# CRIPAC-DIG/GET

Measured on AMD Instinct MI355X. Metric: claim-evidence pairs/sec fwd+bwd (B=32, h=300), higher is better.
Workload: dtype f32

## Files before the change

### get_amd/_lib.py

```python
from __future__ import annotations

import ctypes
import os

import torch

_HERE = os.path.dirname(os.path.abspath(__file__))
LIB_PATH = os.environ.get("GET_AMD_LIB") or os.path.join(_HERE, "lib", "libget_hip.so")

_P = ctypes.c_void_p
_I = ctypes.c_int
_F = ctypes.c_float
_L = ctypes.c_int64
_U = ctypes.c_uint32
ABI_VERSION = 10

SIGNATURES = {
    "gh_graph_build": [_P, _P, _I, _I, _I, _P, _P, _P, _P, _P],
    "gh_adj_pack_f64": [_P, _I, _I, _P, _P, _P],
    "gh_ref_depad": [_P, _I, _I, _I, _P, _I, _P, _P, _P, _P, _P, _P, _P, _I, _P],
    "gh_adj_pack_f32": [_P, _I, _I, _P, _P, _P],
    "gh_ragged_plan": [_P, _P, _I, _I, _P, _P, _P, _P, _P, _P],
    "gh_spmm": [_P, _P, _P, _P, _P, _I, _P, _P, _I, _I, _I, _I, _I, _P],
    "gh_spmm_bf16": [_P, _P, _P, _P, _P, _I, _P, _P, _I, _I, _I, _I, _I, _P],
    "gh_transpose": [_P, _P, _I, _I, _P],
    "gh_transpose_batch": [_I, _P, _P, _P, _P, _P],
    "gh_ggnn_cell_fwd": [_P] * 5 + [_I, _I] + [_P] * 2 + [_I] * 4 + [_P] * 13 + [_P] * 7 + [_F, _U, _P, _P, _F, _U, _P],
    "gh_ggnn_cell_bwd": [_P] * 5 + [_I] + [_P] * 2 + [_I] * 4 + [_P] * 7 + [_P] * 7 + [_P] * 5 + [_P] * 14 + [_F, _U, _P],
    "gh_ggnn_cell_fwd_bf16": [_P] * 5 + [_I, _I] + [_P] * 2 + [_I] * 4 + [_P] * 13 + [_P] * 8 + [_F, _U, _P, _P, _F, _U, _P],
    "gh_ggnn_cell_bwd_bf16": [_P] * 5 + [_I] + [_P] * 2 + [_I] * 4 + [_P] * 7 + [_P] * 7 + [_P] * 5 + [_P] * 14 + [_F, _U, _P],
    "gh_scorer_gsl": [_P, _P, _P, _P, _I, _P, _P, _P, _P, _I, _I, _I, _I, _P, _P, _F, _U, _P],
    "gh_gsl_topk": [_P, _I, _I, _I, _P, _P],
    "gh_adj_unpack": [_P, _P, _P, _P, _I, _I, _P, _P],
    "gh_concat_att_fwd": [_P, _P, _P, _P, _P, _I, _I, _I, _I, _I, _I, _I, _P, _P, _P, _P, _P, _P, _P, _P],
    "gh_concat_att_bwd": [_P, _P, _P, _I, _I, _I, _I, _I, _I, _I, _P, _P, _P, _P, _P, _P, _P, _P, _P, _P, _P, _P, _P, _P],
    "gh_linear_fwd": [_P, _P, _P, _P, _I, _I, _I, _P],
    "gh_linear_bwd": [_P, _P, _P, _P, _I, _I, _I, _P, _P, _P, _P],
    "gh_linear_wgrad_bf16": [_P, _I, _P, _I, _I, _I, _I, _P, _I, _P, _P],
    "gh_gat_layer_fwd": [_P] * 6 + [_I] * 5 + [_F, _I, _I, _F, _U] + [_P] * 5 + [_P],
    "gh_gat_layer_bwd": [_P] * 6 + [_I] * 5 + [_F, _I, _I, _F, _U] + [_P] * 11 + [_P],
    "gh_gcn_norm": [_P, _P, _P, _P, _I, _I, _P, _P],
    "gh_feat_dropout": [_P, _P, _I, _I, _F, _U, _P],
    "gh_scale_rows": [_P, _P, _P, _P, _I, _I, _P],
    "gh_evd_assemble_fwd": [_P, _P, _P, _I, _P, _I, _P, _I, _I, _I, _I, _I, _I, _P, _P, _P],
    "gh_evd_assemble_bwd": [_P, _P, _P, _I, _I, _I, _I, _I, _I, _P, _P, _P],
    "gh_clamp_events": [_P, _I],
    "gh_weights_refresh": [_I, _P, _P, _P, _P, _P, _P, _P],
    "gh_seg_offsets": [_P, _I, _P, _P, _I, _P, _P],
    "gh_seg_broadcast": [_P, _P, _P, _I, _I, _P],
    "gh_seg_sum": [_P, _P, _P, _I, _I, _P],
    "gh_seg_pad": [_P, _P, _P, _I, _I, _I, _I, _P],
    "gh_seg_unpad": [_P, _P, _P, _I, _I, _I, _I, _P],
    "gh_masked_mean_fwd": [_P, _P, _P, _P, _I, _I, _I, _P],
    "gh_masked_mean_bwd": [_P, _P, _P, _P, _I, _I, _I, _P],
    "gh_adam_step": [_P, _P, _P, _P, _L, _F, _F, _F, _F, _F, _I, _F, _P],
    "gh_set_workspace": [_P, _L],
    "gh_set_stream_workspace": [_P, _P, _L],
    "gh_profile_enable": [_I],
    "gh_profile_select": [_U],
    "gh_profile_collect": [_P, _I],
    "gh_gemm_path_counters": [_P, _I],
    "gh_set_gemm_mode": [_I],
    "gh_weights_changed": [],
    "gh_fp32x3_refresh": [_P],
    "gh_fp32x3_clear": [],
    "gh_get_plan_buffers": [_P, _P, _P],
    "gh_get_forward": [_P, _P, _P, _P, _P, _P],
    "gh_get_backward": [_P, _P, _P, _P, _P, _P, _P, _P, _I, _P, _P],
    "gh_cross_entropy": [_P, _P, _I, _I, _P, _P, _P],
    "gh_get_prepare": [_P, _P, _I, _I, _P, _P, _I, _I, _I] + [_P] * 8 + [_I] + [_P] * 5 + [_P, _P, _P],
    "gh_get_struct_sizes": [_P],
    "gh_comm_unique_id": [_P],
    "gh_comm_init": [_P, _I, _I, _P],
    "gh_comm_destroy": [_P],
    "gh_comm_info": [_P, _P, _P],
    "gh_flat_allreduce": [_P, _P, _L, _P],
    "gh_flat_broadcast": [_P, _P, _L, _I, _P],
}

PROFILE_ROWS = ["gemm_big", "gemm_big_tn", "gemm_small", "gemm_small_tn", "spmm", "scorer_gsl",
                "graph_build", "att_softmax_fwd", "att_softmax_bwd", "att_dpre", "gate_bwd_pre", "colsum", "adam",
                "few_row_streams"]


def profile_enable(on: bool, only=None):
    mask = 0xFFFFFFFF if only is None else sum(1 << PROFILE_ROWS.index(n) for n in only)
    call("gh_profile_select", mask)
    call("gh_profile_enable", 1 if on else 0)


def profile_collect() -> dict:
    buf = (ctypes.c_double * (len(PROFILE_ROWS) * 3))()
    call("gh_profile_collect", ctypes.cast(buf, ctypes.c_void_p), len(PROFILE_ROWS))
    return {name: {"ms": buf[3 * i], "work": buf[3 * i + 1], "launches": int(buf[3 * i + 2])}
            for i, name in enumerate(PROFILE_ROWS)}

_GEMM_MODE = "fp32"


def set_gemm_mode(mode: str):
    global _GEMM_MODE
    call("gh_set_gemm_mode", {"fp32": 0, "bf16": 1, "fp32x3": 2, "fp32x3p": 3}[mode])
    _GEMM_MODE = mode


def gemm_mode() -> str:
    return _GEMM_MODE


def gemm_path_counters(reset: bool = False) -> dict:
    buf = (ctypes.c_int64 * 3)()
    call("gh_gemm_path_counters", ctypes.cast(buf, ctypes.c_void_p), 1 if reset else 0)
    return {"fast": int(buf[0]), "generic": int(buf[1]), "generic_large": int(buf[2])}


_lib = None


def load():
    global _lib
    if _lib is not None:
        return _lib
    if not os.path.exists(LIB_PATH):
        raise RuntimeError(
            f"get_amd: HIP library not found at {LIB_PATH}. Build it with "
            "`python -c \"import __graft_entry__ as g; g.build()\"` or `make -C get_amd/csrc`. "
            "There is no CPU fallback.")
    lib = ctypes.CDLL(LIB_PATH)
    lib.gh_abi_version.restype = _I
    lib.gh_last_error.restype = ctypes.c_char_p
    lib.gh_comm_library.restype = ctypes.c_char_p
    for name, args in SIGNATURES.items():
        fn = getattr(lib, name)
        fn.argtypes = args
        fn.restype = _I
    if lib.gh_abi_version() != ABI_VERSION:
        raise RuntimeError(f"get_amd: ABI version mismatch ({lib.gh_abi_version()} != {ABI_VERSION})")
    _lib = lib
    return lib


_workspaces = {}


def has_workspace(device, raw_stream) -> bool:
    dev = torch.device(device)
    idx = dev.index if dev.index is not None else _get_device()
    return (idx, raw_stream) in _workspaces


def ensure_workspace(device, nbytes: int = 256 << 20):
    dev = torch.device(device)
    if dev.index is None:
        dev = torch.device("cuda", torch.cuda.current_device())
    st = _get_raw_stream(dev.index) if _get_raw_stream is not None else torch.cuda.current_stream(dev).cuda_stream
    key = (dev.index, st)
    ws = _workspaces.get(key)
    if ws is None or ws.numel() * 4 < nbytes:
        ws = torch.empty(nbytes // 4, device=dev, dtype=torch.float32)
        _workspaces[key] = ws
        if dev.index != _get_device():
            with torch.cuda.device(dev):
                call("gh_set_stream_workspace", st, ws.data_ptr(), ws.numel() * 4)
        else:
            call("gh_set_stream_workspace", st, ws.data_ptr(), ws.numel() * 4)
    return ws


_get_device = torch._C._cuda_getDevice
_get_raw_stream = getattr(torch._C, "_cuda_getCurrentRawStream", None)


def ptr(t):
    if t is None:
        return None
    assert t.is_contiguous(), "get_amd: non-contiguous tensor handed to the C-ABI"
    if t.is_cuda and t.device.index != _get_device():
        raise RuntimeError(f"get_amd: tensor on cuda:{t.device.index} but the current device is cuda:{torch.cuda.current_device()}; "
                           "launches go to the current device's stream -- use `with torch.cuda.device(tensor.device):`")
    return t.data_ptr()


def stream():
    if _get_raw_stream is not None:
        return _get_raw_stream(_get_device())
    return torch.cuda.current_stream().cuda_stream


_fns: dict = {}


def call(name: str, *args):
    fn = _fns.get(name)
    if fn is None:
        fn = _fns[name] = getattr(load(), name)
    rc = fn(*args)
    if rc != 0:
        raise RuntimeError(f"get_amd: {name} failed (rc={rc}): {load().gh_last_error().decode(errors='replace')}")


def require_cuda(*tensors):
    for t in tensors:
        if t is not None and not t.is_cuda:
            raise RuntimeError("get_amd: tensors must live on a ROCm device (cuda:N); there is no CPU path")
```

### get_amd/csrc/common.h

```cpp
#pragma once
#include <hip/hip_runtime.h>
#include <stdint.h>
#include <stdio.h>
#include <stdlib.h>
#include <string.h>

namespace gh {

void set_error(const char* fmt, ...);

#define GH_CHECK_HIP(expr)                                                                  \
  do {                                                                                      \
    hipError_t _e = (expr);                                                                 \
    if (_e != hipSuccess) {                                                                 \
      gh::set_error("%s:%d: %s -> %s", __FILE__, __LINE__, #expr, hipGetErrorString(_e));   \
      return 1;                                                                             \
    }                                                                                       \
  } while (0)

#define GH_REQUIRE(cond, ...)                     \
  do {                                            \
    if (!(cond)) {                                \
      gh::set_error(__VA_ARGS__);                 \
      return 2;                                   \
    }                                             \
  } while (0)

#define GH_LAUNCH_CHECK() GH_CHECK_HIP(hipGetLastError())

inline int words_for(int r) { return (r + 63) / 64; }

inline int measure_env(const char* name, int dflt) {
#ifdef GH_MEASURE
  const char* e = getenv(name);
  return e ? atoi(e) : dflt;
#else
  (void)name;
  return dflt;
#endif
}
#ifdef GH_MEASURE
#define GH_DBG_BITS(L) ((L).dbg)
#else
#define GH_DBG_BITS(L) 0
#endif

enum ProfTag : int {
  PROF_GEMM_BIG = 0, PROF_GEMM_BIG_TN, PROF_GEMM_SMALL, PROF_GEMM_SMALL_TN,
  PROF_SPMM, PROF_SCORER_GSL, PROF_GRAPH_BUILD, PROF_ATT_SOFTMAX_FWD, PROF_ATT_SOFTMAX_BWD, PROF_ATT_DPRE,
  PROF_GATE_BWD_PRE, PROF_COLSUM, PROF_ADAM,
  PROF_FEW_ROWS,
  PROF_NTAGS
};
constexpr int PROF_FEW_GROUPS = 256;
unsigned int* clamp_counter();
bool prof_enabled();
void prof_begin(hipStream_t s, int tag);
void prof_end(int tag, double work, hipStream_t s);

int scorer_gsl_impl(const uint64_t* bits, const float* dinv, const float* vals, const int32_t* goff, int pads_collapsed, const float* feat,
                    const float* score_x, int score_parts, long long score_stride, const float* w_p, const float* gate, int n, int r, int h,
                    int k, float* score, uint64_t* keep, float drop_p, uint32_t drop_seed, hipStream_t stream);
int launch_ragged_plan(const int32_t* n_nodes, const int32_t* node_ids, int n, int r, int32_t* goff, int32_t* rowg, int32_t* src,
                       int32_t* cids, float* maskf, const int64_t* slot, int32_t* document, hipStream_t s, bool* scattered);
int launch_graph_build2(const int32_t* ta, const int32_t* la, int na, int ra, int32_t* ida, int32_t* nna, uint64_t* ba, float* da,
                        const int32_t* tb, const int32_t* lb, int nb, int rb, int32_t* idb, int32_t* nnb, uint64_t* bb, float* db,
                        int window, hipStream_t s);
struct ZeroFill { float* p0; long long n0; float* p1; long long n1; };
int launch_spmm(const uint64_t* bits, const float* dinv, const float* vals, const uint64_t* keep, const int32_t* goff,
                int m_real, const float* x, float* y, int n, int r, int h, int transpose, int accumulate, hipStream_t s,
                int bf16 = 0,
                const ZeroFill* zf = nullptr, bool* zf_done = nullptr);
int launch_gate_bwd_pre(const float* g, const float* z, const float* hh, const float* xp, float* dhp, float* dzp,
                        float* dxp, size_t count, hipStream_t s, int bf16 = 0);
int launch_colsum3(const float* a, const float* b, const float* c, float* oa, float* ob, float* oc, int m, int h,
                   hipStream_t s, float* oa2 = nullptr, float* ob2 = nullptr, float* oc2 = nullptr);
int launch_colsum(const float* a, float* oa, int m, int h, hipStream_t s);
struct Workspace { float* p; size_t bytes; float* cs; size_t cs_bytes; };
Workspace workspace_for(hipStream_t s);
int launch_gather_rows(const float* table, const int32_t* ids, float* dst, int m, int d, hipStream_t s,
                       float drop_p = 0.f, unsigned drop_seed = 0, int bf16 = 0);
int launch_tiny_linear_fwd(const float* x, const float* w, const float* bias, float* y, int m, int k, int n, hipStream_t s);
int launch_head_bwd(const float* g_phi, const float* y0, const float* w1, const float* w0, int B, int H, int C, int Xl, int E,
                    float* d_y0, float* dw1, float* db1, float* dx0, int dx0_accumulate, float* dx1, hipStream_t s);
size_t head_bwd_lds(int B, int H, int C, int E, const float* w0);
int launch_tiny_linear_bwd(const float* x, const float* w, const float* g, float* dx, float* dw, float* db, int m, int k, int n,
                           hipStream_t s);
int launch_att_softmax_fwd(float* e, const float* mask, const float* right, const int32_t* goff, int m_real,
                           int b, int l, int dr, int heads, float* weights, float* attended, hipStream_t s,
                           const float* e_parts = nullptr, int n_parts = 0, long long part_stride = 0, const void* right16 = nullptr);
int launch_att_softmax_bwd(const float* right, const float* weights, const float* g_att, const float* g_w,
                           const int32_t* goff, int m_real, int b, int l, int dr, int heads, float* de, float* dright,
                           hipStream_t s, const int32_t* rowg = nullptr, float* dw_tmp = nullptr, int* dw_written = nullptr,
                           const void* right16 = nullptr);
int gemm_mode();
int launch_att_dpre(const float* de, const float* w2, const float* t, const int32_t* goff, int m_real, int b, int l,
                    int ha, int heads, float* dpre, float* du, float* dw2_part, hipStream_t s, const float* dw_in = nullptr,
                    const float* weights = nullptr, float* de_out = nullptr, void* dpre16 = nullptr,
                    long long dw_range_stride = 0, int dw_ranges = 1);

struct GateFuse { const float* z; const float* hh; const float* xp; float* dhp; float* dzp; float* dxp; int bf16; };

int cell_fwd_impl(int bf, float* out32, const uint64_t* bits, const float* dinv, const float* vals, const uint64_t* keep,
                  const int32_t* goff, int m_real, int m_rows, const float* x, const int32_t* ids, int n, int r, int din, int h,
                  const float* w_p, const float* w_z0, const float* w_z1, const float* w_r0, const float* w_r1, const float* w_h0,
                  const float* w_h1, const float* b_z0, const float* b_z1, const float* b_r0, const float* b_r1, const float* b_h0,
                  const float* b_h1, float* xp, float* a, float* z, float* rr, float* rx, float* hh, float* out, float drop_p,
                  uint32_t drop_seed, const float* score_w, float* score_x, float score_drop_p, uint32_t score_drop_seed,
                  void* stream, int pad_out_dead = 0,
                  int* score_parts = nullptr,
                  float* xdrop = nullptr);
int cell_bwd_impl(int bf, const uint64_t* bits, const float* dinv, const float* vals, const uint64_t* keep, const int32_t* goff,
                  int m_real, const float* x, const int32_t* ids, int n, int r, int din, int h, const float* wt_p,
                  const float* wt_z0, const float* wt_z1, const float* wt_r0, const float* wt_r1, const float* wt_h0,
                  const float* wt_h1, const float* xp, const float* a, const float* z, const float* rr, const float* rx,
                  const float* hh, const float* g, float* dhp, float* dzp, float* drp, float* dxp, float* da, float* dx,
                  float* dw_p, float* dw_z0, float* dw_z1, float* dw_r0, float* dw_r1, float* dw_h0, float* dw_h1, float* db_z,
                  float* db_r, float* db_h, float* db_z1, float* db_r1, float* db_h1, float drop_p, uint32_t drop_seed, void* stream,
                  void* wstream, hipEvent_t ev_l1, hipEvent_t ev_agg,
                  int pre_done, const GateFuse* next,
                  const float* xdrop = nullptr);
int att_fwd_impl(const float* left, int nl, const int32_t* rowu, const float* right, const float* mask, const int32_t* goff,
                 const int32_t* rowg, int m_real, int b, int l, int xl, int dr, int ha, int heads, const float* w1, const float* w2,
                 float* u, float* t, float* e, float* weights, float* attended, hipStream_t s, int u_mode = 0,
                 const void* right16 = nullptr, const void* w1_16 = nullptr);
int att_bwd_impl(const float* left, const float* right, const int32_t* goff, int m_real, int b, int l, int xl, int dr, int ha,
                 int heads, const float* w1t, const float* w2, const float* t, const float* weights, const float* g_att,
                 const float* g_w, float* de, float* dpre, float* du, float* dleft, float* dright, float* dw1, float* dw2,
                 const int32_t* claim_offsets, int nl, float* du_c, int dleft_accumulate, hipStream_t s,
                 const int32_t* rowg = nullptr, float* dw_tmp = nullptr, const GateFuse* next = nullptr, int dleft_late = 0,
                 float* dw2_buf = nullptr, const void* right16 = nullptr, const void* w1t_16 = nullptr);
int linear2_fwd(const float* x0, int k0, const float* x1, int k1, const float* w, const float* bias, float* y, int m, int n, hipStream_t s,
                const float* w_out = nullptr, const float* b_out = nullptr, float* y_out = nullptr, int n_out = 0);
int linear2_bwd(const float* x0, int k0, const float* x1, int k1, const float* wt, const float* g, int m, int n, float* dx0,
                int dx0_accumulate, float* dx1, float* dw, float* db, hipStream_t s);

}
```

### get_amd/csrc/gemm_ops.hip

```cpp
#include "../../include/get_hip.h"
#include "common.h"
#include "gemm.hip.h"
#include "gemm_nt.hip.h"
#include "gemm_tn.hip.h"
#include "gemm_tn_pp.hip.h"
#include <stdlib.h>

namespace gh {

static inline bool al16(const void* p) { return (reinterpret_cast<uintptr_t>(p) & 15) == 0; }

static bool s_lds_bad(const Problem& p) { return p.seg[0].lda % 8 || p.seg[0].ldb % 8; }
static void fast_why(int rule, int prob, const Problem* p = nullptr, int seg = -1) {
  static const bool dbg = measure_env("GH_FASTOK_DEBUG", 0) != 0;
  if (!dbg) return;
  fprintf(stderr, "gemm: generic kernel (fast_ok rule %d, problem %d)\n", rule, prob);
  if (p && seg >= 0) fprintf(stderr, "   seg %d lda %d M %d N %d K %d\n", seg, p->seg[seg].lda, p->M, p->N, p->seg[seg].K);
}
static bool fast_ok(const Launch& L, bool tn) {
  for (int i = 0; i < L.nprob; ++i) {
    const Problem& p = L.p[i];
    const int ns = tn ? 1 : p.nseg;
    for (int j = 0; j < ns; ++j) {
      const Seg& s = p.seg[j];
      if (!s.vecA || !s.vecB || s.gatherB || s.K < 4) { fast_why(1, i); return false; }
      if (tn && s.gatherA) { fast_why(2, i); return false; }
    }
    if (p.elt && tn && (p.M % 8 || p.N % 8 || s_lds_bad(p))) { fast_why(3, i); return false; }
    if (!tn) {
      for (int j = 0; j < p.nseg; ++j) {
        if (4.0 * (double)p.seg[j].ldb * (double)p.N >= 2147483648.0) { fast_why(4, i); return false; }
        if (!p.seg[j].gatherA && 4.0 * (double)p.seg[j].lda * (double)p.M >= 2147483648.0) { fast_why(5, i, &p, j); return false; }
      }
    }
    if (tn) {
      const Seg& s = p.seg[0];
      if (4.0 * (double)s.lda * (double)s.K >= 2147483648.0 || 4.0 * (double)s.ldb * (double)s.K >= 2147483648.0) { fast_why(6, i); return false; }
    }
    if (p.N % 4 || p.N < 4 || p.ldc % 4 || !al16(p.C)) { fast_why(7, i); return false; }
    if (tn && (p.M % 4 || p.M < 4)) { fast_why(8, i); return false; }
    if ((p.bias && !al16(p.bias)) || (p.bias2 && !al16(p.bias2)) || (p.out1 && !al16(p.out1)) || (p.in0 && !al16(p.in0)) || (p.in1 && !al16(p.in1)))
      { fast_why(9, i); return false; }
    if (p.epi == EPI_ATT && (!al16(p.u) || p.ldu % 4 || !al16(p.w2))) { fast_why(10, i); return false; }
    if (p.epi == EPI_TANH_H && p.w2 && !al16(p.w2)) { fast_why(11, i); return false; }
    if (p.epi == EPI_GATE_PRE && (tn || !p.in0 || !p.in1 || !p.in2 || !p.out1 || !p.out2 || !al16(p.in2) || !al16(p.out2) ||
                                  (p.gin && !al16(p.gin)))) { fast_why(12, i); return false; }
  }
  return true;
}
constexpr int TN_PP_ROWS = 16384;
static bool wants_dropout(const Launch& L) {
  for (int i = 0; i < L.nprob; ++i)
    if (L.p[i].drop_mode) return true;
  return false;
}

static long long g_path_counts[3] = {0, 0, 0};
static int g_gemm_mode = 0;
static bool x3p_substitute(Launch& L, hipStream_t s);

int gemm_mode() { return g_gemm_mode; }

template <int WM, int WN, int NI, int MI = 2>
static hipError_t launch_cfg(const Launch& L, bool tn, hipStream_t s) {
  const bool fast = fast_ok(L, tn);
  {
    double fl = 0.0;
    for (int i = 0; i < L.nprob; ++i)
      for (int j = 0; j < L.p[i].nseg; ++j) fl += 2.0 * L.p[i].M * L.p[i].N * (double)L.p[i].seg[j].K;
    g_path_counts[fast ? 0 : 1] += 1;
    if (!fast && fl >= 1e9) g_path_counts[2] += 1;
  }
  const int n_outer = tn ? L.ksplit : L.m_tiles;
  const int n_inner = tn ? L.m_tiles * L.nprob : L.nprob * L.ksplit;
  const bool nt_few = !tn && L.m_tiles < 8 && fast;
  const int grid = nt_few ? n_outer * n_inner : 8 * ((n_outer + 7) / 8) * n_inner;
  if (grid <= 0) return hipSuccess;
  int max_rows = 0;
  for (int i = 0; i < L.nprob; ++i) { const int rws = tn ? L.p[i].seg[0].K : L.p[i].M; if (rws > max_rows) max_rows = rws; }
  const int tag = (max_rows >= 8192 ? PROF_GEMM_BIG : PROF_GEMM_SMALL) + (tn ? 1 : 0);
  double flops = 0.0;
  if (prof_enabled()) {
    for (int i = 0; i < L.nprob; ++i)
      for (int j = 0; j < L.p[i].nseg; ++j) {
        int rows = L.p[i].M;
        if (j == 0 && !tn && L.p[i].nseg > 1 && L.p[i].seg0_rows > 0) {
          const int bm = 16 * MI * WM, cut = ((L.p[i].seg0_rows + bm - 1) / bm) * bm;
          if (cut < rows) rows = cut;
        }
        flops += 2.0 * rows * L.p[i].N * (double)L.p[i].seg[j].K;
      }
    prof_begin(s, tag);
  }
  if (!fast && wants_dropout(L)) return hipErrorInvalidValue;
  if (!fast && !tn)
    for (int i = 0; i < L.nprob; ++i)
      if ((L.p[i].epi == EPI_TANH_H && L.p[i].w2) || L.p[i].epi == EPI_GATE_PRE || (L.p[i].epi == EPI_ATT && L.p[i].e_atomic == 2))
        return hipErrorInvalidValue;
  bool launched = false;
  bool any_elt = false, all_elt = true;
  for (int i = 0; i < L.nprob; ++i) { any_elt = any_elt || L.p[i].elt; all_elt = all_elt && L.p[i].elt; }
  if (any_elt) {
    if (!fast || !all_elt) return hipErrorInvalidValue;
    if constexpr (WM == 2 && WN == 2 && NI == 10) {
      if (tn) hipLaunchKernelGGL((gemm_tn_bf16_kernel<2, 2, 10, 4>), dim3(grid), dim3(256), 0, s, L);
      else hipLaunchKernelGGL((gemm_nt_kernel<2, 2, 10, 2, 2>), dim3(grid), dim3(256), 0, s, L);
      launched = true;
    } else if constexpr (WM == 2 && WN == 2 && NI == 8 && MI == 4) {
      if (tn) return hipErrorInvalidValue;
      constexpr int kLds = 3 * (128 + 256) * 64;
      static bool attr = false;
      if (!attr) { (void)hipFuncSetAttribute((const void*)gemm_nt_kernel<2, 2, 8, 4, 2>, hipFuncAttributeMaxDynamicSharedMemorySize, kLds); attr = true; }
      hipLaunchKernelGGL((gemm_nt_kernel<2, 2, 8, 4, 2>), dim3(grid), dim3(256), kLds, s, L);
      launched = true;
    } else if constexpr (WM == 2 && WN == 4 && NI == 4 && MI == 8) {
      if (tn) return hipErrorInvalidValue;
      constexpr int kLds = 131072;
      static bool attr = false;
      if (!attr) { (void)hipFuncSetAttribute((const void*)gemm_nt_kernel<2, 4, 4, 8, 2>, hipFuncAttributeMaxDynamicSharedMemorySize, kLds); attr = true; }
      hipLaunchKernelGGL((gemm_nt_kernel<2, 4, 4, 8, 2>), dim3(grid), dim3(512), kLds, s, L);
      launched = true;
    } else return hipErrorInvalidValue;
  } else if (MI >= 4) {
    return hipErrorInvalidValue;
  }
  if constexpr (MI == 2) {
  if (launched) {
  } else if (fast && !tn) {
    if (g_gemm_mode == 1 && WM == 2 && WN == 2 && NI == 10) {
      if constexpr (WM == 2 && WN == 2 && NI == 10)
        hipLaunchKernelGGL((gemm_nt_kernel<2, 2, 10, 2, true>), dim3(grid), dim3(256), 0, s, L);
    } else if (g_gemm_mode == 1 && WM == 1 && WN == 4 && NI == 5) {
      if constexpr (WM == 1 && WN == 4 && NI == 5)
        hipLaunchKernelGGL((gemm_nt_kernel<1, 4, 5, 2, true>), dim3(grid), dim3(256), 0, s, L);
    } else if (g_gemm_mode == 2 || g_gemm_mode == 3) {
      Launch L2;
      bool pre = false;
      if (g_gemm_mode == 3) { L2 = L; pre = x3p_substitute(L2, s); }
      if (pre) {
        constexpr int kLds = 2 * (16 * 2 * WM * 64 + 16 * NI * WN * 112);
        static bool attr = false;
        if (!attr) { (void)hipFuncSetAttribute((const void*)gemm_nt_kernel<WM, WN, NI, 2, 4>, hipFuncAttributeMaxDynamicSharedMemorySize, kLds); attr = true; }
        hipLaunchKernelGGL((gemm_nt_kernel<WM, WN, NI, 2, 4>), dim3(grid), dim3(WM * WN * 64), kLds, s, L2);
      } else
        hipLaunchKernelGGL((gemm_nt_kernel<WM, WN, NI, 2, 3>), dim3(grid), dim3(WM * WN * 64), 0, s, L);
    } else
      hipLaunchKernelGGL((gemm_nt_kernel<WM, WN, NI, 2>), dim3(grid), dim3(WM * WN * 64), 0, s, L);
    launched = true;
  } else if (fast && tn) {
    if constexpr (WM == 2 && WN == 2 && NI == 10) {
      if (g_gemm_mode == 1) hipLaunchKernelGGL((gemm_tn_kernel<2, 2, 10, true>), dim3(grid), dim3(256), 0, s, L);
      else hipLaunchKernelGGL((gemm_tn_kernel<2, 2, 10>), dim3(grid), dim3(256), 0, s, L);
      launched = true;
    }
  }
  if (!launched) {
    if (tn) hipLaunchKernelGGL((gemm_kernel<WM, WN, NI, true>), dim3(grid), dim3(WM * WN * 64), 0, s, L);
    else hipLaunchKernelGGL((gemm_kernel<WM, WN, NI, false>), dim3(grid), dim3(WM * WN * 64), 0, s, L);
  }
  }
  if (!launched && MI != 2) return hipErrorInvalidValue;
  prof_end(tag, flops, s);
  return hipGetLastError();
}

static hipError_t launch_tn_pp(const Launch& L, hipStream_t s) {
  const int grid = 8 * L.per;
  if (grid <= 0) return hipSuccess;
  g_path_counts[0] += 1;
  const int tag = PROF_GEMM_BIG + 1;
  double flops = 0.0;
  if (prof_enabled()) {
    for (int i = 0; i < L.nprob; ++i) flops += 2.0 * L.p[i].M * L.p[i].N * (double)L.p[i].seg[0].K;
    prof_begin(s, tag);
  }
  constexpr int kLds = 131072;
  static bool attr = false;
  if (!attr) { (void)hipFuncSetAttribute((const void*)gemm_tn_pp_kernel, hipFuncAttributeMaxDynamicSharedMemorySize, kLds); attr = true; }
  hipLaunchKernelGGL(gemm_tn_pp_kernel, dim3(grid), dim3(512), kLds, s, L);
  prof_end(tag, flops, s);
  return hipGetLastError();
}

}
#include <mutex>
#include <unordered_map>
#include <vector>
namespace gh {
struct X3Item { const float* src; unsigned char* dst; int N, ldb, K, pitch; };
constexpr int X3_BATCH = 64;
struct X3Args { int n; X3Item it[X3_BATCH]; };
__global__ void __launch_bounds__(256) split3_kernel(const X3Args a) {
  const X3Item& it = a.it[blockIdx.y];
  const int G = it.pitch / 24;
  const long long total = (long long)it.N * G;
  for (long long idx = (long long)blockIdx.x * 256 + threadIdx.x; idx < total; idx += (long long)gridDim.x * 256) {
    const int row = (int)(idx / G), g = (int)(idx - (long long)row * G);
    const float* src = it.src + (size_t)row * it.ldb + 4 * g;
    float v[4];
#pragma unroll
    for (int e = 0; e < 4; ++e) v[e] = (4 * g + e < it.K) ? src[e] : 0.f;
    unsigned hi[2], mid[2], lo[2];
    hi[0] = nt_pack_bf16(v[0], v[1]); hi[1] = nt_pack_bf16(v[2], v[3]);
    const float r0 = v[0] - __builtin_bit_cast(float, hi[0] << 16), r1 = v[1] - __builtin_bit_cast(float, hi[0] & 0xffff0000u);
    const float r2 = v[2] - __builtin_bit_cast(float, hi[1] << 16), r3 = v[3] - __builtin_bit_cast(float, hi[1] & 0xffff0000u);
    mid[0] = nt_pack_bf16(r0, r1); mid[1] = nt_pack_bf16(r2, r3);
    const float q0 = r0 - __builtin_bit_cast(float, mid[0] << 16), q1 = r1 - __builtin_bit_cast(float, mid[0] & 0xffff0000u);
    const float q2 = r2 - __builtin_bit_cast(float, mid[1] << 16), q3 = r3 - __builtin_bit_cast(float, mid[1] & 0xffff0000u);
    lo[0] = nt_pack_bf16(q0, q1); lo[1] = nt_pack_bf16(q2, q3);
    uint2* dst = reinterpret_cast<uint2*>(it.dst + (size_t)row * it.pitch + (size_t)g * 24);
    dst[0] = make_uint2(hi[0], hi[1]); dst[1] = make_uint2(mid[0], mid[1]); dst[2] = make_uint2(lo[0], lo[1]);
  }
}
struct X3Key {
  const void* b; int ldb, K, N;
  bool operator==(const X3Key& o) const { return b == o.b && ldb == o.ldb && K == o.K && N == o.N; }
};
struct X3Hash {
  size_t operator()(const X3Key& k) const {
    size_t h = std::hash<const void*>()(k.b);
    h ^= std::hash<long long>()(((long long)k.ldb << 40) ^ ((long long)k.K << 20) ^ (long long)k.N) + 0x9e3779b97f4a7c15ull + (h << 6) + (h >> 2);
    return h;
  }
};
struct X3Ent { unsigned char* img; int pitch; long long epoch; };
static std::mutex g_x3_mu;
static std::unordered_map<X3Key, X3Ent, X3Hash> g_x3;
static std::unordered_multimap<size_t, unsigned char*> g_x3_pool;
static long long g_x3_epoch = 0;

static void x3p_split(const X3Item* items, int n, hipStream_t s) {
  for (int i0 = 0; i0 < n; i0 += X3_BATCH) {
    X3Args a;
    a.n = n - i0 < X3_BATCH ? n - i0 : X3_BATCH;
    long long mx = 0;
    for (int i = 0; i < a.n; ++i) {
      a.it[i] = items[i0 + i];
      const long long t = (long long)a.it[i].N * (a.it[i].pitch / 24);
      if (t > mx) mx = t;
    }
    int gx = (int)((mx + 255) / 256);
    if (gx > 256) gx = 256;
    if (gx < 1) gx = 1;
    hipLaunchKernelGGL(split3_kernel, dim3(gx, a.n), dim3(256), 0, s, a);
  }
}

static bool x3p_substitute(Launch& L, hipStream_t s) {
  std::lock_guard<std::mutex> lk(g_x3_mu);
  X3Item todo[2 * GH_MAX_PROBLEMS];
  int nt = 0;
  for (int i = 0; i < L.nprob; ++i) {
    Problem& q = L.p[i];
    if (q.elt) return false;
    for (int j = 0; j < q.nseg; ++j) {
      Seg& g = q.seg[j];
      if (g.K <= 0 || g.gatherB) return false;
      const X3Key key{g.B, g.ldb, g.K, q.N};
      auto f = g_x3.find(key);
      if (f == g_x3.end()) {
        if (g_x3.size() >= 512) return false;
        X3Ent e;
        e.pitch = ((g.K + 15) / 16) * 96;
        e.epoch = -1;
        const size_t bytes = (size_t)q.N * e.pitch + 256;
        auto pf = g_x3_pool.find(bytes);
        if (pf != g_x3_pool.end()) { e.img = pf->second; g_x3_pool.erase(pf); }
        else if (hipMalloc((void**)&e.img, bytes) != hipSuccess) { (void)hipGetLastError(); return false; }
        f = g_x3.emplace(key, e).first;
      }
      if (f->second.epoch != g_x3_epoch) {
        todo[nt++] = X3Item{g.B, f->second.img, q.N, g.ldb, g.K, f->second.pitch};
        f->second.epoch = g_x3_epoch;
      }
      g.B = reinterpret_cast<const float*>(f->second.img);
      g.ldb = f->second.pitch / 4;
    }
  }
  if (nt > 0) x3p_split(todo, nt, s);
  return true;
}
static std::mutex g_ws_mu;
static Workspace g_ws_default = {nullptr, 0, nullptr, 0};
struct WsKey { int dev; hipStream_t s; bool operator==(const WsKey& o) const { return dev == o.dev && s == o.s; } };
struct WsKeyHash { size_t operator()(const WsKey& k) const { return std::hash<const void*>()((const void*)k.s) * 31u + (size_t)(k.dev + 1); } };
static std::unordered_map<WsKey, Workspace, WsKeyHash> g_ws_stream;
static int current_device() { int d = 0; if (hipGetDevice(&d) != hipSuccess) d = 0; return d; }
static Workspace make_workspace(void* ptr, int64_t bytes) {
  Workspace w = {nullptr, 0, nullptr, 0};
  if (!ptr || bytes < (1 << 20)) return w;
  const size_t tail = ((size_t)bytes / 16) & ~(size_t)15;
  w.p = (float*)ptr;
  w.bytes = ((size_t)bytes - tail) & ~(size_t)15;
  w.cs = (float*)((char*)ptr + w.bytes);
  w.cs_bytes = tail;
  return w;
}
Workspace workspace_for(hipStream_t s) {
  std::lock_guard<std::mutex> lk(g_ws_mu);
  auto it = g_ws_stream.find(WsKey{current_device(), s});
  return it != g_ws_stream.end() ? it->second : g_ws_default;
}

struct ReduceItem { const float* ws; float* out; int I, J, ldc, ks; long long stride; };
struct ReduceArgs { ReduceItem it[3 * GH_MAX_PROBLEMS]; int n; };

__global__ void __launch_bounds__(256)
reduce_partials_kernel(const ReduceArgs R) {
  const ReduceItem& it = R.it[blockIdx.y];
  const int J4 = it.J / 4;
  const size_t total = (size_t)it.I * J4;
  for (size_t e = (size_t)blockIdx.x * blockDim.x + threadIdx.x; e < total; e += (size_t)gridDim.x * blockDim.x) {
    const int i = (int)(e / J4), j = 4 * (int)(e % J4);
    float4 acc = make_float4(0.f, 0.f, 0.f, 0.f);
    const float* p = it.ws + (size_t)i * it.J + j;
    int k = 0;
    for (; k + 8 <= it.ks; k += 8) {
      float4 v[8];
#pragma unroll
      for (int u = 0; u < 8; ++u) v[u] = *reinterpret_cast<const float4*>(p + (size_t)(k + u) * it.stride);
#pragma unroll
      for (int u = 0; u < 8; ++u) { acc.x += v[u].x; acc.y += v[u].y; acc.z += v[u].z; acc.w += v[u].w; }
    }
    for (; k < it.ks; ++k) {
      const float4 v = *reinterpret_cast<const float4*>(p + (size_t)k * it.stride);
      acc.x += v.x; acc.y += v.y; acc.z += v.z; acc.w += v.w;
    }
    float* o = it.out + (size_t)i * it.ldc + j;
    o[0] += acc.x; o[1] += acc.y; o[2] += acc.z; o[3] += acc.w;
  }
}

__global__ void __launch_bounds__(256)
reduce_partials_wave_kernel(const ReduceArgs R) {
  const ReduceItem& it = R.it[blockIdx.y];
  const int J4 = it.J / 4;
  const int total = it.I * J4;
  const int e = blockIdx.x * 4 + (threadIdx.x >> 6), lane = threadIdx.x & 63;
  if (e >= total) return;
  const int i = e / J4, j = 4 * (e % J4);
  const float* p = it.ws + (size_t)i * it.J + j;
  float4 acc = make_float4(0.f, 0.f, 0.f, 0.f);
  for (int k = lane; k < it.ks; k += 64) {
    const float4 v = *reinterpret_cast<const float4*>(p + (size_t)k * it.stride);
    acc.x += v.x; acc.y += v.y; acc.z += v.z; acc.w += v.w;
  }
  for (int o = 32; o > 0; o >>= 1) {
    acc.x += __shfl_xor(acc.x, o); acc.y += __shfl_xor(acc.y, o); acc.z += __shfl_xor(acc.z, o); acc.w += __shfl_xor(acc.w, o);
  }
  if (lane == 0) {
    float* o = it.out + (size_t)i * it.ldc + j;
    o[0] += acc.x; o[1] += acc.y; o[2] += acc.z; o[3] += acc.w;
  }
}

struct FinishItem {
  const float* ws; long long stride; int ks; int M, N, epi, accumulate, ldc;
  float* C; const float* bias; const float* bias2; float* out1; const float* in0; const float* in1;
  const float* u; const float* w2; float* e; int ldu, R, heads;
  const int32_t* rowg;
};

struct FinishArgs { FinishItem it[GH_MAX_PROBLEMS]; int n; int split; };

__global__ void __launch_bounds__(256)
nt_finish_kernel(const FinishArgs F) {
  const FinishItem& it = F.it[blockIdx.y];
  const int lane = threadIdx.x & 63, wave = threadIdx.x >> 6;
  const bool split = F.split != 0;
  const int row = split ? (int)blockIdx.x : (int)blockIdx.x * 4 + wave;
  if (row >= it.M) return;
  const int N4 = it.N / 4;
  __shared__ float4 part[3][64];
  int kb = 0, ke = it.ks;
  if (split) { const int kq = (it.ks + 3) / 4; kb = wave * kq; ke = min(it.ks, kb + kq); }
  float pe[8];
#pragma unroll
  for (int c = 0; c < 8; ++c) pe[c] = 0.f;
  for (int c0 = 0; c0 < N4; c0 += 64) {
    const int c4 = c0 + lane;
    const int col = 4 * c4;
    float4 v = make_float4(0.f, 0.f, 0.f, 0.f);
    if (c4 < N4 && kb < ke) {
      const float* p = it.ws + (size_t)row * it.N + col;
      for (int k0 = kb; k0 < ke; k0 += 8) {
        float4 x[8];
#pragma unroll
        for (int u = 0; u < 8; ++u) x[u] = *reinterpret_cast<const float4*>(p + (size_t)min(k0 + u, ke - 1) * it.stride);
#pragma unroll
        for (int u = 0; u < 8; ++u)
          if (k0 + u < ke) { v.x += x[u].x; v.y += x[u].y; v.z += x[u].z; v.w += x[u].w; }
      }
    }
    if (split) {
      if (c0 > 0) __syncthreads();
      if (wave > 0) part[wave - 1][lane] = v;
      __syncthreads();
      if (wave > 0) continue;
#pragma unroll
      for (int w = 0; w < 3; ++w) { const float4 q = part[w][lane]; v.x += q.x; v.y += q.y; v.z += q.z; v.w += q.w; }
    }
    if (c4 >= N4) continue;
    const size_t oo = (size_t)row * it.ldc + col;
    float* o = it.C + oo;
    if (it.bias) { const float4 b4 = *reinterpret_cast<const float4*>(it.bias + col); v.x += b4.x; v.y += b4.y; v.z += b4.z; v.w += b4.w; }
    if (it.bias2) { const float4 b4 = *reinterpret_cast<const float4*>(it.bias2 + col); v.x += b4.x; v.y += b4.y; v.z += b4.z; v.w += b4.w; }
    if (it.epi == EPI_ATT) {
      const float4 u4 = *reinterpret_cast<const float4*>(it.u + (size_t)(it.rowg ? it.rowg[row] : row / it.R) * it.ldu + col);
      const float4 t = make_float4(tanhf_(v.x + u4.x), tanhf_(v.y + u4.y), tanhf_(v.z + u4.z), tanhf_(v.w + u4.w));
      *reinterpret_cast<float4*>(o) = t;
#pragma unroll
      for (int c = 0; c < 8; ++c)
        if (c < it.heads) {
          const float4 w = *reinterpret_cast<const float4*>(it.w2 + (size_t)c * it.N + col);
          pe[c] += t.x * w.x + t.y * w.y + t.z * w.z + t.w * w.w;
        }
    } else if (it.epi == EPI_SIGMOID_Z) {
      *reinterpret_cast<float4*>(o) = make_float4(sigmoidf_(v.x), sigmoidf_(v.y), sigmoidf_(v.z), sigmoidf_(v.w));
    } else if (it.epi == EPI_SIGMOID_R) {
      const float4 x = *reinterpret_cast<const float4*>(it.in0 + oo);
      const float4 r4 = make_float4(sigmoidf_(v.x), sigmoidf_(v.y), sigmoidf_(v.z), sigmoidf_(v.w));
      *reinterpret_cast<float4*>(o) = r4;
      *reinterpret_cast<float4*>(it.out1 + oo) = make_float4(r4.x * x.x, r4.y * x.y, r4.z * x.z, r4.w * x.w);
    } else if (it.epi == EPI_TANH_H) {
      const float4 z = *reinterpret_cast<const float4*>(it.in0 + oo);
      const float4 x = *reinterpret_cast<const float4*>(it.in1 + oo);
      const float4 h = make_float4(tanhf_(v.x), tanhf_(v.y), tanhf_(v.z), tanhf_(v.w));
      *reinterpret_cast<float4*>(o) = h;
      *reinterpret_cast<float4*>(it.out1 + oo) = make_float4(h.x * z.x + x.x * (1.f - z.x), h.y * z.y + x.y * (1.f - z.y),
                                                             h.z * z.z + x.z * (1.f - z.z), h.w * z.w + x.w * (1.f - z.w));
    } else if (it.epi == EPI_BWD_DRX) {
      const float4 x = *reinterpret_cast<const float4*>(it.in0 + oo);
      const float4 r4 = *reinterpret_cast<const float4*>(it.in1 + oo);
      float4 d = *reinterpret_cast<const float4*>(it.out1 + oo);
      *reinterpret_cast<float4*>(o) = make_float4(v.x * x.x * r4.x * (1.f - r4.x), v.y * x.y * r4.y * (1.f - r4.y),
                                                  v.z * x.z * r4.z * (1.f - r4.z), v.w * x.w * r4.w * (1.f - r4.w));
      d.x += v.x * r4.x; d.y += v.y * r4.y; d.z += v.z * r4.z; d.w += v.w * r4.w;
      *reinterpret_cast<float4*>(it.out1 + oo) = d;
    } else {
      if (it.accumulate) {
        const float4 c4v = *reinterpret_cast<const float4*>(o);
        v.x += c4v.x; v.y += c4v.y; v.z += c4v.z; v.w += c4v.w;
      }
      *reinterpret_cast<float4*>(o) = v;
      if (it.w2) {
#pragma unroll
        for (int c = 0; c < 8; ++c)
          if (c < it.heads) {
            const float4 w = *reinterpret_cast<const float4*>(it.w2 + (size_t)c * it.N + col);
            pe[c] += v.x * w.x + v.y * w.y + v.z * w.z + v.w * w.w;
          }
      }
    }
  }
  const bool proj = it.epi == EPI_STORE && it.w2 != nullptr;
  if ((it.epi == EPI_ATT || proj) && (!split || wave == 0)) {
#pragma unroll
    for (int c = 0; c < 8; ++c) {
      float v = pe[c];
      for (int o = 32; o > 0; o >>= 1) v += __shfl_xor(v, o);
      if (lane == 0 && c < it.heads) it.e[(size_t)row * it.heads + c] = v + ((proj && it.in0) ? it.in0[c] : 0.f);
    }
  }
}

constexpr int NARROW_DEFAULT = 14;
struct Batch {
  Launch L;
  bool tn, big;
  hipStream_t s;
  int bm, bn;
  hipError_t err = hipSuccess;
  int k_total = 0;
  float* cs_out[GH_MAX_PROBLEMS] = {nullptr};
  float* cs_out2[GH_MAX_PROBLEMS] = {nullptr};
  bool colsum_fused = false;
  bool colsum_missed = false;
  bool split_done = false;
  void want_colsum(float* o, float* o2) { if (L.nprob > 0) { cs_out[L.nprob - 1] = o; cs_out2[L.nprob - 1] = o2; } }

  float* g_ws = nullptr;
  size_t g_ws_bytes = 0;
  bool narrow = false;
  long long e_block_stride = 0;
  bool wide = false;
  bool wide256 = false;
  bool tn_pp = false;
  bool tn_pp_ok(const Problem& p) const {
    if (!tn || !p.elt || p.nseg != 1 || g_ws == nullptr || p.epi != EPI_ATOMIC) return false;
    const Seg& sg = p.seg[0];
    if (sg.gatherA || sg.gatherB || !sg.vecA || !sg.vecB || sg.K < TN_PP_ROWS) return false;
    if (p.M % 256 || p.N % 256 || p.ldc % 4 || (reinterpret_cast<uintptr_t>(p.C) & 15)) return false;
    return (size_t)sg.K * (size_t)sg.lda * 2 < ((size_t)1 << 31) && (size_t)sg.K * (size_t)sg.ldb * 2 < ((size_t)1 << 31);
  }
  Batch(bool tn_, int rows_hint, hipStream_t s_, bool wide_bf16 = false, int site = 0, int n_hint = 0) : tn(tn_), s(s_) {
    const Workspace w = workspace_for(s_);
    g_ws = w.p; g_ws_bytes = w.bytes;
    big = tn_ || rows_hint >= 8192;
    bm = big ? 64 : 32;
    bn = 320;
    if (wide_bf16 && big && !tn_) { wide = true; bm = 128; bn = 256; }
    constexpr int tile256_rows = 32768;
    if (wide && rows_hint >= tile256_rows) { wide256 = true; bm = 256; }
    const bool less_pad = n_hint > 0 && (n_hint + 159) / 160 * 160 < (n_hint + 319) / 320 * 320;
    const bool thin = rows_hint <= 24576;
    if (site > 0 && big && !tn_ && !wide && g_gemm_mode == 0 && (((NARROW_DEFAULT >> (site - 1)) & 1) || less_pad || thin)) { narrow = true; bn = 160; }
    reset();
  }
  void reset() {
    L.nprob = 0; L.m_tiles = 0; L.ksplit = 1; L.kchunk = 0; k_total = 0; L.n_tiles = 0; L.per = 0;
    static const int dbg = measure_env("GH_DBG", 0);
    L.dbg = dbg;
    for (int i = 0; i < GH_MAX_PROBLEMS; ++i) cs_out[i] = cs_out2[i] = nullptr;
  }

  void add(const Problem& p) {
    const bool scorer_blocks = p.epi == EPI_TANH_H && p.w2 && p.N > bn && narrow && p.N <= 2 * bn;
    const bool att_blocks = p.epi == EPI_ATT && p.N > bn && e_block_stride > 0;
    const bool scorer_parts = p.epi == EPI_TANH_H && p.w2 && p.N > bn && !scorer_blocks && e_block_stride > 0;
    if ((p.epi == EPI_ATT || (p.epi == EPI_TANH_H && p.w2)) && p.N > bn && !scorer_blocks && !att_blocks && !scorer_parts) { err = hipErrorInvalidValue; return; }
    if (tn) {
      const bool want = tn_pp_ok(p);
      if (L.nprob > 0 && want != tn_pp) flush();
      if (L.nprob == 0) tn_pp = want;
    }
    const int bn = tn_pp ? (1 << 30) : this->bn;
    for (int n0 = 0; n0 < p.N; n0 += bn) {
      Problem q = p;
      q.N = (p.N - n0 < bn) ? p.N - n0 : bn;
      auto adv = [](const float* ptr, size_t elems, bool bf) { return (const float*)((const char*)ptr + elems * (bf ? 2 : 4)); };
      for (int i = 0; i < q.nseg; ++i) {
        if (tn) {
          q.seg[i].B = adv(q.seg[i].B, (size_t)n0, q.elt);
          q.seg[i].vecB = q.elt ? (((reinterpret_cast<uintptr_t>(q.seg[i].B) & 15) == 0) && q.seg[i].ldb % 8 == 0 && q.N % 8 == 0)
                                : vec_ok(q.seg[i].B, q.seg[i].ldb, q.N);
        } else {
          q.seg[i].B = adv(q.seg[i].B, (size_t)n0 * q.seg[i].ldb, q.elt);
        }
      }
      q.C = (float*)adv(q.C, (size_t)n0, q.io & 1);
      q.drop_col0 = p.drop_col0 + n0;
      if (q.bias) q.bias += n0;
      if (q.bias2) q.bias2 += n0;
      if (q.out1) q.out1 = (float*)adv(q.out1, (size_t)n0, q.io & 2);
      if (q.in0) q.in0 = adv(q.in0, (size_t)n0, q.io & 4);
      if (q.in1) q.in1 = adv(q.in1, (size_t)n0, q.io & 8);
      if (q.c32) q.c32 += n0;
      if (q.gin) q.gin += n0;
      if (q.in2) q.in2 = adv(q.in2, (size_t)n0, q.io & 16);
      if (q.out2) q.out2 = (float*)adv(q.out2, (size_t)n0, q.io & 32);
      if (scorer_blocks) { q.w2 += n0; q.e_atomic = 1; }
      if (scorer_parts) { q.w2 += n0; q.e = p.e + (size_t)(n0 / bn) * (size_t)e_block_stride; q.e_atomic = 2; }
      if (att_blocks) { q.w2 += n0; q.u += n0; q.e = p.e + (size_t)(n0 / bn) * (size_t)e_block_stride; q.e_atomic = 2; }
      if (L.nprob == GH_MAX_PROBLEMS) flush();
      L.p[L.nprob++] = q;
      const int bm_eff = tn_pp ? 256 : (tn && q.elt) ? 128 : bm;
      const int mt = (q.M + bm_eff - 1) / bm_eff;
      if (mt > L.m_tiles) L.m_tiles = mt;
      if (tn_pp && (q.N + 255) / 256 > L.n_tiles) L.n_tiles = (q.N + 255) / 256;
      if (q.seg[0].K > k_total) k_total = q.seg[0].K;
    }
  }

  void flush() {
    if (L.nprob == 0 || err != hipSuccess) { reset(); return; }
    if (tn) {
      const int n_inner = L.m_tiles * L.nprob;
      constexpr int target = 2304;
      int ks = (target + n_inner - 1) / n_inner;
      constexpr int min_rows16 = 4096;
      const int min_rows = L.p[0].elt ? min_rows16 : 256;
      const int ks_max = (k_total / min_rows > 1) ? k_total / min_rows : 1;
      if (ks > ks_max) ks = ks_max;
      if (ks < 1) ks = 1;
      const int align = tn_pp ? 64 : L.p[0].elt ? 32 : 16;
      if (tn_pp) {
        const int tiles = L.nprob * L.m_tiles * L.n_tiles;
        const int ks1 = 256 / tiles > 0 ? 256 / tiles : 1, ks2 = 512 / tiles > 0 ? 512 / tiles : 1;
        const double e1 = tiles * ks1 / 256.0, e2 = tiles * ks2 / 512.0;
        ks = (e1 >= 0.85 || e1 >= e2) ? ks1 : ks2;
        const int kmax = k_total / 1024 > 1 ? k_total / 1024 : 1;
        if (ks > kmax) ks = kmax;
        size_t out_bytes = 0;
        for (int i = 0; i < L.nprob; ++i) out_bytes += ((size_t)L.p[i].M * L.p[i].N + (cs_out[i] ? (size_t)L.p[i].M : 0)) * sizeof(float);
        while (ks > 1 && (size_t)ks * out_bytes > g_ws_bytes) --ks;
      } else
      if (ks >= 12) ks = ((ks + 4) / 8) * 8;
      int chunk = (k_total + ks - 1) / ks;
      chunk = ((chunk + align - 1) / align) * align;
      L.kchunk = chunk;
      L.ksplit = (k_total + chunk - 1) / chunk;
      if (tn_pp) L.per = (L.nprob * L.m_tiles * L.n_tiles * L.ksplit + 7) / 8;
      if (!tn_pp && L.ksplit >= 12 && L.ksplit % 8 != 0) {
        const int k8 = (L.ksplit / 8) * 8;
        chunk = (((k_total + k8 - 1) / k8 + align - 1) / align) * align;
        if ((k_total + chunk - 1) / chunk % 8 == 0) { L.kchunk = chunk; L.ksplit = (k_total + chunk - 1) / chunk; }
      }
      size_t need = 0;
      bool want_cs0 = false;
      for (int i = 0; i < L.nprob; ++i) want_cs0 = want_cs0 || cs_out[i] != nullptr;
      bool ws_ok = g_ws != nullptr && (L.ksplit > 1 || tn_pp || (want_cs0 && L.p[0].elt));
      bool any_cs = false;
      for (int i = 0; i < L.nprob && ws_ok; ++i) {
        if (L.p[i].N % 4) ws_ok = false;
        need += (size_t)L.ksplit * L.p[i].M * L.p[i].N * sizeof(float);
        if (cs_out[i]) { need += (size_t)L.ksplit * L.p[i].M * sizeof(float); any_cs = true; }
      }
      bool want_cs = false;
      for (int i = 0; i < L.nprob; ++i) want_cs = want_cs || cs_out[i] != nullptr;
      if (any_cs && !(ws_ok && need <= g_ws_bytes && fast_ok(L, true) && (g_gemm_mode != 1 || L.p[0].elt))) any_cs = false;
      if (want_cs && !any_cs) {
        for (int i = 0; i < L.nprob; ++i) {
          if (!cs_out[i]) continue;
          const Seg& sg = L.p[i].seg[0];
          if (L.p[i].elt || sg.lda != L.p[i].M) { colsum_missed = true; continue; }
          if (launch_colsum3(sg.A, nullptr, nullptr, cs_out[i], nullptr, nullptr, sg.K, L.p[i].M, s, cs_out2[i], nullptr, nullptr)) colsum_missed = true;
          else colsum_fused = true;
        }
      }
      if (ws_ok && need <= g_ws_bytes) {
        ReduceArgs R;
        R.n = L.nprob;
        float* w = g_ws;
        int max_elems = 0;
        for (int i = 0; i < L.nprob; ++i) {
          Problem& q = L.p[i];
          R.it[i] = ReduceItem{w, q.C, q.M, q.N, q.ldc, L.ksplit, (long long)q.M * q.N};
          q.C = w; q.ldc = q.N; q.epi = EPI_STORE; q.accumulate = 0; q.split_stride = (long long)q.M * q.N;
          w += (size_t)L.ksplit * q.M * q.N;
          if (q.M * (q.N / 4) > max_elems) max_elems = q.M * (q.N / 4);
        }
        ReduceArgs RC;
        RC.n = 0;
        int max_cs = 0;
        for (int i = 0; i < L.nprob && any_cs; ++i) {
          Problem& q = L.p[i];
          if (!cs_out[i]) continue;
          q.colsum = w; q.colsum_stride = q.M;
          RC.it[RC.n++] = ReduceItem{w, cs_out[i], 1, q.M, q.M, L.ksplit, (long long)q.M};
          if (cs_out2[i] && RC.n < GH_MAX_PROBLEMS) RC.it[RC.n++] = ReduceItem{w, cs_out2[i], 1, q.M, q.M, L.ksplit, (long long)q.M};
          w += (size_t)L.ksplit * q.M;
          if (q.M / 4 > max_cs) max_cs = q.M / 4;
        }
        hipError_t e = launch_any();
        if (e != hipSuccess) err = e;
        for (int i = 0; i < RC.n; ++i) R.it[R.n++] = RC.it[i];
        if (max_cs > max_elems) max_elems = max_cs;
        hipLaunchKernelGGL(reduce_partials_kernel, dim3((max_elems + 255) / 256, R.n), dim3(256), 0, s, R);
        if (RC.n > 0) colsum_fused = true;
        e = hipGetLastError();
        if (e != hipSuccess) err = e;
        reset();
        return;
      }
    }
    if (tn && tn_pp) { err = hipErrorInvalidValue; reset(); return; }
    if (!tn && nt_split_plan()) return;
    hipError_t e = launch_any();
    if (e != hipSuccess) err = e;
    reset();
  }

  hipError_t launch_any() {
    if (tn && tn_pp) return launch_tn_pp(L, s);
    if (narrow && !tn && L.ksplit == 1 && !L.p[0].elt) return launch_cfg<2, 2, 5>(L, tn, s);
    if (big && !tn && L.ksplit == 1 && !L.p[0].elt) {
      const double r = (double)L.m_tiles * L.nprob / 768.0;
      const double frac = r - (double)(long long)r;
      if (g_gemm_mode != 1 && r < 3.0 && frac > 0.02 && frac < 0.45) {
        int mt = 0;
        for (int i = 0; i < L.nprob; ++i) { const int t = (L.p[i].M + 31) / 32; if (t > mt) mt = t; }
        L.m_tiles = mt;
        return launch_cfg<1, 4, 5>(L, tn, s);
      }
    }
    if (wide256) {
      bool ok = L.ksplit == 1;
      for (int i = 0; i < L.nprob; ++i) {
        if (L.p[i].drop_mode == 1) ok = false;
        for (int j = 0; j < L.p[i].nseg; ++j) if (L.p[i].seg[j].K % 64) ok = false;
      }
      if (ok) return launch_cfg<2, 4, 4, 8>(L, tn, s);
      int mt = 0;
      for (int i = 0; i < L.nprob; ++i) { const int t = (L.p[i].M + 127) / 128; if (t > mt) mt = t; }
      L.m_tiles = mt;
      return launch_cfg<2, 2, 8, 4>(L, tn, s);
    }
    if (wide) return launch_cfg<2, 2, 8, 4>(L, tn, s);
    return big ? launch_cfg<2, 2, 10>(L, tn, s) : launch_cfg<1, 4, 5>(L, tn, s);
  }

  bool nt_split_plan() {
    const int blocks = L.m_tiles * L.nprob;
    constexpr int max_blocks = 96;
    if (g_ws == nullptr || blocks >= max_blocks || !fast_ok(L, false)) return false;
    int tmax = 0;
    for (int i = 0; i < L.nprob; ++i) {
      const Problem& q = L.p[i];
      if (q.epi == EPI_ATOMIC || q.epi == EPI_GATE_PRE || q.drop_mode != 0 || (q.epi == EPI_TANH_H && q.w2) || q.seg0_rows > 0 || q.elt) return false;
      int t = 0;
      for (int j = 0; j < q.nseg; ++j) t += (q.seg[j].K + 15) / 16;
      if (i > 0 && t != tmax) return false;
      tmax = t;
    }
    int ks = tmax / 4;
    const int tgt = tmax >= 128 ? 512 : 256;
    const int want = (tgt + blocks - 1) / blocks;
    if (ks > want) ks = want;
    if (ks < 2) return false;
    const int ct = (tmax + ks - 1) / ks;
    ks = (tmax + ct - 1) / ct;
    if (ks < 2) return false;
    size_t need = 0;
    for (int i = 0; i < L.nprob; ++i) need += (size_t)ks * L.p[i].M * L.p[i].N * sizeof(float);
    if (need > g_ws_bytes) return false;
    FinishArgs F;
    F.n = L.nprob;
    float* w = g_ws;
    int max_m = 0;
    for (int i = 0; i < L.nprob; ++i) {
      Problem& q = L.p[i];
      F.it[i] = FinishItem{w, (long long)q.M * q.N, ks, q.M, q.N, q.epi, q.accumulate, q.ldc,
                           q.C, q.bias, q.bias2, q.out1, q.in0, q.in1, q.u, q.w2, q.e, q.ldu, q.R, q.heads, q.rowg};
      q.C = w; q.ldc = q.N; q.epi = EPI_STORE; q.accumulate = 0; q.bias = nullptr; q.bias2 = nullptr;
      q.split_stride = (long long)q.M * q.N;
      w += (size_t)ks * q.M * q.N;
      if (q.M > max_m) max_m = q.M;
    }
    L.ksplit = ks;
    L.kchunk = ct * 16;
    hipError_t e = launch_any();
    if (e != hipSuccess) err = e;
    F.split = (ks >= 16 && max_m <= 8192) ? 1 : 0;
    hipLaunchKernelGGL(nt_finish_kernel, dim3(F.split ? max_m : (max_m + 3) / 4, F.n), dim3(256), 0, s, F);
    split_done = true;
    e = hipGetLastError();
    if (e != hipSuccess) err = e;
    reset();
    return true;
  }
};

static Problem gemm_problem(int M, int N, int epi, float* C, int ldc, const float* A, int lda, const float* B, int ldb,
                            int K, const int32_t* gatherA = nullptr, int elt = 0) {
  Problem p = make_problem(M, N, epi, C, ldc);
  p.elt = elt;
  p.seg[0] = make_seg_nt(A, lda, B, ldb, K, gatherA, elt);
  return p;
}
static void add_seg(Problem& p, const float* A, int lda, const float* B, int ldb, int K) {
  p.seg[p.nseg++] = make_seg_nt(A, lda, B, ldb, K, nullptr, p.elt);
}
static void set_dropout(Problem& p, int mode, int ld, float drop_p, unsigned seed) {
  if (drop_p <= 0.f) return;
  p.drop_mode = mode; p.drop_ld = ld; p.drop_col0 = 0; p.drop_seed = seed;
  const double t = (double)drop_p * 4294967296.0;
  p.drop_thresh = t >= 4294967295.0 ? 4294967295u : (unsigned)t;
  p.drop_scale = 1.0f / (1.0f - drop_p);
}
static Problem tn_problem(int I, int J, float* C, int ldc, const float* A, int lda, const float* B, int ldb, int K,
                          const int32_t* gatherB = nullptr, int elt = 0) {
  Problem p = make_problem(I, J, EPI_ATOMIC, C, ldc);
  p.seg[0] = make_seg_tn(A, lda, I, B, ldb, J, K, nullptr, gatherB);
  p.elt = elt;
  if (elt) {
    p.seg[0].vecA = ((reinterpret_cast<uintptr_t>(A) & 15) == 0) && lda % 8 == 0 && I % 8 == 0;
    p.seg[0].vecB = ((reinterpret_cast<uintptr_t>(B) & 15) == 0) && ldb % 8 == 0 && J % 8 == 0;
  }
  return p;
}

}

using namespace gh;

int gh::cell_fwd_impl(int bf, float* out32, const uint64_t* bits, const float* dinv, const float* vals, const uint64_t* keep,
                                const int32_t* goff, int m_real, int m_rows,
                                const float* x, const int32_t* ids, int n, int r, int din, int h,
                                const float* w_p, const float* w_z0, const float* w_z1, const float* w_r0,
                                const float* w_r1, const float* w_h0, const float* w_h1,
                                const float* b_z0, const float* b_z1, const float* b_r0, const float* b_r1,
                                const float* b_h0, const float* b_h1,
                                float* xp, float* a, float* z, float* rr, float* rx, float* hh, float* out,
                                float drop_p, uint32_t drop_seed,
                                const float* score_w, float* score_x, float score_drop_p, uint32_t score_drop_seed,
                                gh_stream_t stream, int pad_out_dead, int* score_parts, float* xdrop) {
  hipStream_t s = (hipStream_t)stream;
  if (score_parts) *score_parts = 1;
  GH_REQUIRE(n > 0 && r > 0 && din > 0 && h > 0, "ggnn_cell_fwd: bad sizes n=%d r=%d din=%d h=%d", n, r, din, h);
  GH_REQUIRE(!bf || (din % 8 == 0 && h % 8 == 0), "ggnn_cell_fwd_bf16: needs din %% 8 == 0, h %% 8 == 0 (din=%d h=%d)", din, h);
  if (!goff) { m_real = n * r; m_rows = n * r; }
  GH_REQUIRE(m_real >= 0 && m_real <= m_rows && m_rows <= n * r, "ggnn_cell_fwd: node-compact rows %d/%d do not fit n*r=%d", m_real, m_rows, n * r);
  const int M = m_rows;
  if (M == 0) return 0;
  GH_REQUIRE(drop_p >= 0.f && drop_p < 1.f, "ggnn_cell_fwd: dropout p=%f not in [0,1)", drop_p);
  GH_REQUIRE((drop_p <= 0.f && score_drop_p <= 0.f) || (long long)M * (long long)(din > h ? din : h) < (1LL << 32),
             "ggnn_cell_fwd: %d rows x %d columns exceed the dropout mask's 32-bit element index", M, din > h ? din : h);
  GH_REQUIRE((score_w == nullptr) == (score_x == nullptr), "ggnn_cell_fwd: score_w and score_x come together");
  GH_REQUIRE(score_drop_p >= 0.f && score_drop_p < 1.f, "ggnn_cell_fwd: scorer dropout p=%f not in [0,1)", score_drop_p);
  const bool wide = bf && h % 256 == 0;
  const bool pre_drop = bf && xdrop && drop_p > 0.f && din <= h;
  if (pre_drop) {
    if (int e = launch_gather_rows(x, ids, xdrop, M, din, s, drop_p, drop_seed, 1)) return e;
  }
  {
    Batch b(false, M, s, wide, 7, h);
    Problem p = pre_drop ? gemm_problem(M, h, EPI_STORE, xp, h, xdrop, din, w_p, din, din, nullptr, bf)
                         : gemm_problem(M, h, EPI_STORE, xp, h, x, din, w_p, din, din, ids, bf);
    p.io = bf ? 1 : 0;
    if (!pre_drop) set_dropout(p, 1, din, drop_p, drop_seed);
    b.add(p);
    b.flush();
    GH_REQUIRE(b.err != hipErrorInvalidValue || drop_p == 0.f, "ggnn_cell_fwd: fused dropout needs float4-shaped rows (din=%d, h=%d)", din, h);
    GH_CHECK_HIP(b.err);
  }
  bool partial_zero = false;
  ZeroFill zf = {nullptr, 0, nullptr, 0};
  bool zf_done = false, score_zero = false;
  if (score_w) {
    Batch bh(false, M, s, false, 2, h);
    score_zero = bh.narrow && h <= 2 * bh.bn && h > bh.bn;
  }
  if (m_rows > m_real) {
    const uintptr_t al = (uintptr_t)a | (uintptr_t)xp | (uintptr_t)z | (uintptr_t)rr | (uintptr_t)rx | (uintptr_t)hh | (uintptr_t)out |
                         (uintptr_t)w_z0 | (uintptr_t)w_z1 | (uintptr_t)w_r0 | (uintptr_t)w_r1 | (uintptr_t)w_h0 | (uintptr_t)w_h1 |
                         (uintptr_t)b_z0 | (uintptr_t)b_z1 | (uintptr_t)b_r0 | (uintptr_t)b_r1 | (uintptr_t)b_h0 | (uintptr_t)b_h1;
    partial_zero = ((al & 15) == 0) && (h % (bf ? 8 : 4) == 0) && h >= 4 && 4.0 * (double)h * (double)M < 2147483648.0;
    const int zfull = ((m_real + 127) / 128 + 1) * 128;
    const int zend = (partial_zero && zfull < m_rows) ? zfull : m_rows;
    if (!bf) { zf.p0 = a + (size_t)m_real * h; zf.n0 = (long long)(zend - m_real) * h; }
    if (!bf && score_zero && M % 4 == 0) { zf.p1 = score_x; zf.n1 = M; }
    if (int e = launch_spmm(bits, dinv, vals, keep, goff, m_real, xp, a, n, r, h, 0, 0, s, bf, bf ? nullptr : &zf, &zf_done)) return e;
    if (!zf_done)
      GH_CHECK_HIP(hipMemsetAsync((char*)a + (size_t)m_real * h * (bf ? 2 : 4), 0, (size_t)(bf ? 2 : 4) * (size_t)(zend - m_real) * h, s));
  } else {
    if (int e = launch_spmm(bits, dinv, vals, keep, goff, m_real, xp, a, n, r, h, 0, 0, s, bf)) return e;
  }
  const long long generic_before = g_path_counts[1];
  {
    Batch b(false, M, s, wide, 1, h);
    Problem pz = gemm_problem(M, h, EPI_SIGMOID_Z, z, h, a, h, w_z0, h, h, nullptr, bf);
    pz.io = bf ? 1 : 0;
    add_seg(pz, xp, h, w_z1, h, h);
    pz.bias = b_z0; pz.bias2 = b_z1;
    Problem pr = gemm_problem(M, h, EPI_SIGMOID_R, rr, h, a, h, w_r0, h, h, nullptr, bf);
    pr.io = bf ? 7 : 0;
    add_seg(pr, xp, h, w_r1, h, h);
    pr.bias = b_r0; pr.bias2 = b_r1; pr.out1 = rx; pr.in0 = xp;
    if (m_rows > m_real) pz.seg0_rows = pr.seg0_rows = (m_real > 0 ? m_real : 1);
    b.add(pz); b.add(pr);
    b.flush();
    GH_CHECK_HIP(b.err);
  }
  {
    const bool parts_ok = score_w && score_parts != nullptr;
    Batch b(false, M, s, wide && (!score_w || parts_ok), 2, h);
    if (parts_ok && h > b.bn && !(b.narrow && h <= 2 * b.bn)) {
      b.e_block_stride = M;
      *score_parts = (h + b.bn - 1) / b.bn;
    } else if (score_w && b.narrow) {
      if (h > 2 * b.bn) { b.narrow = false; b.bn = 320; }
      else if (h > b.bn && !(zf_done && zf.p1 == score_x)) GH_CHECK_HIP(hipMemsetAsync(score_x, 0, sizeof(float) * (size_t)M, s));
    }
    Problem ph = gemm_problem(M, h, EPI_TANH_H, hh, h, a, h, w_h0, h, h, nullptr, bf);
    ph.io = bf ? 15 : 0; ph.c32 = bf ? out32 : nullptr;
    add_seg(ph, rx, h, w_h1, h, h);
    ph.bias = b_h0; ph.bias2 = b_h1; ph.out1 = out; ph.in0 = z; ph.in1 = xp;
    if (m_rows > m_real) ph.seg0_rows = (m_real > 0 ? m_real : 1);
    if (score_w) {
      ph.w2 = score_w; ph.e = score_x;
      if (pad_out_dead && m_rows > m_real) ph.ldu = 1;
      set_dropout(ph, 2, h, score_drop_p, score_drop_seed);
    }
    b.add(ph);
    b.flush();
    GH_REQUIRE(b.err != hipErrorInvalidValue || !score_w, "ggnn_cell_fwd: the fused scorer projection needs h %% 4 == 0 and h <= 320 (h=%d)", h);
    GH_CHECK_HIP(b.err);
  }
  GH_REQUIRE(!partial_zero || g_path_counts[1] == generic_before,
             "ggnn_cell_fwd: internal -- a gate GEMM took the generic kernel although the padding rows of `a` were only zeroed for the fast one");
  return 0;
}

extern "C" int gh_ggnn_cell_fwd(const uint64_t* bits, const float* dinv, const float* vals, const uint64_t* keep,
                                const int32_t* goff, int m_real, int m_rows,
                                const float* x, const int32_t* ids, int n, int r, int din, int h,
                                const float* w_p, const float* w_z0, const float* w_z1, const float* w_r0,
                                const float* w_r1, const float* w_h0, const float* w_h1,
                                const float* b_z0, const float* b_z1, const float* b_r0, const float* b_r1,
                                const float* b_h0, const float* b_h1,
                                float* xp, float* a, float* z, float* rr, float* rx, float* hh, float* out,
                                float drop_p, uint32_t drop_seed,
                                const float* score_w, float* score_x, float score_drop_p, uint32_t score_drop_seed,
                                gh_stream_t stream) {
  return cell_fwd_impl(0, nullptr, bits, dinv, vals, keep, goff, m_real, m_rows, x, ids, n, r, din, h, w_p, w_z0, w_z1, w_r0, w_r1,
                       w_h0, w_h1, b_z0, b_z1, b_r0, b_r1, b_h0, b_h1, xp, a, z, rr, rx, hh, out, drop_p, drop_seed, score_w,
                       score_x, score_drop_p, score_drop_seed, stream, 0, nullptr, nullptr);
}

extern "C" int gh_ggnn_cell_fwd_bf16(const uint64_t* bits, const float* dinv, const float* vals, const uint64_t* keep,
                                     const int32_t* goff, int m_real, int m_rows,
                                     const void* x, const int32_t* ids, int n, int r, int din, int h,
                                     const void* w_p, const void* w_z0, const void* w_z1, const void* w_r0,
                                     const void* w_r1, const void* w_h0, const void* w_h1,
                                     const float* b_z0, const float* b_z1, const float* b_r0, const float* b_r1,
                                     const float* b_h0, const float* b_h1,
                                     void* xp, void* a, void* z, void* rr, void* rx, void* hh, void* out, float* out32,
                                     float drop_p, uint32_t drop_seed,
                                     const float* score_w, float* score_x, float score_drop_p, uint32_t score_drop_seed,
                                     gh_stream_t stream) {
  typedef const float* cf;
  typedef float* mf;
  return cell_fwd_impl(1, out32, bits, dinv, vals, keep, goff, m_real, m_rows, (cf)x, ids, n, r, din, h, (cf)w_p, (cf)w_z0, (cf)w_z1,
                       (cf)w_r0, (cf)w_r1, (cf)w_h0, (cf)w_h1, b_z0, b_z1, b_r0, b_r1, b_h0, b_h1, (mf)xp, (mf)a, (mf)z, (mf)rr,
                       (mf)rx, (mf)hh, (mf)out, drop_p, drop_seed, score_w, score_x, score_drop_p, score_drop_seed, stream, 0, nullptr, nullptr);
}

int gh::cell_bwd_impl(int bf, const uint64_t* bits, const float* dinv, const float* vals, const uint64_t* keep,
                                const int32_t* goff, int m_real,
                                const float* x, const int32_t* ids, int n, int r, int din, int h,
                                const float* wt_p, const float* wt_z0, const float* wt_z1, const float* wt_r0,
                                const float* wt_r1, const float* wt_h0, const float* wt_h1,
                                const float* xp, const float* a, const float* z, const float* rr, const float* rx,
                                const float* hh, const float* g,
                                float* dhp, float* dzp, float* drp, float* dxp, float* da,
                                float* dx, float* dw_p, float* dw_z0, float* dw_z1, float* dw_r0, float* dw_r1,
                                float* dw_h0, float* dw_h1, float* db_z, float* db_r, float* db_h,
                                float* db_z1, float* db_r1, float* db_h1, float drop_p, uint32_t drop_seed,
                                gh_stream_t stream, gh_stream_t wstream, hipEvent_t ev_l1, hipEvent_t ev_agg,
                                int pre_done, const GateFuse* next, const float* xdrop) {
  hipStream_t s = (hipStream_t)stream;
  hipStream_t sw = wstream ? (hipStream_t)wstream : s;
  const bool two = sw != s;
  GH_REQUIRE(!two || (ev_l1 && ev_agg), "ggnn_cell_bwd: a separate weight-gradient stream needs its two events");
  GH_REQUIRE(n > 0 && r > 0 && din > 0 && h > 0, "ggnn_cell_bwd: bad sizes");
  GH_REQUIRE(!bf || (din % 8 == 0 && h % 8 == 0 && din <= h), "ggnn_cell_bwd_bf16: needs din %% 8 == 0, h %% 8 == 0, din <= h (din=%d h=%d)", din, h);
  if (!goff) m_real = n * r;
  GH_REQUIRE(m_real >= 0 && m_real <= n * r, "ggnn_cell_bwd: node-compact rows %d do not fit n*r=%d", m_real, n * r);
  GH_REQUIRE(drop_p <= 0.f || (long long)n * r * (long long)din < (1LL << 32),
             "ggnn_cell_bwd: %d rows x %d columns exceed the dropout mask's 32-bit element index", n * r, din);
  const int M = m_real;
  if (M == 0) return 0;
  if (!pre_done)
    if (int e = launch_gate_bwd_pre(g, z, hh, xp, dhp, dzp, dxp, (size_t)M * h, s, bf)) return e;
  const bool wide = bf && h % 256 == 0;
  {
    Batch b(false, M, s, wide, 3, h);
    Problem p0 = gemm_problem(M, h, EPI_STORE, da, h, dhp, h, wt_h0, h, h, nullptr, bf);
    Problem p1 = gemm_problem(M, h, EPI_BWD_DRX, drp, h, dhp, h, wt_h1, h, h, nullptr, bf);
    p1.out1 = dxp; p1.in0 = xp; p1.in1 = rr;
    p0.io = bf ? 1 : 0; p1.io = bf ? 15 : 0;
    b.add(p0); b.add(p1);
    b.flush();
    GH_CHECK_HIP(b.err);
  }
  const bool cs = bf ? true : (h % 4 == 0);
  bool colsum_done = false;
  if (two) {
    GH_CHECK_HIP(hipEventRecord(ev_l1, s));
    GH_CHECK_HIP(hipStreamWaitEvent(sw, ev_l1, 0));
    Batch b(true, M, sw);
    b.add(tn_problem(h, h, dw_z0, h, dzp, h, a, h, M, nullptr, bf));  if (cs) b.want_colsum(db_z, db_z1);
    b.add(tn_problem(h, h, dw_z1, h, dzp, h, xp, h, M, nullptr, bf));
    b.add(tn_problem(h, h, dw_r0, h, drp, h, a, h, M, nullptr, bf));  if (cs) b.want_colsum(db_r, db_r1);
    b.add(tn_problem(h, h, dw_r1, h, drp, h, xp, h, M, nullptr, bf));
    b.add(tn_problem(h, h, dw_h0, h, dhp, h, a, h, M, nullptr, bf));  if (cs) b.want_colsum(db_h, db_h1);
    b.add(tn_problem(h, h, dw_h1, h, dhp, h, rx, h, M, nullptr, bf));
    b.flush();
    GH_CHECK_HIP(b.err);
    colsum_done = b.colsum_fused && !b.colsum_missed;
    if (!colsum_done) {
      GH_REQUIRE(!bf, "ggnn_cell_bwd_bf16: the bias gradients need the split-K workspace (gh_set_workspace)");
      if (int e = launch_colsum3(dzp, drp, dhp, db_z, db_r, db_h, M, h, sw, db_z1, db_r1, db_h1)) return e;
    }
  }
  {
    Batch b(false, M, s, wide, 4, h);
    Problem p0 = gemm_problem(M, h, EPI_STORE, da, h, dzp, h, wt_z0, h, h, nullptr, bf);
    add_seg(p0, drp, h, wt_r0, h, h);
    p0.accumulate = 1;
    Problem p1 = gemm_problem(M, h, EPI_STORE, dxp, h, dzp, h, wt_z1, h, h, nullptr, bf);
    add_seg(p1, drp, h, wt_r1, h, h);
    p1.accumulate = 1;
    p0.io = p1.io = bf ? 1 : 0;
    b.add(p0); b.add(p1);
    b.flush();
    GH_CHECK_HIP(b.err);
  }
  if (int e = launch_spmm(bits, dinv, vals, keep, goff, m_real, da, dxp, n, r, h, 1, 1, s, bf)) return e;
  if (two) {
    GH_CHECK_HIP(hipEventRecord(ev_agg, s));
    GH_CHECK_HIP(hipStreamWaitEvent(sw, ev_agg, 0));
  }
  if (dx || next) {
    GH_REQUIRE(!next || (din % 4 == 0 && (next->bf16 != 0) == (bf != 0)), "ggnn_cell_bwd: the fused gate head needs float4-shaped rows and both cells in the same storage mode");
    Batch b(false, M, s, wide && din % 256 == 0, 5, din);
    Problem p = gemm_problem(M, din, next ? EPI_GATE_PRE : EPI_STORE, next ? next->dhp : dx, din, dxp, h, wt_p, h, h, nullptr, bf);
    if (next) {
      p.in0 = next->z; p.in1 = next->hh; p.in2 = next->xp; p.out1 = next->dzp; p.out2 = next->dxp;
      p.io = next->bf16 ? (1 | 2 | 4 | 8 | 16 | 32) : 0;
    }
    set_dropout(p, 3, din, drop_p, drop_seed);
    b.add(p);
    b.flush();
    GH_CHECK_HIP(b.err);
  }
  {
    Batch b(true, M, sw);
    if (!two) {
      b.add(tn_problem(h, h, dw_z0, h, dzp, h, a, h, M, nullptr, bf));  if (cs) b.want_colsum(db_z, db_z1);
      b.add(tn_problem(h, h, dw_z1, h, dzp, h, xp, h, M, nullptr, bf));
      b.add(tn_problem(h, h, dw_r0, h, drp, h, a, h, M, nullptr, bf));  if (cs) b.want_colsum(db_r, db_r1);
      b.add(tn_problem(h, h, dw_r1, h, drp, h, xp, h, M, nullptr, bf));
      b.add(tn_problem(h, h, dw_h0, h, dhp, h, a, h, M, nullptr, bf));  if (cs) b.want_colsum(db_h, db_h1);
      b.add(tn_problem(h, h, dw_h1, h, dhp, h, rx, h, M, nullptr, bf));
    }
    if (bf && xdrop && drop_p > 0.f && din <= h) {
      b.add(tn_problem(h, din, dw_p, din, dxp, h, xdrop, din, M, nullptr, bf));
    } else if ((ids || drop_p > 0.f || bf) && din <= h) {
      if (int e = launch_gather_rows(x, ids, da, M, din, sw, drop_p, drop_seed, bf)) return e;
      b.add(tn_problem(h, din, dw_p, din, dxp, h, da, din, M, nullptr, bf));
    } else {
      GH_REQUIRE(drop_p == 0.f, "ggnn_cell_bwd: fused dropout needs din (%d) <= h (%d)", din, h);
      b.add(tn_problem(h, din, dw_p, din, dxp, h, x, din, M, ids));
    }
    b.flush();
    GH_CHECK_HIP(b.err);
    if (two || (b.colsum_fused && !b.colsum_missed)) return 0;
  }
  GH_REQUIRE(!bf, "ggnn_cell_bwd_bf16: the bias gradients need the split-K workspace (gh_set_workspace)");
  return launch_colsum3(dzp, drp, dhp, db_z, db_r, db_h, M, h, s, db_z1, db_r1, db_h1);
}

extern "C" int gh_ggnn_cell_bwd(const uint64_t* bits, const float* dinv, const float* vals, const uint64_t* keep,
                                const int32_t* goff, int m_real,
                                const float* x, const int32_t* ids, int n, int r, int din, int h,
                                const float* wt_p, const float* wt_z0, const float* wt_z1, const float* wt_r0,
                                const float* wt_r1, const float* wt_h0, const float* wt_h1,
                                const float* xp, const float* a, const float* z, const float* rr, const float* rx,
                                const float* hh, const float* g,
                                float* dhp, float* dzp, float* drp, float* dxp, float* da,
                                float* dx, float* dw_p, float* dw_z0, float* dw_z1, float* dw_r0, float* dw_r1,
                                float* dw_h0, float* dw_h1, float* db_z, float* db_r, float* db_h,
                                float* db_z1, float* db_r1, float* db_h1, float drop_p, uint32_t drop_seed,
                                gh_stream_t stream) {
  return cell_bwd_impl(0, bits, dinv, vals, keep, goff, m_real, x, ids, n, r, din, h, wt_p, wt_z0, wt_z1, wt_r0, wt_r1, wt_h0, wt_h1,
                       xp, a, z, rr, rx, hh, g, dhp, dzp, drp, dxp, da, dx, dw_p, dw_z0, dw_z1, dw_r0, dw_r1, dw_h0, dw_h1,
                       db_z, db_r, db_h, db_z1, db_r1, db_h1, drop_p, drop_seed, stream, nullptr, nullptr, nullptr, 0, nullptr, nullptr);
}

extern "C" int gh_ggnn_cell_bwd_bf16(const uint64_t* bits, const float* dinv, const float* vals, const uint64_t* keep,
                                     const int32_t* goff, int m_real,
                                     const void* x, const int32_t* ids, int n, int r, int din, int h,
                                     const void* wt_p, const void* wt_z0, const void* wt_z1, const void* wt_r0,
                                     const void* wt_r1, const void* wt_h0, const void* wt_h1,
                                     const void* xp, const void* a, const void* z, const void* rr, const void* rx,
                                     const void* hh, const float* g,
                                     void* dhp, void* dzp, void* drp, void* dxp, void* da,
                                     float* dx, float* dw_p, float* dw_z0, float* dw_z1, float* dw_r0, float* dw_r1,
                                     float* dw_h0, float* dw_h1, float* db_z, float* db_r, float* db_h,
                                     float* db_z1, float* db_r1, float* db_h1, float drop_p, uint32_t drop_seed,
                                     gh_stream_t stream) {
  typedef const float* cf;
  typedef float* mf;
  return cell_bwd_impl(1, bits, dinv, vals, keep, goff, m_real, (cf)x, ids, n, r, din, h, (cf)wt_p, (cf)wt_z0, (cf)wt_z1, (cf)wt_r0,
                       (cf)wt_r1, (cf)wt_h0, (cf)wt_h1, (cf)xp, (cf)a, (cf)z, (cf)rr, (cf)rx, (cf)hh, g, (mf)dhp, (mf)dzp, (mf)drp,
                       (mf)dxp, (mf)da, dx, dw_p, dw_z0, dw_z1, dw_r0, dw_r1, dw_h0, dw_h1, db_z, db_r, db_h, db_z1, db_r1,
                       db_h1, drop_p, drop_seed, stream, nullptr, nullptr, nullptr, 0, nullptr, nullptr);
}

int gh::att_fwd_impl(const float* left, int nl, const int32_t* rowu, const float* right, const float* mask, const int32_t* goff,
                 const int32_t* rowg, int m_real, int b, int l, int xl, int dr, int ha, int heads, const float* w1, const float* w2,
                 float* u, float* t, float* e, float* weights, float* attended, hipStream_t s, int u_mode,
                 const void* right16, const void* w1_16) {
  GH_REQUIRE(heads >= 1 && heads <= 8, "concat_att: heads=%d not in [1,8]", heads);
  GH_REQUIRE(b > 0 && l > 0 && dr > 0 && ha > 0, "concat_att_fwd: bad sizes");
  GH_REQUIRE(u_mode >= 0 && u_mode <= 2, "concat_att_fwd: u_mode %d not in {0,1,2}", u_mode);
  GH_REQUIRE((goff == nullptr) == (rowg == nullptr), "concat_att_fwd: goff and rowg come together");
  if (!goff) m_real = b * l;
  GH_REQUIRE(m_real >= 0 && m_real <= b * l, "concat_att_fwd: node-compact rows %d do not fit b*l=%d", m_real, b * l);
  if (!rowu && u_mode != 1) nl = b;
  const int M = m_real;
  const bool one_block = ha <= Batch(false, M, s).bn;
  GH_REQUIRE(one_block || (ha % 4 == 0 && al16(t) && al16(u) && al16(w2)),
             "concat_att_fwd: attention hidden %d wider than one column block needs float4-shaped rows", ha);
  const int xl_in = (left && xl > 0) ? xl : 0;
  if (u_mode != 2) {
    if (left && xl > 0) {
      Batch bt(false, nl, s);
      bt.add(gemm_problem(nl, ha, EPI_STORE, u, ha, left, xl, w1, xl + dr, xl));
      bt.flush();
      GH_CHECK_HIP(bt.err);
    } else {
      GH_CHECK_HIP(hipMemsetAsync(u, 0, sizeof(float) * (size_t)nl * ha, s));
    }
  }
  if (u_mode == 1) return 0;
  if (!(left && xl > 0)) xl = 0;
  const int32_t* urow = rowu ? rowu : rowg;
  const float* e_parts = nullptr;
  int n_parts = 0;
  bool right_is16 = false;
  if (M > 0) {
    const bool use16 = right16 && w1_16 && g_gemm_mode == 1 && M >= 8192 && dr % 8 == 0 && (xl_in + dr) % 8 == 0 && xl_in % 8 == 0 && ha % 8 == 0;
    GH_REQUIRE(use16 || right, "concat_att_fwd: no fp32 right operand and the bf16 twins do not apply");
    right_is16 = use16;
    Batch bt(false, M, s, use16 && ha % 256 == 0);
    Problem p = use16 ? gemm_problem(M, ha, EPI_ATT, t, ha, (const float*)right16, dr,
                                     (const float*)((const unsigned short*)w1_16 + xl_in), xl_in + dr, dr, nullptr, 1)
                      : gemm_problem(M, ha, EPI_ATT, t, ha, right, dr, w1 + xl_in, xl_in + dr, dr);
    p.u = u; p.ldu = ha; p.R = l; p.w2 = w2; p.heads = heads; p.e = e; p.rowg = urow;
    bool blocks = false;
    if (!one_block) {
      const int nb = (ha + bt.bn - 1) / bt.bn;
      const Workspace wsp = workspace_for(s);
      const size_t need = (size_t)nb * (size_t)M * heads * sizeof(float);
      if (M >= 8192 && wsp.p && need <= wsp.bytes && ha % 4 == 0) {
        blocks = true;
        bt.e_block_stride = (long long)M * heads;
        p.e = wsp.p;
        e_parts = wsp.p; n_parts = nb;
      } else {
        p.epi = EPI_STORE;
      }
    }
    bt.add(p);
    bt.flush();
    GH_CHECK_HIP(bt.err);
    if (!one_block && !blocks) {
      FinishArgs F;
      F.n = 1; F.split = 0;
      F.it[0] = FinishItem{t, 0, 1, M, ha, EPI_ATT, 0, ha, t, nullptr, nullptr, nullptr, nullptr, nullptr, u, w2, e, ha, l, heads, urow};
      hipLaunchKernelGGL(nt_finish_kernel, dim3((M + 3) / 4, 1), dim3(256), 0, s, F);
      GH_LAUNCH_CHECK();
    }
  }
  return launch_att_softmax_fwd(e, mask, right, goff, m_real, b, l, dr, heads, weights, attended, s, e_parts, n_parts,
                                (long long)M * heads, right_is16 ? right16 : nullptr);
}

extern "C" int gh_concat_att_fwd(const float* left, const float* right, const float* mask, const int32_t* goff,
                                 const int32_t* rowg, int m_real, int b, int l, int xl,
                                 int dr, int ha, int heads, const float* w1, const float* w2,
                                 float* u, float* t, float* e, float* weights, float* attended,
                                 gh_stream_t stream) {
  return att_fwd_impl(left, b, nullptr, right, mask, goff, rowg, m_real, b, l, xl, dr, ha, heads, w1, w2, u, t, e, weights, attended,
                      (hipStream_t)stream);
}

int gh::att_bwd_impl(const float* left, const float* right, const int32_t* goff, int m_real, int b, int l,
                 int xl, int dr, int ha, int heads, const float* w1t, const float* w2, const float* t, const float* weights,
                 const float* g_att, const float* g_w, float* de, float* dpre, float* du,
                 float* dleft, float* dright, float* dw1, float* dw2,
                 const int32_t* claim_offsets, int nl, float* du_c, int dleft_accumulate, hipStream_t s,
                 const int32_t* rowg, float* dw_tmp, const GateFuse* next, int dleft_late, float* dw2_buf,
                 const void* right16, const void* w1t_16) {
  GH_REQUIRE(heads >= 1 && heads <= 8, "concat_att: heads=%d not in [1,8]", heads);
  if (!goff) m_real = b * l;
  GH_REQUIRE(m_real >= 0 && m_real <= b * l, "concat_att_bwd: node-compact rows %d do not fit b*l=%d", m_real, b * l);
  GH_REQUIRE((claim_offsets == nullptr) == (du_c == nullptr), "concat_att_bwd: claim_offsets and du_c come together");
  const int M = m_real;
  if (!left) xl = 0;
  if (!claim_offsets) nl = b;
  const float* dul = claim_offsets ? du_c : du;
  const int ldw = xl + dr;
  const bool weights_only = (dright == nullptr);
  GH_REQUIRE(!weights_only || dw1, "concat_att_bwd: dright == NULL asks for the dw1-only phase, which needs dw1");
  const bool use16 = right16 && w1t_16 && g_gemm_mode == 1 && m_real >= 8192 && dr % 8 == 0 && ha % 8 == 0 && xl % 8 == 0;
  void* const dpre16 = use16 ? (void*)dpre : nullptr;
  float* dw2_part = nullptr;
  if (!weights_only) {
  int dw_written = 0;
  if (int e = launch_att_softmax_bwd(right, weights, g_att, g_w, goff, m_real, b, l, dr, heads, de, dright, s, rowg, dw_tmp, &dw_written,
                                     use16 ? right16 : nullptr)) return e;
  const size_t dw2_bytes = (size_t)b * heads * ha * sizeof(float);
  const Workspace wsp = workspace_for(s);
  const bool late = dleft_late && dw2_buf && ha % 4 == 0;
  dw2_part = late ? dw2_buf : ((wsp.p && dw2_bytes <= wsp.bytes && ha % 4 == 0) ? wsp.p : nullptr);
  if (int e = launch_att_dpre(de, w2, t, goff, m_real, b, l, ha, heads, dpre, du, dw2_part, s, dw_written ? dw_tmp : nullptr,
                              dw_written ? weights : nullptr, dw_written ? de : nullptr, dpre16,
                              (long long)m_real * heads, dw_written > 1 ? dw_written : 1)) return e;
  if (dw2_part && !late) {
    ReduceArgs R;
    R.n = 1;
    R.it[0] = ReduceItem{dw2_part, dw2, heads, ha, ha, b, (long long)heads * ha};
    hipLaunchKernelGGL(reduce_partials_wave_kernel, dim3((heads * (ha / 4) + 3) / 4, 1), dim3(256), 0, s, R);
    GH_LAUNCH_CHECK();
  }
  if (claim_offsets && xl > 0 && !dleft_late)
    if (int e = gh_seg_sum(du, claim_offsets, du_c, nl, ha, (gh_stream_t)s)) return e;
  const float* w1t_r16 = use16 ? (const float*)((const unsigned short*)w1t_16 + (size_t)xl * ha) : nullptr;
  GH_REQUIRE(!next || !next->bf16 || use16, "concat_att_bwd: a bf16 gate head needs the bf16 twins of right and w1t");
  if (M > 0 && next) {
    Batch bt(false, M, s, use16 && dr % 256 == 0, 6, dr);
    Problem p = use16 ? gemm_problem(M, dr, EPI_GATE_PRE, next->dhp, dr, (const float*)dpre16, ha, w1t_r16, ha, ha, nullptr, 1)
                      : gemm_problem(M, dr, EPI_GATE_PRE, next->dhp, dr, dpre, ha, w1t + (size_t)xl * ha, ha, ha);
    p.gin = dright; p.in0 = next->z; p.in1 = next->hh; p.in2 = next->xp; p.out1 = next->dzp; p.out2 = next->dxp;
    p.io = next->bf16 ? (1 | 2 | 4 | 8 | 16 | 32) : 0;
    bt.add(p);
    bt.flush();
    GH_CHECK_HIP(bt.err);
  } else if (M > 0) {
    Batch bt(false, M, s, use16 && dr % 256 == 0);
    Problem p = use16 ? gemm_problem(M, dr, EPI_STORE, dright, dr, (const float*)dpre16, ha, w1t_r16, ha, ha, nullptr, 1)
                      : gemm_problem(M, dr, EPI_STORE, dright, dr, dpre, ha, w1t + (size_t)xl * ha, ha, ha);
    p.accumulate = 1;
    bt.add(p);
    bt.flush();
    GH_CHECK_HIP(bt.err);
  }
  if (xl > 0 && dleft && !dleft_late) {
    Batch bt(false, nl, s);
    Problem p = gemm_problem(nl, xl, EPI_STORE, dleft, xl, dul, ha, w1t, ha, ha);
    p.accumulate = dleft_accumulate ? 1 : 0;
    bt.add(p);
    bt.flush();
    GH_CHECK_HIP(bt.err);
  }
  if (!dw2_part && M > 0) {
    Batch bt(true, M, s);
    bt.add(tn_problem(heads, ha, dw2, ha, de, heads, t, ha, M));
    bt.flush();
    GH_CHECK_HIP(bt.err);
  }
  }
  if (weights_only && dleft_late) {
    if (dw2_buf && ha % 4 == 0) {
      ReduceArgs R;
      R.n = 1;
      R.it[0] = ReduceItem{dw2_buf, dw2, heads, ha, ha, b, (long long)heads * ha};
      hipLaunchKernelGGL(reduce_partials_wave_kernel, dim3((heads * (ha / 4) + 3) / 4, 1), dim3(256), 0, s, R);
      GH_LAUNCH_CHECK();
    }
    if (claim_offsets && xl > 0)
      if (int e = gh_seg_sum(du, claim_offsets, du_c, nl, ha, (gh_stream_t)s)) return e;
  }
  if (weights_only && dleft_late && xl > 0 && dleft) {
    Batch bt(false, nl, s);
    Problem p = gemm_problem(nl, xl, EPI_STORE, dleft, xl, dul, ha, w1t, ha, ha);
    p.accumulate = dleft_accumulate ? 1 : 0;
    bt.add(p);
    bt.flush();
    GH_CHECK_HIP(bt.err);
  }
  if (!dw1) return 0;
  if (M > 0) {
    Batch bt(true, M, s);
    if (use16) bt.add(tn_problem(ha, dr, dw1 + xl, ldw, (const float*)dpre16, ha, (const float*)right16, dr, M, nullptr, 1));
    else bt.add(tn_problem(ha, dr, dw1 + xl, ldw, dpre, ha, right, dr, M));
    bt.flush();
    GH_CHECK_HIP(bt.err);
  }
  if (xl > 0) {
    Batch bt(true, nl, s);
    bt.add(tn_problem(ha, xl, dw1, ldw, dul, ha, left, xl, nl));
    bt.flush();
    GH_CHECK_HIP(bt.err);
  }
  return 0;
}

extern "C" int gh_concat_att_bwd(const float* left, const float* right, const int32_t* goff, int m_real, int b, int l,
                                 int xl, int dr, int ha, int heads, const float* w1t, const float* w2, const float* t, const float* weights,
                                 const float* g_att, const float* g_w, float* de, float* dpre, float* du,
                                 float* dleft, float* dright, float* dw1, float* dw2, gh_stream_t stream) {
  return att_bwd_impl(left, right, goff, m_real, b, l, xl, dr, ha, heads, w1t, w2, t, weights, g_att, g_w, de, dpre, du, dleft, dright,
                      dw1, dw2, nullptr, b, nullptr, 0, (hipStream_t)stream, nullptr, nullptr, nullptr);
}

int gh::linear2_fwd(const float* x0, int k0, const float* x1, int k1, const float* w, const float* bias, float* y, int m, int n, hipStream_t s,
                    const float* w_out, const float* b_out, float* y_out, int n_out) {
  Batch b(false, m, s);
  Problem p = gemm_problem(m, n, EPI_STORE, y, n, x0, k0, w, k0 + k1, k0);
  if (k1 > 0) add_seg(p, x1, k1, w + k0, k0 + k1, k1);
  p.bias = bias;
  const bool two = w_out && y_out && n_out >= 1;
  const bool fuse = two && n_out <= 8 && n % 4 == 0 && n <= b.bn && al16(w_out);
  if (fuse) { p.w2 = w_out; p.e = y_out; p.heads = n_out; p.in0 = b_out; }
  b.add(p);
  b.flush();
  GH_CHECK_HIP(b.err);
  if (two && !(fuse && b.split_done)) return launch_tiny_linear_fwd(y, w_out, b_out, y_out, m, n, n_out, s);
  return 0;
}
int gh::linear2_bwd(const float* x0, int k0, const float* x1, int k1, const float* wt, const float* g, int m, int n,
                float* dx0, int dx0_accumulate, float* dx1, float* dw, float* db, hipStream_t s) {
  if (dx0 || dx1) {
    Batch b(false, m, s);
    if (dx0) { Problem p = gemm_problem(m, k0, EPI_STORE, dx0, k0, g, n, wt, n, n); p.accumulate = dx0_accumulate ? 1 : 0; b.add(p); }
    if (dx1 && k1 > 0) b.add(gemm_problem(m, k1, EPI_STORE, dx1, k1, g, n, wt + (size_t)k0 * n, n, n));
    b.flush();
    GH_CHECK_HIP(b.err);
  }
  if (dw) {
    Batch b(true, m, s);
    b.add(tn_problem(n, k0, dw, k0 + k1, g, n, x0, k0, m));
    if (k1 > 0) b.add(tn_problem(n, k1, dw + k0, k0 + k1, g, n, x1, k1, m));
    b.flush();
    GH_CHECK_HIP(b.err);
  }
  if (db) return launch_colsum(g, db, m, n, s);
  return 0;
}

extern "C" int gh_set_gemm_mode(int mode) {
  GH_REQUIRE(mode >= 0 && mode <= 3, "set_gemm_mode: %d is not 0 (fp32), 1 (bf16 operands in the big NT/NN GEMMs), 2 (fp32x3) or 3 (fp32x3, pre-split weights)", mode);
  g_gemm_mode = mode;
  return 0;
}

extern "C" int gh_weights_changed(void) {
  std::lock_guard<std::mutex> lk(g_x3_mu);
  ++g_x3_epoch;
  return 0;
}

extern "C" int gh_fp32x3_refresh(gh_stream_t stream) {
  std::lock_guard<std::mutex> lk(g_x3_mu);
  if (g_x3.empty()) return 0;
  std::vector<X3Item> items;
  items.reserve(g_x3.size());
  for (auto& kv : g_x3) {
    items.push_back(X3Item{(const float*)kv.first.b, kv.second.img, kv.first.N, kv.first.ldb, kv.first.K, kv.second.pitch});
    kv.second.epoch = g_x3_epoch;
  }
  x3p_split(items.data(), (int)items.size(), (hipStream_t)stream);
  GH_CHECK_HIP(hipGetLastError());
  return 0;
}

extern "C" int gh_fp32x3_clear(void) {
  std::lock_guard<std::mutex> lk(g_x3_mu);
  if (g_x3.empty()) return 0;
  GH_CHECK_HIP(hipDeviceSynchronize());
  for (auto& kv : g_x3) g_x3_pool.emplace((size_t)kv.first.N * kv.second.pitch + 256, kv.second.img);
  g_x3.clear();
  if (g_x3_pool.size() > 2048) {
    for (auto& kv : g_x3_pool) (void)hipFree(kv.second);
    g_x3_pool.clear();
  }
  return 0;
}

extern "C" int gh_gemm_path_counters(int64_t* out_host, int reset) {
  if (out_host)
    for (int i = 0; i < 3; ++i) out_host[i] = g_path_counts[i];
  if (reset) g_path_counts[0] = g_path_counts[1] = g_path_counts[2] = 0;
  return 0;
}

extern "C" int gh_set_workspace(void* ptr, int64_t bytes) {
  std::lock_guard<std::mutex> lk(g_ws_mu);
  g_ws_default = make_workspace(ptr, bytes);
  return 0;
}

extern "C" int gh_set_stream_workspace(gh_stream_t stream, void* ptr, int64_t bytes) {
  std::lock_guard<std::mutex> lk(g_ws_mu);
  const WsKey key{current_device(), (hipStream_t)stream};
  if (!ptr) g_ws_stream.erase(key);
  else g_ws_stream[key] = make_workspace(ptr, bytes);
  return 0;
}

extern "C" int gh_linear_fwd(const float* x, const float* w, const float* bias, float* y, int m, int k, int n,
                             gh_stream_t stream) {
  hipStream_t s = (hipStream_t)stream;
  GH_REQUIRE(m > 0 && k > 0 && n > 0, "linear_fwd: bad sizes");
  if (n <= 8) return launch_tiny_linear_fwd(x, w, bias, y, m, k, n, s);
  Batch b(false, m, s);
  Problem p = gemm_problem(m, n, EPI_STORE, y, n, x, k, w, k, k);
  p.bias = bias;
  b.add(p);
  b.flush();
  GH_CHECK_HIP(b.err);
  return 0;
}

#ifdef GH_MEASURE
extern "C" int gh_debug_nt_phases(unsigned long long* out, int reset) {
  if (out && hipMemcpyFromSymbol(out, HIP_SYMBOL(g_nt_phase), 64 * sizeof(unsigned long long)) != hipSuccess) return 1;
  if (reset) { void* p = nullptr; if (hipGetSymbolAddress(&p, HIP_SYMBOL(g_nt_phase)) != hipSuccess || hipMemset(p, 0, 64 * sizeof(unsigned long long)) != hipSuccess) return 1; }
  return 0;
}
#endif

extern "C" int gh_linear_wgrad_bf16(const void* g16, int ldg, const void* x16, int ldx, int m, int n, int k,
                                    float* dw, int lddw, float* db, gh_stream_t stream) {
  hipStream_t s = (hipStream_t)stream;
  GH_REQUIRE(m > 0 && k > 0 && n > 0 && g16 && x16 && dw, "linear_wgrad_bf16: bad arguments");
  GH_REQUIRE(n % 8 == 0 && k % 8 == 0 && ldg % 8 == 0 && ldx % 8 == 0 && ldg >= n && ldx >= k && lddw >= k && lddw % 4 == 0,
             "linear_wgrad_bf16: widths and leading dimensions must be multiples of 8 (lddw: of 4)");
  GH_REQUIRE(((reinterpret_cast<uintptr_t>(g16) | reinterpret_cast<uintptr_t>(x16) | reinterpret_cast<uintptr_t>(dw)) & 15) == 0,
             "linear_wgrad_bf16: operands must be 16-byte aligned");
  Batch b(true, m, s);
  GH_REQUIRE(b.g_ws != nullptr, "linear_wgrad_bf16: needs the split-K workspace (gh_set_workspace)");
  b.add(tn_problem(n, k, dw, lddw, (const float*)g16, ldg, (const float*)x16, ldx, m, nullptr, 1));
  if (db) b.want_colsum(db, nullptr);
  b.flush();
  GH_CHECK_HIP(b.err);
  GH_REQUIRE(!db || (b.colsum_fused && !b.colsum_missed), "linear_wgrad_bf16: the bias gradient did not fit the split-K workspace");
  return 0;
}

extern "C" int gh_linear_bwd(const float* x, const float* wt, const float* w, const float* g, int m, int k, int n, float* dx,
                             float* dw, float* db, gh_stream_t stream) {
  hipStream_t s = (hipStream_t)stream;
  GH_REQUIRE(m > 0 && k > 0 && n > 0, "linear_bwd: bad sizes");
  if (n <= 8 && w) return launch_tiny_linear_bwd(x, w, g, dx, dw, db, m, k, n, s);
  if (dx) {
    Batch b(false, m, s);
    b.add(gemm_problem(m, k, EPI_STORE, dx, k, g, n, wt, n, n));
    b.flush();
    GH_CHECK_HIP(b.err);
  }
  if (dw) {
    Batch b(true, m, s);
    b.add(tn_problem(n, k, dw, k, g, n, x, k, m));
    b.flush();
    GH_CHECK_HIP(b.err);
  }
  if (db) return launch_colsum(g, db, m, n, s);
  return 0;
}
```

### get_amd/csrc/model_ops.hip

```cpp
#include "../../include/get_hip.h"
#include "common.h"
#include <mutex>
#include <unordered_map>

namespace gh {

struct Dims {
  int B, B1, L, R, n, D, H, hw, he, C, cs, as, Xl, Xa, Dre, E, W;
  bool compact;
  int Mr, Mt, M1, Mq;
  bool bf;
  bool att16;
  bool fuse_scorer;
};
struct CellBuf { int64_t xp, a, z, rr, rx, hh, out, out32, xdrop; };
struct FwdBuf {
  int64_t offsets, pair2claim, has, lens_eff, rowc, maskf_p;
  CellBuf q, c1, c2;
  int64_t q_repr, score_x, score, keep;
  int64_t uw, tw, ew, ww, avg, new_left;
  int64_t right_e, mask_e, ue, te, ee, we, att_e, y0, phi;
  int64_t total;
  int64_t obs_total;
};
struct BwdBuf {
  int64_t d_y0, d_new_left, d_att_e, de_e, dpre_e, du_e, dright_e, d_avg;
  int64_t de_w, dw_w, dpre_w, du_w, du_c, d_q, g2, d_qhid, qs[5], sc2[5], sc1[5], dx2, dw2p_e, dw2p_w, dw_e;
  int64_t total;
};
struct Bump {
  int64_t off = 0;
  int64_t take(int64_t nfloats) { const int64_t o = off; off += (nfloats + 63) & ~(int64_t)63; return o; }
};

static int make_dims(const gh_get_model* Mo, const gh_get_batch* Ba, Dims& d) {
  GH_REQUIRE(Mo && Ba, "get: NULL model / batch descriptor");
  d.B = Ba->b; d.B1 = Ba->b1; d.L = Ba->l; d.R = Ba->r; d.n = Ba->n_max;
  d.D = Mo->d; d.H = Mo->h; d.hw = Mo->word_heads; d.he = Mo->evd_heads; d.C = Mo->n_classes;
  d.cs = Mo->claim_src_dim; d.as = Mo->article_src_dim;
  GH_REQUIRE(d.B > 0 && d.B1 > 0 && d.L > 0 && d.R > 0 && d.n > 0, "get: bad batch sizes b=%d b1=%d l=%d r=%d n_max=%d", d.B, d.B1, d.L, d.R, d.n);
  GH_REQUIRE(d.R <= 256 && d.L <= 256, "get: padded graph sizes above 256 nodes are not supported (l=%d r=%d)", d.L, d.R);
  GH_REQUIRE(d.D % 4 == 0 && d.H % 4 == 0 && d.D >= 4 && d.D <= d.H && d.H <= 1024,
             "get: the composite path needs float4-shaped widths with d <= h <= 1024 (d=%d h=%d); use the per-module entry points", d.D, d.H);
  GH_REQUIRE(Mo->storage == 0 || Mo->storage == 1, "get: model->storage %d not in {0 (fp32), 1 (bf16 storage in the evidence cells)}", Mo->storage);
  GH_REQUIRE(d.hw >= 1 && d.hw <= 8 && d.he >= 1 && d.he <= 8, "get: heads %d / %d not in [1,8]", d.hw, d.he);
  GH_REQUIRE(Ba->k_keep >= 0 && Ba->k_keep <= d.R, "get: k_keep=%d not in [0, r=%d]", Ba->k_keep, d.R);
  GH_REQUIRE(d.C >= 1 && d.cs >= 0 && d.as >= 0 && d.cs % 4 == 0 && d.as % 4 == 0, "get: bad class / source widths (%d, %d, %d)", d.C, d.cs, d.as);
  d.Xl = d.H + d.cs; d.Xa = d.H * d.hw; d.Dre = d.Xa + d.as; d.E = d.Xl + d.Dre * d.he; d.W = words_for(d.R);
  d.compact = Ba->m_real >= 0;
  d.Mt = d.B1 * d.R;
  if (d.compact) {
    GH_REQUIRE(Ba->goff && Ba->rowg && Ba->cids && Ba->maskf, "get: the node-compact layout needs goff, rowg, cids and maskf");
    GH_REQUIRE(Ba->m_real > 0 && Ba->m_real <= d.Mt, "get: m_real=%d does not fit b1*r=%d", Ba->m_real, d.Mt);
    d.Mr = Ba->m_real;
    d.M1 = Ba->collapsed ? (d.Mr + 1 < d.Mt ? d.Mr + 1 : d.Mt) : d.Mt;
    GH_REQUIRE(!(Ba->collapsed && Ba->drop_gnn > 0.f), "get: collapsed padding rows are an evaluation-mode layout (no dropout)");
  } else {
    d.Mr = d.Mt; d.M1 = d.Mt;
  }
  d.Mq = d.B * d.L;
  d.fuse_scorer = d.H <= 320;
  d.bf = Mo->storage == 1 && d.D % 8 == 0 && d.H % 8 == 0 && d.Mr >= 8192;
  if (d.bf) {
    const gh_cell_bf16* cs[2] = {&Mo->cell1_16, &Mo->cell2_16};
    for (const gh_cell_bf16* c : cs)
      GH_REQUIRE(c->w_p && c->w_z0 && c->w_z1 && c->w_r0 && c->w_r1 && c->w_h0 && c->w_h1,
                 "get: storage = 1 needs the bf16 twins of both evidence cells' weights (gh_weights_refresh)");
    GH_REQUIRE(Mo->embedding16, "get: storage = 1 needs the bf16 copy of the word table (embedding16)");
  }
  d.att16 = d.bf && gemm_mode() == 1 && Mo->att_word_w1_16 && Mo->att_word_w1t_16 && d.Mr >= 8192 && d.H % 8 == 0;
  return 0;
}

static void cell_buf(Bump& b, CellBuf& c, int64_t rows, int H, bool bf = false, bool need32 = true, int64_t drop_din = 0) {
  c.xdrop = (bf && drop_din > 0) ? b.take(rows * drop_din / 2) : -1;
  const int64_t e = bf ? rows * H / 2 : rows * H;
  c.xp = b.take(e); c.a = b.take(e); c.z = b.take(e); c.rr = b.take(e);
  c.rx = b.take(e); c.hh = b.take(e); c.out = b.take(e);
  c.out32 = bf ? (need32 ? b.take(rows * H) : -1) : c.out;
}

static int layout(const gh_get_model* Mo, const gh_get_batch* Ba, Dims& d, FwdBuf& f, BwdBuf& w) {
  if (int e = make_dims(Mo, Ba, d)) return e;
  Bump b;
  f.offsets = b.take(d.B + 1); f.pair2claim = b.take(d.B1); f.has = b.take(d.B); f.lens_eff = b.take(d.B);
  f.rowc = b.take(d.Mr);
  f.maskf_p = d.compact ? -1 : b.take(d.Mt);
  {
    Bump o;
    f.phi = o.take((int64_t)d.B * d.C);
    f.ww = o.take((int64_t)d.Mr * d.hw);
    f.we = o.take((int64_t)d.B * d.n * d.he);
    f.score = o.take((int64_t)d.B1 * d.R);
    f.keep = o.take((int64_t)d.B1 * d.W * 2);
    f.obs_total = o.off;
  }
  cell_buf(b, f.q, d.Mq, d.H);
  f.q_repr = b.take((int64_t)d.B * d.H);
  const bool pre_drop = d.bf && Ba->drop_gnn > 0.f;
  cell_buf(b, f.c1, d.M1, d.H, d.bf, !d.bf, pre_drop ? d.D : 0);
  f.score_x = b.take((int64_t)d.M1 * ((d.fuse_scorer || !d.bf) ? 1 : 8));
  cell_buf(b, f.c2, d.Mr, d.H, d.bf, !d.att16, pre_drop ? d.H : 0);
  f.uw = b.take((int64_t)d.B * d.H); f.tw = b.take((int64_t)d.Mr * d.H); f.ew = b.take((int64_t)d.Mr * d.hw);
  f.avg = b.take((int64_t)d.B1 * d.Xa);
  f.new_left = d.cs > 0 ? b.take((int64_t)d.B * d.Xl) : f.q_repr;
  f.right_e = b.take((int64_t)d.B * d.n * d.Dre); f.mask_e = b.take((int64_t)d.B * d.n);
  f.ue = b.take((int64_t)d.B * d.H); f.te = b.take((int64_t)d.B * d.n * d.H); f.ee = b.take((int64_t)d.B * d.n * d.he);
  f.att_e = b.take((int64_t)d.B * d.Dre * d.he);
  f.y0 = b.take((int64_t)d.B * d.H);
  f.total = b.off;
  Bump c;
  w.d_y0 = c.take((int64_t)d.B * d.H); w.d_new_left = c.take((int64_t)d.B * d.Xl); w.d_att_e = c.take((int64_t)d.B * d.Dre * d.he);
  w.de_e = c.take((int64_t)d.B * d.n * d.he); w.dpre_e = c.take((int64_t)d.B * d.n * d.H); w.du_e = c.take((int64_t)d.B * d.H);
  w.dright_e = c.take((int64_t)d.B * d.n * d.Dre);
  w.d_avg = c.take((int64_t)d.B1 * d.Xa);
  w.de_w = c.take((int64_t)d.Mr * d.hw); w.dw_w = c.take((int64_t)((d.H + 511) / 512) * d.Mr * d.hw);
  w.dw_e = c.take((int64_t)((d.Dre + 511) / 512) * d.B * d.n * d.he); w.dpre_w = c.take((int64_t)d.Mr * d.H); w.du_w = c.take((int64_t)d.B1 * d.H);
  w.du_c = c.take((int64_t)d.B * d.H);
  w.d_q = d.cs > 0 ? c.take((int64_t)d.B * d.H) : w.d_new_left;
  w.g2 = c.take((int64_t)d.Mr * d.H);
  w.d_qhid = c.take((int64_t)d.Mq * d.H);
  for (int i = 0; i < 5; ++i) w.qs[i] = c.take((int64_t)d.Mq * d.H);
  const int64_t se = d.bf ? (int64_t)d.Mr * d.H / 2 : (int64_t)d.Mr * d.H;
  for (int i = 0; i < 5; ++i) w.sc2[i] = c.take(se);
  for (int i = 0; i < 5; ++i) w.sc1[i] = c.take(se);
  w.dx2 = d.bf ? c.take((int64_t)d.Mr * d.H) : w.g2;
  w.dw2p_e = c.take((int64_t)d.B * d.he * d.H); w.dw2p_w = c.take((int64_t)d.B1 * d.hw * d.H);
  w.total = c.off;
  return 0;
}

struct DevEvents { hipEvent_t ev[12]; };
static std::mutex g_ev_mu;
static std::unordered_map<int, DevEvents> g_events;
static int get_events(DevEvents& out) {
  int dev = 0;
  GH_CHECK_HIP(hipGetDevice(&dev));
  std::lock_guard<std::mutex> lk(g_ev_mu);
  auto it = g_events.find(dev);
  if (it == g_events.end()) {
    DevEvents e;
    for (int i = 0; i < 12; ++i) GH_CHECK_HIP(hipEventCreateWithFlags(&e.ev[i], hipEventDisableTiming));
    it = g_events.emplace(dev, e).first;
  }
  out = it->second;
  return 0;
}
static int stream_after(hipStream_t to, hipStream_t from, hipEvent_t ev) {
  if (to == from) return 0;
  GH_CHECK_HIP(hipEventRecord(ev, from));
  GH_CHECK_HIP(hipStreamWaitEvent(to, ev, 0));
  return 0;
}

__global__ void __launch_bounds__(256)
rows_prep_kernel(const int32_t* __restrict__ pair2claim, const int32_t* __restrict__ rowg, int R, int Mr,
                 int32_t* __restrict__ rowc, const int32_t* __restrict__ d_ids, float* __restrict__ maskf_p,
                 const void* __restrict__ q_lens, int kind, const float* __restrict__ has, float* __restrict__ lens_eff, int B) {
  const int i = blockIdx.x * blockDim.x + threadIdx.x;
  if (i < Mr) {
    const int pair = rowg ? rowg[i] : i / R;
    rowc[i] = pair2claim[pair];
    if (maskf_p) maskf_p[i] = d_ids[i] >= 1 ? 1.f : 0.f;
  }
  if (i < B) {
    float len;
    if (kind == 0) len = reinterpret_cast<const float*>(q_lens)[i];
    else if (kind == 1) len = (float)reinterpret_cast<const int32_t*>(q_lens)[i];
    else len = (float)reinterpret_cast<const int64_t*>(q_lens)[i];
    lens_eff[i] = has[i] > 0.f ? len : INFINITY;
  }
}

template <typename TL>
__global__ void __launch_bounds__(256)
seg_rows_kernel(const int64_t* __restrict__ counts, int B, int b1, const int32_t* __restrict__ rowg, int R, int Mr,
                int32_t* __restrict__ offsets, int32_t* __restrict__ pair2claim, float* __restrict__ has, int32_t* __restrict__ rowc,
                const int32_t* __restrict__ d_ids, float* __restrict__ maskf_p, const TL* __restrict__ q_lens, float* __restrict__ lens_eff) {
  __shared__ int off[1025];
  const int tid = threadIdx.x;
  int c[4], sum = 0;
#pragma unroll
  for (int k = 0; k < 4; ++k) { const int b = 4 * tid + k; c[k] = b < B ? (int)counts[b] : 0; sum += c[k]; }
  __shared__ int part[256];
  part[tid] = sum;
  __syncthreads();
  for (int o = 1; o < 256; o <<= 1) {
    const int v = tid >= o ? part[tid - o] : 0;
    __syncthreads();
    part[tid] += v;
    __syncthreads();
  }
  int run = part[tid] - sum;
#pragma unroll
  for (int k = 0; k < 4; ++k) { const int b = 4 * tid + k; if (b < B) off[b] = run; run += c[k]; }
  if (tid == 255) off[B] = part[255];
  __syncthreads();
  const int total = off[B];
  if (blockIdx.x == 0) {
    for (int b = tid; b <= B; b += 256) offsets[b] = off[b];
    for (int b = tid; b < B; b += 256) {
      const float hb = counts[b] > 0 ? 1.f : 0.f;
      has[b] = hb;
      lens_eff[b] = hb > 0.f ? (float)q_lens[b] : INFINITY;
    }
  }
  auto claim_of = [&](int p) {
    if (p >= total) return 0;
    int lo = 0, hi = B - 1;
    while (lo < hi) { const int mid = (lo + hi + 1) >> 1; if (off[mid] <= p) lo = mid; else hi = mid - 1; }
    return lo;
  };
  const int i = blockIdx.x * 256 + tid;
  if (i < b1) pair2claim[i] = claim_of(i);
  if (i < Mr) {
    const int pair = rowg ? rowg[i] : i / R;
    rowc[i] = claim_of(pair);
    if (maskf_p) maskf_p[i] = d_ids[i] >= 1 ? 1.f : 0.f;
  }
}

template <typename TS>
__global__ void __launch_bounds__(256)
left_assemble_fwd_kernel(const float* __restrict__ table, const TS* __restrict__ src, const float* __restrict__ q_repr,
                         const float* __restrict__ has, float* __restrict__ new_left, int cs, int H, int rows,
                         unsigned int* __restrict__ clamped) {
  const int b = blockIdx.x;
  const float hb = has[b];
  const long long sb = (long long)src[b];
  if ((sb < 0 || sb >= rows) && threadIdx.x == 0) atomicAdd(clamped + 1, 1u);
  const float* tp = table + (size_t)(sb < 0 ? 0 : (sb >= rows ? rows - 1 : sb)) * cs;
  float* o = new_left + (size_t)b * (cs + H);
  for (int i = threadIdx.x; i < cs; i += blockDim.x) o[i] = tp[i] * hb;
  for (int i = threadIdx.x; i < H; i += blockDim.x) o[cs + i] = q_repr[(size_t)b * H + i];
}
template <typename TS>
__global__ void __launch_bounds__(256)
left_assemble_bwd_kernel(const float* __restrict__ d_new_left, const TS* __restrict__ src, const float* __restrict__ has,
                         float* __restrict__ d_q, float* __restrict__ d_table, int B, int cs, int H, int rows) {
  for (int i = threadIdx.x; i < B * H; i += blockDim.x) {
    const int b = i / H, c = i - b * H;
    d_q[i] = d_new_left[(size_t)b * (cs + H) + cs + c];
  }
  if (!d_table) return;
  for (int c = threadIdx.x; c < cs; c += blockDim.x)
    for (int b = 0; b < B; ++b) {
      const long long sb = (long long)src[b];
      d_table[(size_t)(sb < 0 ? 0 : (sb >= rows ? rows - 1 : sb)) * cs + c] += d_new_left[(size_t)b * (cs + H) + c] * has[b];
    }
}

__global__ void __launch_bounds__(256)
cross_entropy_kernel(const float* __restrict__ phi, const int64_t* __restrict__ labels, int B, int C, float* __restrict__ loss,
                     float* __restrict__ dphi, unsigned int* __restrict__ clamped) {
  __shared__ float part[256];
  float acc = 0.f;
  const float invb = 1.f / (float)B;
  for (int b = threadIdx.x; b < B; b += blockDim.x) {
    const float* p = phi + (size_t)b * C;
    float mx = p[0];
    for (int c = 1; c < C; ++c) mx = fmaxf(mx, p[c]);
    float se = 0.f;
    for (int c = 0; c < C; ++c) se += expf(p[c] - mx);
    const float lse = mx + logf(se);
    const long long yl = labels[b];
    const int y = yl < 0 ? 0 : (yl >= C ? C - 1 : (int)yl);
    if (yl < 0 || yl >= C) atomicAdd(clamped, 1u);
    acc += lse - p[y];
    for (int c = 0; c < C; ++c) dphi[(size_t)b * C + c] = (expf(p[c] - lse) - (c == y ? 1.f : 0.f)) * invb;
  }
  part[threadIdx.x] = acc;
  __syncthreads();
  for (int o = 128; o > 0; o >>= 1) {
    if ((int)threadIdx.x < o) part[threadIdx.x] += part[threadIdx.x + o];
    __syncthreads();
  }
  if (threadIdx.x == 0) loss[0] = part[0] * invb;
}

__global__ void __launch_bounds__(256)
document_scatter_kernel(const int32_t* __restrict__ d_ids, const int64_t* __restrict__ slot, int32_t* __restrict__ document, int R) {
  const int g = blockIdx.x;
  const size_t dst = (size_t)slot[g] * R;
  for (int j = threadIdx.x; j < R; j += blockDim.x) document[dst + j] = d_ids[(size_t)g * R + j];
}

}

using namespace gh;

extern "C" int gh_get_plan_buffers(const gh_get_model* Mo, const gh_get_batch* Ba, gh_get_plan* P) {
  GH_REQUIRE(P, "get_plan_buffers: NULL plan");
  Dims d; FwdBuf f; BwdBuf w;
  if (int e = layout(Mo, Ba, d, f, w)) return e;
  P->fwd_floats = f.total; P->bwd_floats = w.total; P->obs_floats = f.obs_total;
  P->phi = f.phi; P->word_w = f.ww; P->evd_w = f.we; P->score = f.score; P->keep = f.keep;
  return 0;
}

extern "C" int gh_get_struct_sizes(int64_t* out) {
  GH_REQUIRE(out, "get_struct_sizes: NULL");
  out[0] = sizeof(gh_get_model); out[1] = sizeof(gh_get_batch); out[2] = sizeof(gh_get_plan); out[3] = sizeof(gh_cell_params);
  out[4] = sizeof(gh_cell_bf16);
  return 0;
}

#define GH_TRY(expr) do { if (int _rc = (expr)) return _rc; } while (0)

static inline const int32_t* I32(const float* A, int64_t off) { return reinterpret_cast<const int32_t*>(A + off); }
static inline int32_t* I32(float* A, int64_t off) { return reinterpret_cast<int32_t*>(A + off); }

static int cell_fwd(const gh_cell_params& c, const gh_cell_bf16* c16, const CellBuf& cb, float* A, const uint64_t* bits, const float* dinv,
                    const float* vals, const uint64_t* keep, const int32_t* goff, int m_real, int m_rows, const float* x, const int32_t* ids,
                    int n, int r, int din, int h, float drop_p, uint32_t seed, const float* score_w, float* score_x, float sdrop,
                    uint32_t sseed, hipStream_t s, int pad_out_dead = 0, int* score_parts = nullptr) {
  typedef const float* cf;
  if (c16)
    return cell_fwd_impl(1, cb.out32 >= 0 ? A + cb.out32 : nullptr, bits, dinv, vals, keep, goff, m_real, m_rows, x, ids, n, r, din, h, (cf)c16->w_p, (cf)c16->w_z0,
                         (cf)c16->w_z1, (cf)c16->w_r0, (cf)c16->w_r1, (cf)c16->w_h0, (cf)c16->w_h1, c.b_z0, c.b_z1, c.b_r0, c.b_r1, c.b_h0,
                         c.b_h1, A + cb.xp, A + cb.a, A + cb.z, A + cb.rr, A + cb.rx, A + cb.hh, A + cb.out, drop_p, seed, score_w, score_x,
                         sdrop, sseed, (void*)s, 0, score_parts, cb.xdrop >= 0 ? A + cb.xdrop : nullptr);
  return cell_fwd_impl(0, nullptr, bits, dinv, vals, keep, goff, m_real, m_rows, x, ids, n, r, din, h, c.w_p, c.w_z0, c.w_z1, c.w_r0,
                       c.w_r1, c.w_h0, c.w_h1, c.b_z0, c.b_z1, c.b_r0, c.b_r1, c.b_h0, c.b_h1, A + cb.xp, A + cb.a, A + cb.z,
                       A + cb.rr, A + cb.rx, A + cb.hh, A + cb.out, drop_p, seed, score_w, score_x, sdrop, sseed, (void*)s, pad_out_dead);
}
static int cell_bwd(const gh_cell_params& c, const gh_cell_bf16* c16, const CellBuf& cb, const float* A, const uint64_t* bits, const float* dinv,
                    const float* vals, const uint64_t* keep, const int32_t* goff, int m_real, const float* x, const int32_t* ids, int n,
                    int r, int din, int h, const float* g, float* W, const int64_t* sc, float* dx, float drop_p, uint32_t seed,
                    hipStream_t s, int pre_done = 0, const GateFuse* next = nullptr) {
  GH_REQUIRE(c.dw_p && c.db_z0 && c.db_z1, "get_backward: a cell's gradient outputs are missing");
  if (c16) {
    typedef const float* cf;
    GH_REQUIRE(c16->wt_p && c16->wt_z0 && c16->wt_z1 && c16->wt_r0 && c16->wt_r1 && c16->wt_h0 && c16->wt_h1,
               "get_backward: storage = 1 needs the bf16 twins of the cells' transposed weights (gh_weights_refresh)");
    return cell_bwd_impl(1, bits, dinv, vals, keep, goff, m_real, x, ids, n, r, din, h, (cf)c16->wt_p, (cf)c16->wt_z0, (cf)c16->wt_z1,
                         (cf)c16->wt_r0, (cf)c16->wt_r1, (cf)c16->wt_h0, (cf)c16->wt_h1, A + cb.xp, A + cb.a, A + cb.z, A + cb.rr,
                         A + cb.rx, A + cb.hh, g, W + sc[0], W + sc[1], W + sc[2], W + sc[3], W + sc[4], dx, c.dw_p, c.dw_z0, c.dw_z1,
                         c.dw_r0, c.dw_r1, c.dw_h0, c.dw_h1, c.db_z0, c.db_r0, c.db_h0, c.db_z1, c.db_r1, c.db_h1, drop_p, seed, (void*)s,
                         nullptr, nullptr, nullptr, pre_done, next, cb.xdrop >= 0 ? A + cb.xdrop : nullptr);
  }
  GH_REQUIRE(c.wt_p, "get_backward: a cell's transposes are missing");
  return cell_bwd_impl(0, bits, dinv, vals, keep, goff, m_real, x, ids, n, r, din, h, c.wt_p, c.wt_z0, c.wt_z1, c.wt_r0, c.wt_r1,
                       c.wt_h0, c.wt_h1, A + cb.xp, A + cb.a, A + cb.z, A + cb.rr, A + cb.rx, A + cb.hh, g, W + sc[0], W + sc[1],
                       W + sc[2], W + sc[3], W + sc[4], dx, c.dw_p, c.dw_z0, c.dw_z1, c.dw_r0, c.dw_r1, c.dw_h0, c.dw_h1, c.db_z0,
                       c.db_r0, c.db_h0, c.db_z1, c.db_r1, c.db_h1, drop_p, seed, (void*)s, nullptr, nullptr, nullptr, pre_done, next);
}

extern "C" int gh_get_forward(const gh_get_model* Mo, const gh_get_batch* Ba, float* A, float* O, gh_stream_t stream, gh_stream_t side_stream) {
  Dims d; FwdBuf f; BwdBuf w;
  GH_TRY(layout(Mo, Ba, d, f, w));
  GH_REQUIRE(A && (reinterpret_cast<uintptr_t>(A) & 255) == 0, "get_forward: the arena must be 256-byte aligned");
  GH_REQUIRE(O && (reinterpret_cast<uintptr_t>(O) & 255) == 0, "get_forward: the observables buffer must be 256-byte aligned");
  GH_REQUIRE(Ba->q_ids && Ba->q_lens && Ba->q_bits && (Ba->q_dinv || Ba->q_vals) && Ba->d_ids && Ba->d_bits && (Ba->d_dinv || Ba->d_vals) &&
             Ba->counts && Ba->document, "get_forward: a batch tensor is missing (ids, lens, packed graphs, counts, document)");
  GH_REQUIRE(Ba->q_lens_kind >= 0 && Ba->q_lens_kind <= 2, "get_forward: q_lens_kind %d not in {0,1,2}", Ba->q_lens_kind);
  GH_REQUIRE(d.as == 0 || Ba->doc_sources, "get_forward: article-source ids are missing");
  GH_REQUIRE(d.cs == 0 || Ba->query_sources, "get_forward: claim-source ids are missing");
  GH_REQUIRE(Mo->embedding && Mo->scorer_w && Mo->scorer_gate && Mo->out0_w && Mo->out1_w, "get_forward: missing model tensors");
  GH_REQUIRE((d.cs == 0) == (Mo->claim_src_table == nullptr) && (d.as == 0) == (Mo->article_src_table == nullptr),
             "get_forward: source tables and their widths must come together");
  GH_REQUIRE(d.cs == 0 || Mo->claim_src_rows > 0, "get_forward: claim_src_rows must give the claim-source table's row count");
  GH_REQUIRE(d.as == 0 || Mo->article_src_rows > 0, "get_forward: article_src_rows must give the article-source table's row count");
  GH_REQUIRE(Ba->drop_claim >= 0.f && Ba->drop_claim < 1.f && Ba->drop_gnn >= 0.f && Ba->drop_gnn < 1.f, "get_forward: dropout p not in [0,1)");
  hipStream_t s = (hipStream_t)stream, ss = side_stream ? (hipStream_t)side_stream : s;
  DevEvents ev;
  GH_TRY(get_events(ev));
  const int H = d.H;
  if (d.B <= 1024) {
    const int nthr = d.Mr > d.B1 ? d.Mr : d.B1;
    const dim3 grid((nthr + 255) / 256);
    const int32_t* rg = d.compact ? Ba->rowg : nullptr;
    float* mp = d.compact ? nullptr : A + f.maskf_p;
    if (Ba->q_lens_kind == 0)
      hipLaunchKernelGGL(seg_rows_kernel<float>, grid, dim3(256), 0, s, Ba->counts, d.B, d.B1, rg, d.R, d.Mr, I32(A, f.offsets), I32(A, f.pair2claim),
                         A + f.has, I32(A, f.rowc), Ba->d_ids, mp, (const float*)Ba->q_lens, A + f.lens_eff);
    else if (Ba->q_lens_kind == 1)
      hipLaunchKernelGGL(seg_rows_kernel<int32_t>, grid, dim3(256), 0, s, Ba->counts, d.B, d.B1, rg, d.R, d.Mr, I32(A, f.offsets), I32(A, f.pair2claim),
                         A + f.has, I32(A, f.rowc), Ba->d_ids, mp, (const int32_t*)Ba->q_lens, A + f.lens_eff);
    else
      hipLaunchKernelGGL(seg_rows_kernel<int64_t>, grid, dim3(256), 0, s, Ba->counts, d.B, d.B1, rg, d.R, d.Mr, I32(A, f.offsets), I32(A, f.pair2claim),
                         A + f.has, I32(A, f.rowc), Ba->d_ids, mp, (const int64_t*)Ba->q_lens, A + f.lens_eff);
    GH_LAUNCH_CHECK();
  } else {
  GH_TRY(gh_seg_offsets(Ba->counts, d.B, I32(A, f.offsets), I32(A, f.pair2claim), d.B1, A + f.has, (void*)s));
  {
    const int nthr = d.Mr > d.B ? d.Mr : d.B;
    hipLaunchKernelGGL(rows_prep_kernel, dim3((nthr + 255) / 256), dim3(256), 0, s, I32(A, f.pair2claim), d.compact ? Ba->rowg : nullptr, d.R,
                       d.Mr, I32(A, f.rowc), Ba->d_ids, d.compact ? nullptr : A + f.maskf_p, Ba->q_lens, Ba->q_lens_kind, A + f.has,
                       A + f.lens_eff, d.B);
    GH_LAUNCH_CHECK();
  }
  }
  GH_TRY(stream_after(ss, s, ev.ev[0]));
  GH_TRY(cell_fwd(Mo->claim, nullptr, f.q, A, Ba->q_bits, Ba->q_dinv, Ba->q_vals, nullptr, nullptr, 0, 0, Mo->embedding, Ba->q_ids, d.B, d.L,
                  d.D, H, Ba->drop_claim, Ba->seed_claim, nullptr, nullptr, 0.f, 0, ss));
  GH_TRY(gh_masked_mean_fwd(A + f.q.out, Ba->q_ids, A + f.lens_eff, A + f.q_repr, d.B, d.L, H, (void*)ss));
  if (d.cs > 0) {
    unsigned int* cl = clamp_counter();
    GH_REQUIRE(cl, "get_forward: cannot allocate the clamp counter");
    if (Ba->query_sources_i64)
      hipLaunchKernelGGL(left_assemble_fwd_kernel<int64_t>, dim3(d.B), dim3(256), 0, ss, Mo->claim_src_table, (const int64_t*)Ba->query_sources,
                         A + f.q_repr, A + f.has, A + f.new_left, d.cs, H, Mo->claim_src_rows, cl);
    else
      hipLaunchKernelGGL(left_assemble_fwd_kernel<int32_t>, dim3(d.B), dim3(256), 0, ss, Mo->claim_src_table, (const int32_t*)Ba->query_sources,
                         A + f.q_repr, A + f.has, A + f.new_left, d.cs, H, Mo->claim_src_rows, cl);
    GH_LAUNCH_CHECK();
  }
  GH_TRY(att_fwd_impl(A + f.q_repr, d.B, nullptr, nullptr, nullptr, nullptr, nullptr, 0, d.B1, d.R, H, H, H, d.hw, Mo->att_word.w1,
                      Mo->att_word.w2, A + f.uw, nullptr, nullptr, nullptr, nullptr, ss, 1));
  GH_TRY(att_fwd_impl(A + f.new_left, d.B, nullptr, nullptr, nullptr, nullptr, nullptr, 0, d.B, d.n, d.Xl, d.Dre, H, d.he, Mo->att_evd.w1,
                      Mo->att_evd.w2, A + f.ue, nullptr, nullptr, nullptr, nullptr, ss, 1));
  const int32_t* goff = d.compact ? Ba->goff : nullptr;
  const int32_t* ids1 = d.compact ? Ba->cids : Ba->d_ids;
  const gh_cell_bf16* c16_1 = d.bf ? &Mo->cell1_16 : nullptr;
  const gh_cell_bf16* c16_2 = d.bf ? &Mo->cell2_16 : nullptr;
  const float* table1 = d.bf ? (const float*)Mo->embedding16 : Mo->embedding;
  uint64_t* keep = reinterpret_cast<uint64_t*>(O + f.keep);
  if (d.fuse_scorer) {
    GH_TRY(cell_fwd(Mo->cell1, c16_1, f.c1, A, Ba->d_bits, Ba->d_dinv, Ba->d_vals, nullptr, goff, d.Mr, d.M1, table1, ids1, d.B1, d.R, d.D, H,
                    Ba->drop_gnn, Ba->seed_cell1, Mo->scorer_w, A + f.score_x, Ba->drop_gnn, Ba->seed_scorer, s, 1));
    GH_TRY(gh_scorer_gsl(Ba->d_bits, Ba->d_dinv, Ba->d_vals, goff, (d.compact && Ba->collapsed) ? 1 : 0, nullptr, A + f.score_x, Mo->scorer_w,
                         Mo->scorer_gate, d.B1, d.R, H, Ba->k_keep, O + f.score, keep, 0.f, 0, (void*)s));
  } else if (d.bf) {
    GH_REQUIRE((H + 127) / 128 <= 8, "get_forward: hidden width %d needs more than the 8 scorer-partial slots", H);
    int parts = 1;
    GH_TRY(cell_fwd(Mo->cell1, c16_1, f.c1, A, Ba->d_bits, Ba->d_dinv, Ba->d_vals, nullptr, goff, d.Mr, d.M1, table1, ids1, d.B1, d.R, d.D, H,
                    Ba->drop_gnn, Ba->seed_cell1, Mo->scorer_w, A + f.score_x, Ba->drop_gnn, Ba->seed_scorer, s, 0, &parts));
    GH_REQUIRE(parts >= 1 && parts <= 8, "get_forward: internal -- %d scorer partials", parts);
    GH_TRY(scorer_gsl_impl(Ba->d_bits, Ba->d_dinv, Ba->d_vals, goff, (d.compact && Ba->collapsed) ? 1 : 0, nullptr, A + f.score_x, parts, d.M1,
                           Mo->scorer_w, Mo->scorer_gate, d.B1, d.R, H, Ba->k_keep, O + f.score, keep, 0.f, 0, s));
  } else {
    GH_TRY(cell_fwd(Mo->cell1, c16_1, f.c1, A, Ba->d_bits, Ba->d_dinv, Ba->d_vals, nullptr, goff, d.Mr, d.M1, table1, ids1, d.B1, d.R, d.D, H,
                    Ba->drop_gnn, Ba->seed_cell1, nullptr, nullptr, 0.f, 0, s, 0));
    GH_TRY(gh_scorer_gsl(Ba->d_bits, Ba->d_dinv, Ba->d_vals, goff, (d.compact && Ba->collapsed) ? 1 : 0, A + f.c1.out32, nullptr, Mo->scorer_w,
                         Mo->scorer_gate, d.B1, d.R, H, Ba->k_keep, O + f.score, keep, Ba->drop_gnn, Ba->seed_scorer, (void*)s));
  }
  GH_TRY(cell_fwd(Mo->cell2, c16_2, f.c2, A, Ba->d_bits, Ba->d_dinv, Ba->d_vals, keep, goff, d.Mr, d.Mr, A + f.c1.out, nullptr, d.B1, d.R, H, H,
                  Ba->drop_gnn, Ba->seed_cell2, nullptr, nullptr, 0.f, 0, s));
  GH_TRY(stream_after(s, ss, ev.ev[1]));
  GH_TRY(att_fwd_impl(A + f.q_repr, d.B, I32(A, f.rowc), f.c2.out32 >= 0 ? A + f.c2.out32 : nullptr, d.compact ? Ba->maskf : A + f.maskf_p, goff,
                      d.compact ? Ba->rowg : nullptr, d.Mr, d.B1, d.R, H, H, H, d.hw, Mo->att_word.w1, Mo->att_word.w2, A + f.uw, A + f.tw,
                      A + f.ew, O + f.ww, A + f.avg, s, 2, d.bf ? (const void*)(A + f.c2.out) : nullptr, d.bf ? Mo->att_word_w1_16 : nullptr));
  GH_TRY(gh_evd_assemble_fwd(A + f.avg, I32(A, f.offsets), Mo->article_src_table, Mo->article_src_rows, d.as > 0 ? Ba->doc_sources : nullptr, Ba->doc_sources_i64,
                             Ba->document, Ba->document_i64, d.B, d.n, d.Xa, d.as, d.R, A + f.right_e, A + f.mask_e, (void*)s));
  GH_TRY(att_fwd_impl(A + f.new_left, d.B, nullptr, A + f.right_e, A + f.mask_e, nullptr, nullptr, 0, d.B, d.n, d.Xl, d.Dre, H, d.he,
                      Mo->att_evd.w1, Mo->att_evd.w2, A + f.ue, A + f.te, A + f.ee, O + f.we, A + f.att_e, s, 2));
  if (d.C <= 8) {
    GH_TRY(linear2_fwd(A + f.new_left, d.Xl, A + f.att_e, d.Dre * d.he, Mo->out0_w, Mo->out0_b, A + f.y0, d.B, H, s, Mo->out1_w, Mo->out1_b,
                       O + f.phi, d.C));
  } else {
    GH_TRY(linear2_fwd(A + f.new_left, d.Xl, A + f.att_e, d.Dre * d.he, Mo->out0_w, Mo->out0_b, A + f.y0, d.B, H, s));
    GH_TRY(gh_linear_fwd(A + f.y0, Mo->out1_w, Mo->out1_b, O + f.phi, d.B, H, d.C, (void*)s));
  }
  return 0;
}

extern "C" int gh_get_backward(const gh_get_model* Mo, const gh_get_batch* Ba, const float* A, const float* O, float* Wb, const float* g_phi,
                               const float* g_word_w, const float* g_evd_w, int phase, gh_stream_t stream, gh_stream_t side_stream) {
  Dims d; FwdBuf f; BwdBuf w;
  GH_TRY(layout(Mo, Ba, d, f, w));
  GH_REQUIRE(phase >= 0 && phase <= 2, "get_backward: phase %d not in {0,1,2}", phase);
  GH_REQUIRE(A && O && Wb && g_phi, "get_backward: NULL arena / observables / gradient");
  GH_REQUIRE(Mo->out0_wt && Mo->out1_wt && Mo->att_word.w1t && Mo->att_evd.w1t && Mo->d_out0_w && Mo->d_out0_b && Mo->d_out1_w &&
             Mo->d_out1_b && Mo->att_word.dw1 && Mo->att_word.dw2 && Mo->att_evd.dw1 && Mo->att_evd.dw2,
             "get_backward: transposes / gradient outputs of the attention layers or the head are missing");
  hipStream_t s = (hipStream_t)stream, ss = side_stream ? (hipStream_t)side_stream : s;
  DevEvents ev;
  GH_TRY(get_events(ev));
  const int H = d.H;
  const int32_t* goff = d.compact ? Ba->goff : nullptr;
  const int32_t* ids1 = d.compact ? Ba->cids : Ba->d_ids;
  const uint64_t* keep = reinterpret_cast<const uint64_t*>(O + f.keep);
  const GateFuse gf2 = {A + f.c2.z, A + f.c2.hh, A + f.c2.xp, Wb + w.sc2[0], Wb + w.sc2[1], Wb + w.sc2[3], d.bf ? 1 : 0};
  const GateFuse gf1 = {A + f.c1.z, A + f.c1.hh, A + f.c1.xp, Wb + w.sc1[0], Wb + w.sc1[1], Wb + w.sc1[3], d.bf ? 1 : 0};
  const bool fuse_gate = !d.bf || (Mo->att_word_w1t_16 != nullptr);
  const void* att_r16 = d.bf ? (const void*)(A + f.c2.out) : nullptr;
  const void* att_w1t16 = d.bf ? Mo->att_word_w1t_16 : nullptr;
  const gh_cell_bf16* c16_1 = d.bf ? &Mo->cell1_16 : nullptr;
  const gh_cell_bf16* c16_2 = d.bf ? &Mo->cell2_16 : nullptr;
  const float* table1 = d.bf ? (const float*)Mo->embedding16 : Mo->embedding;
  if (phase != 2) {
    if (d.C <= 8 && H % 4 == 0 && Mo->out0_w && Mo->out1_w && head_bwd_lds(d.B, H, d.C, d.E, Mo->out0_w) > 0) {
      GH_TRY(launch_head_bwd(g_phi, A + f.y0, Mo->out1_w, Mo->out0_w, d.B, H, d.C, d.Xl, d.E, Wb + w.d_y0, Mo->d_out1_w, Mo->d_out1_b,
                             Wb + w.d_new_left, 0, Wb + w.d_att_e, s));
    } else {
      GH_TRY(gh_linear_bwd(A + f.y0, Mo->out1_wt, Mo->out1_w, g_phi, d.B, H, d.C, Wb + w.d_y0, Mo->d_out1_w, Mo->d_out1_b, (void*)s));
      GH_TRY(linear2_bwd(A + f.new_left, d.Xl, A + f.att_e, d.Dre * d.he, Mo->out0_wt, Wb + w.d_y0, d.B, H, Wb + w.d_new_left, 0,
                         Wb + w.d_att_e, nullptr, nullptr, s));
    }
    GH_TRY(stream_after(ss, s, ev.ev[2]));
    GH_TRY(linear2_bwd(A + f.new_left, d.Xl, A + f.att_e, d.Dre * d.he, Mo->out0_wt, Wb + w.d_y0, d.B, H, nullptr, 0, nullptr,
                       Mo->d_out0_w, Mo->d_out0_b, ss));
    GH_TRY(att_bwd_impl(A + f.new_left, A + f.right_e, nullptr, 0, d.B, d.n, d.Xl, d.Dre, H, d.he, Mo->att_evd.w1t, Mo->att_evd.w2, A + f.te,
                        O + f.we, Wb + w.d_att_e, g_evd_w, Wb + w.de_e, Wb + w.dpre_e, Wb + w.du_e, Wb + w.d_new_left, Wb + w.dright_e,
                        nullptr, Mo->att_evd.dw2, nullptr, d.B, nullptr, 1, s, nullptr, (d.Dre + 511) / 512 <= 16 ? Wb + w.dw_e : nullptr, nullptr, 1,
                        Wb + w.dw2p_e));
    GH_TRY(stream_after(ss, s, ev.ev[3]));
    GH_TRY(att_bwd_impl(A + f.new_left, A + f.right_e, nullptr, 0, d.B, d.n, d.Xl, d.Dre, H, d.he, Mo->att_evd.w1t, Mo->att_evd.w2, A + f.te,
                        O + f.we, Wb + w.d_att_e, g_evd_w, Wb + w.de_e, Wb + w.dpre_e, Wb + w.du_e, Wb + w.d_new_left, nullptr, Mo->att_evd.dw1,
                        Mo->att_evd.dw2, nullptr, d.B, nullptr, 1, ss, nullptr, nullptr, nullptr, 1, Wb + w.dw2p_e));
    if (d.cs > 0) {
      if (Ba->query_sources_i64)
        hipLaunchKernelGGL(left_assemble_bwd_kernel<int64_t>, dim3(1), dim3(256), 0, ss, Wb + w.d_new_left, (const int64_t*)Ba->query_sources,
                           A + f.has, Wb + w.d_q, Mo->d_claim_src_table, d.B, d.cs, H, Mo->claim_src_rows);
      else
        hipLaunchKernelGGL(left_assemble_bwd_kernel<int32_t>, dim3(1), dim3(256), 0, ss, Wb + w.d_new_left, (const int32_t*)Ba->query_sources,
                           A + f.has, Wb + w.d_q, Mo->d_claim_src_table, d.B, d.cs, H, Mo->claim_src_rows);
      GH_LAUNCH_CHECK();
    }
    GH_TRY(gh_evd_assemble_bwd(Wb + w.dright_e, I32(A, f.offsets), d.as > 0 ? Ba->doc_sources : nullptr, Ba->doc_sources_i64, Mo->article_src_rows, d.B, d.n, d.Xa,
                               d.as, Wb + w.d_avg, d.as > 0 ? Mo->d_article_src_table : nullptr, (void*)s));
    GH_TRY(att_bwd_impl(A + f.q_repr, f.c2.out32 >= 0 ? A + f.c2.out32 : nullptr, goff, d.Mr, d.B1, d.R, H, H, H, d.hw, Mo->att_word.w1t, Mo->att_word.w2, A + f.tw,
                        O + f.ww, Wb + w.d_avg, g_word_w, Wb + w.de_w, Wb + w.dpre_w, Wb + w.du_w, Wb + w.d_q, Wb + w.g2, nullptr,
                        Mo->att_word.dw2, I32(A, f.offsets), d.B, Wb + w.du_c, 1, s, d.compact ? Ba->rowg : nullptr, Wb + w.dw_w,
                        fuse_gate ? &gf2 : nullptr, 1, Wb + w.dw2p_w, att_r16, att_w1t16));
    GH_TRY(stream_after(ss, s, ev.ev[4]));
    GH_TRY(att_bwd_impl(A + f.q_repr, f.c2.out32 >= 0 ? A + f.c2.out32 : nullptr, goff, d.Mr, d.B1, d.R, H, H, H, d.hw, Mo->att_word.w1t, Mo->att_word.w2, A + f.tw,
                        O + f.ww, Wb + w.d_avg, g_word_w, Wb + w.de_w, Wb + w.dpre_w, Wb + w.du_w, Wb + w.d_q, nullptr, Mo->att_word.dw1,
                        Mo->att_word.dw2, I32(A, f.offsets), d.B, Wb + w.du_c, 1, ss, nullptr, nullptr, nullptr, 1, Wb + w.dw2p_w, att_r16,
                        att_w1t16));
    GH_TRY(gh_masked_mean_bwd(Wb + w.d_q, Ba->q_ids, A + f.lens_eff, Wb + w.d_qhid, d.B, d.L, H, (void*)ss));
    GH_TRY(cell_bwd(Mo->claim, nullptr, f.q, A, Ba->q_bits, Ba->q_dinv, Ba->q_vals, nullptr, nullptr, 0, Mo->embedding, Ba->q_ids, d.B, d.L, d.D, H,
                    Wb + w.d_qhid, Wb, w.qs, nullptr, Ba->drop_claim, Ba->seed_claim, ss));
    if (fuse_gate)
      GH_TRY(cell_bwd(Mo->cell2, c16_2, f.c2, A, Ba->d_bits, Ba->d_dinv, Ba->d_vals, keep, goff, d.Mr, A + f.c1.out, nullptr, d.B1, d.R, H, H,
                      Wb + w.g2, Wb, w.sc2, nullptr, Ba->drop_gnn, Ba->seed_cell2, s, 1, &gf1));
    else
      GH_TRY(cell_bwd(Mo->cell2, c16_2, f.c2, A, Ba->d_bits, Ba->d_dinv, Ba->d_vals, keep, goff, d.Mr, A + f.c1.out, nullptr, d.B1, d.R, H, H,
                      Wb + w.g2, Wb, w.sc2, Wb + w.dx2, Ba->drop_gnn, Ba->seed_cell2, s, 0, nullptr));
  }
  if (phase != 1) {
    if (fuse_gate)
      GH_TRY(cell_bwd(Mo->cell1, c16_1, f.c1, A, Ba->d_bits, Ba->d_dinv, Ba->d_vals, nullptr, goff, d.Mr, table1, ids1, d.B1, d.R, d.D, H,
                      nullptr, Wb, w.sc1, nullptr, Ba->drop_gnn, Ba->seed_cell1, s, 1, nullptr));
    else
      GH_TRY(cell_bwd(Mo->cell1, c16_1, f.c1, A, Ba->d_bits, Ba->d_dinv, Ba->d_vals, nullptr, goff, d.Mr, table1, ids1, d.B1, d.R, d.D, H,
                      Wb + w.dx2, Wb, w.sc1, nullptr, Ba->drop_gnn, Ba->seed_cell1, s, 0, nullptr));
    GH_TRY(stream_after(s, ss, ev.ev[5]));
  }
  return 0;
}

extern "C" int gh_cross_entropy(const float* phi, const int64_t* labels, int b, int c, float* loss, float* dphi, gh_stream_t stream) {
  GH_REQUIRE(b > 0 && c > 0 && phi && labels && loss && dphi, "cross_entropy: bad arguments");
  unsigned int* cl = clamp_counter();
  GH_REQUIRE(cl, "cross_entropy: cannot allocate the clamp counter");
  hipLaunchKernelGGL(cross_entropy_kernel, dim3(1), dim3(256), 0, (hipStream_t)stream, phi, labels, b, c, loss, dphi, cl);
  GH_LAUNCH_CHECK();
  return 0;
}

extern "C" int gh_get_prepare(const int32_t* claim_tokens, const int32_t* claim_len, int b, int l,
                              const int32_t* evd_tokens, const int32_t* evd_len, int b1, int r, int window,
                              int32_t* q_ids, int32_t* q_n, uint64_t* q_bits, float* q_dinv,
                              int32_t* d_ids, int32_t* d_n, uint64_t* d_bits, float* d_dinv,
                              int m_real, int32_t* goff, int32_t* rowg, int32_t* src, int32_t* cids, float* maskf,
                              const int64_t* slot, int32_t* document, gh_stream_t stream) {
  if (b > 0 && b1 > 0) {
    GH_TRY(launch_graph_build2(claim_tokens, claim_len, b, l, q_ids, q_n, q_bits, q_dinv, evd_tokens, evd_len, b1, r, d_ids, d_n, d_bits,
                               d_dinv, window, (hipStream_t)stream));
  } else {
    GH_TRY(gh_graph_build(claim_tokens, claim_len, b, l, window, q_ids, q_n, q_bits, q_dinv, stream));
    GH_TRY(gh_graph_build(evd_tokens, evd_len, b1, r, window, d_ids, d_n, d_bits, d_dinv, stream));
  }
  bool scattered = false;
  if (m_real >= 0 && b1 > 0) {
    GH_TRY(launch_ragged_plan(d_n, d_ids, b1, r, goff, rowg, src, cids, maskf, slot, document, (hipStream_t)stream, &scattered));
  }
  if (slot && document && b1 > 0 && !scattered) {
    hipLaunchKernelGGL(document_scatter_kernel, dim3(b1), dim3(256), 0, (hipStream_t)stream, d_ids, slot, document, r);
    GH_LAUNCH_CHECK();
  }
  return 0;
}
```

### get_amd/fused.py

```python
from __future__ import annotations

import ctypes
import os
import weakref

import torch

from . import _lib, ops
from .keywords import KeyWordSettings as K
from .ops import PackedAdj

ENABLED = os.environ.get("GET_AMD_FUSED", "1") != "0"

_P, _I, _F, _U, _L = ctypes.c_void_p, ctypes.c_int, ctypes.c_float, ctypes.c_uint32, ctypes.c_int64

_CELL_W = ["w_p", "w_z0", "w_z1", "w_r0", "w_r1", "w_h0", "w_h1"]
_CELL_B = ["b_z0", "b_z1", "b_r0", "b_r1", "b_h0", "b_h1"]


class CellParams(ctypes.Structure):
    _fields_ = ([(n, _P) for n in _CELL_W] + [(n, _P) for n in _CELL_B] + [("wt" + n[1:], _P) for n in _CELL_W] +
                [("d" + n, _P) for n in _CELL_W] + [("d" + n, _P) for n in _CELL_B])


class CellBf16(ctypes.Structure):
    _fields_ = [(n, _P) for n in _CELL_W] + [("wt" + n[1:], _P) for n in _CELL_W]


class AttParams(ctypes.Structure):
    _fields_ = [("w1", _P), ("w2", _P), ("w1t", _P), ("dw1", _P), ("dw2", _P)]


class GetModel(ctypes.Structure):
    _fields_ = [("d", _I), ("h", _I), ("word_heads", _I), ("evd_heads", _I), ("n_classes", _I),
                ("claim_src_dim", _I), ("article_src_dim", _I), ("claim_src_rows", _I), ("article_src_rows", _I),
                ("embedding", _P),
                ("claim", CellParams), ("cell1", CellParams), ("cell2", CellParams),
                ("scorer_w", _P), ("scorer_gate", _P),
                ("att_word", AttParams), ("att_evd", AttParams),
                ("claim_src_table", _P), ("article_src_table", _P),
                ("d_claim_src_table", _P), ("d_article_src_table", _P),
                ("out0_w", _P), ("out0_b", _P), ("out0_wt", _P),
                ("out1_w", _P), ("out1_b", _P), ("out1_wt", _P),
                ("d_out0_w", _P), ("d_out0_b", _P), ("d_out1_w", _P), ("d_out1_b", _P),
                ("storage", _I), ("embedding16", _P), ("cell1_16", CellBf16), ("cell2_16", CellBf16),
                ("att_word_w1_16", _P), ("att_word_w1t_16", _P)]


class GetBatch(ctypes.Structure):
    _fields_ = [("b", _I), ("b1", _I), ("l", _I), ("r", _I), ("n_max", _I),
                ("m_real", _I), ("collapsed", _I), ("k_keep", _I),
                ("q_ids", _P), ("q_lens", _P), ("q_lens_kind", _I),
                ("q_bits", _P), ("q_dinv", _P), ("q_vals", _P),
                ("d_ids", _P), ("d_bits", _P), ("d_dinv", _P), ("d_vals", _P),
                ("goff", _P), ("rowg", _P), ("cids", _P), ("maskf", _P),
                ("counts", _P), ("counts_fit", _I),
                ("doc_sources", _P), ("doc_sources_i64", _I),
                ("query_sources", _P), ("query_sources_i64", _I),
                ("document", _P), ("document_i64", _I),
                ("drop_claim", _F), ("drop_gnn", _F),
                ("seed_claim", _U), ("seed_cell1", _U), ("seed_scorer", _U), ("seed_cell2", _U)]


class GetPlan(ctypes.Structure):
    _fields_ = [("fwd_floats", _L), ("bwd_floats", _L), ("obs_floats", _L), ("phi", _L), ("word_w", _L), ("evd_w", _L), ("score", _L),
                ("keep", _L)]


def _cell_tensors(cell):
    g = lambda m: m.linear
    ws = [cell.proj.linear.weight, g(cell.linearz0).weight, g(cell.linearz1).weight, g(cell.linearr0).weight,
          g(cell.linearr1).weight, g(cell.linearh0).weight, g(cell.linearh1).weight]
    bs = [g(cell.linearz0).bias, g(cell.linearz1).bias, g(cell.linearr0).bias, g(cell.linearr1).bias,
          g(cell.linearh0).bias, g(cell.linearh1).bias]
    return ws, bs


class Binding:

    def __init__(self, model):
        self._model = weakref.ref(model)
        gw = model.ggnn_with_gsl
        self.cells = [model.ggnn4claim_1, gw.feat_prop1, gw.feat_prop2]
        self.params = []
        self.mats = []
        for c in self.cells:
            ws, bs = _cell_tensors(c)
            self.params += ws + bs
            self.mats += ws
        aw, ae = model.self_att_word, model.self_att_evd
        self.params += [aw.linear1.weight, aw.linear2.weight, ae.linear1.weight, ae.linear2.weight]
        self.mats += [aw.linear1.weight, ae.linear1.weight]
        self.params += [model.out[0].weight, model.out[0].bias, model.out[1].weight, model.out[1].bias]
        self.mats += [model.out[0].weight, model.out[1].weight]
        self.tables = []
        if model.use_claim_source:
            self.tables.append(model.claim_source_embs.weight)
        if model.use_article_source:
            self.tables.append(model.article_source_embs.weight)
        self.struct = {False: None, True: None}
        self._sig = {False: None, True: None}
        self._mat_ids = [id(m) for m in self.mats]
        self._checked = False
        self.pool = _ArenaPool()

    @property
    def model(self):
        return self._model()

    def eligible(self) -> bool:
        m = self.model
        d = m.embedding.weight.shape[1]
        h = m.hidden_size
        cs = m.claim_emb_size if m.use_claim_source else 0
        as_ = m.article_emb_size if m.use_article_source else 0
        return (not m.embedding.weight.requires_grad and d % 4 == 0 and h % 4 == 0 and 4 <= d <= h <= 1024 and
                1 <= m.num_att_heads_for_words <= 8 and 1 <= m.num_att_heads_for_evds <= 8 and cs % 4 == 0 and as_ % 4 == 0 and
                m.ggnn4claim_1.proj.linear.weight.shape == (h, d) and m.out[1].weight.shape[1] == h and
                all(p.dtype == torch.float32 and p.is_contiguous() for p in self.params))

    def get(self, need_grads: bool):
        if not self._checked:
            sz = (ctypes.c_int64 * 5)()
            _lib.call("gh_get_struct_sizes", ctypes.cast(sz, ctypes.c_void_p))
            mine = (ctypes.sizeof(GetModel), ctypes.sizeof(GetBatch), ctypes.sizeof(GetPlan), ctypes.sizeof(CellParams),
                    ctypes.sizeof(CellBf16))
            if tuple(sz) != mine:
                raise RuntimeError(f"get_amd: struct layout mismatch between fused.py {mine} and libget_hip.so {tuple(sz)}")
            self._checked = True
        m = self.model
        direct = need_grads and all(ops._direct(p) for p in self.params) and all((not t.requires_grad) or ops._direct(t) for t in self.tables)
        wts = [ops.transposed(w) for w in self.mats] if need_grads else None
        gscorer = m.ggnn_with_gsl._gate12()
        bf = _lib.gemm_mode() == "bf16" and S_bf16_shapes(m)
        twins = emb16 = None
        if bf:
            twins = [[ops.bf16_twins(w) for w in _cell_tensors(c)[0]] for c in self.cells[1:]]
            twins.append([ops.bf16_twins(m.self_att_word.linear1.weight)])
            emb = m.embedding.weight
            emb16 = ops.derived("table_bf16", (emb,), lambda: emb.detach().to(torch.bfloat16), frozen=not emb.requires_grad)
        sig = (tuple(p.data_ptr() for p in self.params), tuple(t.data_ptr() for t in self.tables),
               (emb16.data_ptr(), tuple(t.data_ptr() for cell in twins for pair in cell for t in pair)) if bf else None,
               tuple(t.data_ptr() for t in wts) if wts else None,
               tuple(p.grad.data_ptr() for p in self.params) if direct else None,
               tuple((t.grad.data_ptr() if t.requires_grad else 0) for t in self.tables) if direct else None,
               m.embedding.weight.data_ptr(), gscorer.data_ptr(), m.ggnn_with_gsl.word_scorer1.proj.linear.weight.data_ptr())
        gbuf = views = None
        if need_grads and not direct:
            sizes = [(p.numel() + 63) // 64 * 64 for p in self.params] + [(t.numel() + 63) // 64 * 64 for t in self.tables]
            gbuf = torch.zeros(sum(sizes), device=self.params[0].device, dtype=torch.float32)
            views, off = {}, 0
            for t, sz in zip(self.params + self.tables, sizes):
                views[id(t)] = gbuf[off:off + t.numel()].view_as(t)
                off += sz
        if self.struct[need_grads] is not None and sig == self._sig[need_grads] and gbuf is None:
            return self.struct[need_grads], direct, None, None
        S = GetModel()
        S.d, S.h = m.embedding.weight.shape[1], m.hidden_size
        S.word_heads, S.evd_heads, S.n_classes = m.num_att_heads_for_words, m.num_att_heads_for_evds, m.out[1].weight.shape[0]
        S.claim_src_dim = m.claim_emb_size if m.use_claim_source else 0
        S.article_src_dim = m.article_emb_size if m.use_article_source else 0
        S.claim_src_rows = m.claim_source_embs.weight.shape[0] if m.use_claim_source else 0
        S.article_src_rows = m.article_source_embs.weight.shape[0] if m.use_article_source else 0
        S.embedding = m.embedding.weight.data_ptr()
        S.storage = 1 if bf else 0
        if bf:
            S.embedding16 = emb16.data_ptr()
            S.att_word_w1_16, S.att_word_w1t_16 = twins[2][0][0].data_ptr(), twins[2][0][1].data_ptr()
            for c16, cell in zip((S.cell1_16, S.cell2_16), twins[:2]):
                for name, (w16, wt16) in zip(_CELL_W, cell):
                    setattr(c16, name, w16.data_ptr())
                    setattr(c16, "wt" + name[1:], wt16.data_ptr())
        gptr = None
        if need_grads:
            gl = [p.grad for p in self.params] if direct else [views[id(p)] for p in self.params]
            gptr = [g.data_ptr() for g in gl]
        wt_of = {i: t.data_ptr() for i, t in zip(self._mat_ids, wts)} if wts else {}
        k = 0
        for cs_, cell in zip((S.claim, S.cell1, S.cell2), self.cells):
            ws, bs = _cell_tensors(cell)
            for name, t in zip(_CELL_W, ws):
                setattr(cs_, name, t.data_ptr())
                if need_grads:
                    setattr(cs_, "wt" + name[1:], wt_of[id(t)])
                    setattr(cs_, "d" + name, gptr[k])
                k += 1
            for name, t in zip(_CELL_B, bs):
                setattr(cs_, name, t.data_ptr())
                if need_grads:
                    setattr(cs_, "d" + name, gptr[k])
                k += 1
        S.scorer_w = m.ggnn_with_gsl.word_scorer1.proj.linear.weight.data_ptr()
        S.scorer_gate = gscorer.data_ptr()
        self._keep_alive = (gscorer, wts, twins, emb16)
        for a_, att in zip((S.att_word, S.att_evd), (m.self_att_word, m.self_att_evd)):
            a_.w1, a_.w2 = att.linear1.weight.data_ptr(), att.linear2.weight.data_ptr()
            if need_grads:
                a_.w1t = wt_of[id(att.linear1.weight)]
                a_.dw1, a_.dw2 = gptr[k], gptr[k + 1]
            k += 2
        S.out0_w, S.out0_b = m.out[0].weight.data_ptr(), m.out[0].bias.data_ptr()
        S.out1_w, S.out1_b = m.out[1].weight.data_ptr(), m.out[1].bias.data_ptr()
        if need_grads:
            S.out0_wt, S.out1_wt = wt_of[id(m.out[0].weight)], wt_of[id(m.out[1].weight)]
            S.d_out0_w, S.d_out0_b, S.d_out1_w, S.d_out1_b = gptr[k], gptr[k + 1], gptr[k + 2], gptr[k + 3]
        k += 4
        for use, fld, tab in ((m.use_claim_source, "claim_src_table", getattr(m, "claim_source_embs", None)),
                              (m.use_article_source, "article_src_table", getattr(m, "article_source_embs", None))):
            if not use:
                continue
            w = tab.weight
            setattr(S, fld, w.data_ptr())
            if need_grads and w.requires_grad:
                setattr(S, "d_" + fld, w.grad.data_ptr() if direct else views[id(w)].data_ptr())
        if gbuf is None:
            self.struct[need_grads], self._sig[need_grads] = S, sig
        return S, direct, gbuf, views


def S_bf16_shapes(m) -> bool:
    return m.embedding.weight.shape[1] % 8 == 0 and m.hidden_size % 8 == 0


def _binding(model) -> Binding:
    b = model.__dict__.get("_gh_binding")
    if b is None:
        b = Binding(model)
        model.__dict__["_gh_binding"] = b
    return b


def _i32(t):
    return t if t.dtype == torch.int32 and t.is_contiguous() else t.to(torch.int32).contiguous()


class _Prepared:
    __slots__ = ("struct", "keep", "b", "b1", "r", "plan", "n_max", "hw", "he", "rows", "w", "c")


def _prepare(model, query, document, kargs, q_adj: PackedAdj, d_adj: PackedAdj, plan, doc):
    m = model
    B, L = query.shape
    n_max = int(kargs[K.FIXED_NUM_EVIDENCES])
    b1, R = doc.shape
    S = GetBatch()
    S.b, S.b1, S.l, S.r, S.n_max = B, b1, L, R, n_max
    training = m.training
    S.collapsed = 0
    if plan is not None:
        S.m_real = plan.m_real
        S.collapsed = 0 if training else 1
        S.goff, S.rowg, S.cids, S.maskf = plan.goff.data_ptr(), plan.rowg.data_ptr(), plan.cids.data_ptr(), plan.maskf.data_ptr()
        rows = plan.m_real
    else:
        S.m_real = -1
        rows = b1 * R
    S.k_keep = int(m.ggnn_with_gsl.gsl1.rate * R)
    q_ids = _i32(query)
    d_ids = _i32(doc)
    q_lens = kargs[K.Query_lens]
    if q_lens.dtype not in (torch.float32, torch.int32, torch.int64):
        q_lens = q_lens.float()
    q_lens = q_lens.contiguous()
    counts = kargs[K.EvidenceCountPerQuery]
    fit = getattr(counts, "_gh_fit", None) == counts._version
    if counts.dtype != torch.int64 or not counts.is_contiguous():
        counts = counts.to(torch.int64).contiguous()
    S.q_ids, S.q_lens = q_ids.data_ptr(), q_lens.data_ptr()
    S.q_lens_kind = {torch.float32: 0, torch.int32: 1, torch.int64: 2}[q_lens.dtype]
    S.q_bits = q_adj.bits.data_ptr()
    S.q_dinv = q_adj.dinv.data_ptr() if q_adj.dinv is not None else None
    S.q_vals = q_adj.vals.data_ptr() if q_adj.vals is not None else None
    S.d_ids = d_ids.data_ptr()
    S.d_bits = d_adj.bits.data_ptr()
    S.d_dinv = d_adj.dinv.data_ptr() if d_adj.dinv is not None else None
    S.d_vals = d_adj.vals.data_ptr() if d_adj.vals is not None else None
    S.counts, S.counts_fit = counts.data_ptr(), 1 if fit else 0
    keep = [q_ids, d_ids, q_lens, counts, q_adj, d_adj, plan]
    if m.use_article_source:
        src = kargs[K.DocSources]
        if src.dtype not in (torch.int32, torch.int64):
            src = src.long()
        src = src.contiguous()
        assert src.numel() == B * n_max
        S.doc_sources, S.doc_sources_i64 = src.data_ptr(), 1 if src.dtype == torch.int64 else 0
        keep.append(src)
    if m.use_claim_source:
        qs = kargs[K.QuerySources]
        if qs.dtype not in (torch.int32, torch.int64):
            qs = qs.long()
        qs = qs.contiguous()
        assert qs.numel() == B
        S.query_sources, S.query_sources_i64 = qs.data_ptr(), 1 if qs.dtype == torch.int64 else 0
        keep.append(qs)
    dc = document
    if dc.dtype not in (torch.int32, torch.int64):
        dc = dc.long()
    dc = dc.contiguous()
    assert dc.numel() == B * n_max * R
    S.document, S.document_i64 = dc.data_ptr(), 1 if dc.dtype == torch.int64 else 0
    keep.append(dc)
    p_claim = float(m.ggnn4claim_1.dropout.p) if (training and hasattr(m.ggnn4claim_1, "dropout")) else 0.0
    fp1 = m.ggnn_with_gsl.feat_prop1
    p_gnn = float(fp1.dropout.p) if (training and hasattr(fp1, "dropout")) else 0.0
    S.drop_claim, S.drop_gnn = p_claim, p_gnn
    if p_claim > 0.0 or p_gnn > 0.0:
        seeds = torch.randint(0, 2 ** 31 - 1, (4,)).tolist()
        S.seed_claim, S.seed_cell1, S.seed_scorer, S.seed_cell2 = seeds
    P = _Prepared()
    P.struct, P.keep, P.b, P.b1, P.r, P.plan, P.n_max = S, keep, B, b1, R, plan, n_max
    P.hw, P.he, P.rows, P.w, P.c = m.num_att_heads_for_words, m.num_att_heads_for_evds, rows, (R + 63) // 64, m.out[1].weight.shape[0]
    return P


def _arena_floats(n: int) -> int:
    n = int(n)
    if n <= (1 << 22):
        return n
    g = 1 << max(22, n.bit_length() - 4)
    return (n + g - 1) // g * g


class _ArenaPool:
    MAX_FREE = 4
    SLACK = 1.30

    def __init__(self):
        self.free = {}
        self.side = {}

    def note_side(self, dev, side):
        if side is not None:
            dev = torch.device(dev)
            self.side[(dev.type, dev.index if dev.index is not None else torch.cuda.current_device())] = side

    def _release(self, t: torch.Tensor):
        s_ = self.side.get((t.device.type, t.device.index))
        if s_ is not None:
            t.record_stream(s_)

    def _list(self, dev):
        dev = torch.device(dev)
        idx = dev.index if (dev.index is not None or dev.type != "cuda") else torch.cuda.current_device()
        return self.free.setdefault((dev.type, idx), [])

    def take(self, n: int, dev) -> torch.Tensor:
        lst = self._list(dev)
        best = None
        for i, t in enumerate(lst):
            if n <= t.numel() <= max(n * self.SLACK, n + (1 << 22)) and (best is None or t.numel() < lst[best].numel()):
                best = i
        if best is not None:
            return lst.pop(best)
        size = _arena_floats(n)
        for t in lst:
            if size / self.SLACK <= t.numel() < size:
                self._release(t)
        lst[:] = [t for t in lst if not (size / self.SLACK <= t.numel() < size)]
        return torch.empty(size, device=dev, dtype=torch.float32)

    def give(self, t: torch.Tensor):
        lst = self._list(t.device)
        lst.append(t)
        while len(lst) > self.MAX_FREE:
            self._release(lst.pop(min(range(len(lst)), key=lambda i: lst[i].numel())))

    def clear(self):
        for lst in self.free.values():
            for t in lst:
                self._release(t)
        self.free.clear()


POOL_ARENAS = os.environ.get("GET_AMD_ARENA_POOL", "1") != "0"


class _GetFused(torch.autograd.Function):

    @staticmethod
    def forward(ctx, binding: Binding, prep: _Prepared, side, *anchors):
        dev = anchors[0].device
        M, _, _, _ = binding.get(False)
        plan = GetPlan()
        _lib.call("gh_get_plan_buffers", ctypes.addressof(M), ctypes.addressof(prep.struct), ctypes.addressof(plan))
        pool = binding.pool if (POOL_ARENAS and any(ctx.needs_input_grad)) else None
        if pool is None and binding.pool.free:
            binding.pool.clear()
        arena = pool.take(plan.fwd_floats, dev) if pool is not None else torch.empty(_arena_floats(plan.fwd_floats), device=dev, dtype=torch.float32)
        obs = torch.empty(int(plan.obs_floats), device=dev, dtype=torch.float32)
        main = _lib.stream()
        side_raw = side.cuda_stream if side is not None else main
        _lib.ensure_workspace(dev)
        if side is not None and not _lib.has_workspace(dev, side_raw):
            with torch.cuda.stream(side):
                _lib.ensure_workspace(dev)
        if side is not None:
            if pool is None:
                arena.record_stream(side)
            else:
                pool.note_side(dev, side)
            obs.record_stream(side)
        _lib.call("gh_get_forward", ctypes.addressof(M), ctypes.addressof(prep.struct), arena.data_ptr(), obs.data_ptr(), main, side_raw)
        B, b1, R = prep.b, prep.b1, prep.r
        phi = obs[plan.phi:plan.phi + B * prep.c].view(B, prep.c)
        word_w = obs[plan.word_w:plan.word_w + prep.rows * prep.hw].view(prep.rows, prep.hw)
        evd_w = obs[plan.evd_w:plan.evd_w + B * prep.n_max * prep.he].view(B, prep.n_max, prep.he)
        score = obs[plan.score:plan.score + b1 * R].view(b1, R)
        keep = obs[plan.keep:plan.keep + b1 * prep.w * 2].view(torch.int64).view(b1, prep.w)
        ctx.binding, ctx.prep, ctx.side, ctx.arena, ctx.obs, ctx.plan_bwd = binding, prep, side, arena, obs, int(plan.bwd_floats)
        ctx.anchor_ids = [id(a) for a in anchors]
        ctx.mark_non_differentiable(score, keep)
        ctx.set_materialize_grads(False)
        ctx.pool = pool
        return phi, word_w, evd_w, score, keep

    @staticmethod
    def backward(ctx, g_phi, g_word_w=None, g_evd_w=None, *_unused):
        binding, prep, side, arena, obs = ctx.binding, ctx.prep, ctx.side, ctx.arena, ctx.obs
        if arena is None:
            raise RuntimeError("get_amd: the fused GET backward ran twice on one forward (retain_graph / autograd.grad followed "
                               "by backward): the activation arena is released by the first backward.  Run the forward again, or "
                               "set GET_AMD_FUSED=0 for the module-by-module path, which supports retain_graph.")
        dev = arena.device
        if g_phi is None and g_word_w is None and g_evd_w is None:
            ctx.arena = None
            return (None, None, None) + (None,) * len(ctx.anchor_ids)
        if g_phi is None:
            g_phi = torch.zeros((prep.b, prep.c), device=dev, dtype=torch.float32)
        g_phi = ops._f32(g_phi)
        g_word_w = ops._f32(g_word_w) if g_word_w is not None else None
        g_evd_w = ops._f32(g_evd_w) if g_evd_w is not None else None
        M, direct, gbuf, views = binding.get(True)
        main = _lib.stream()
        side_raw = side.cuda_stream if side is not None else main
        _lib.ensure_workspace(dev)
        if side is not None and not _lib.has_workspace(dev, side_raw):
            with torch.cuda.stream(side):
                _lib.ensure_workspace(dev)
        pool = ctx.pool
        work = pool.take(ctx.plan_bwd, dev) if pool is not None else torch.empty(_arena_floats(ctx.plan_bwd), device=dev, dtype=torch.float32)
        if side is not None:
            for t in ((None if pool is not None else work), g_phi, gbuf, g_word_w, g_evd_w):
                if t is not None:
                    t.record_stream(side)
        args = (ctypes.addressof(M), ctypes.addressof(prep.struct), arena.data_ptr(), obs.data_ptr(), work.data_ptr(), g_phi.data_ptr(),
                g_word_w.data_ptr() if g_word_w is not None else None, g_evd_w.data_ptr() if g_evd_w is not None else None)
        hook = binding.model.ggnn_with_gsl.grad_milestone_hook
        if hook is None:
            _lib.call("gh_get_backward", *args, 0, main, side_raw)
        else:
            _lib.call("gh_get_backward", *args, 1, main, side_raw)
            if side is not None:
                ops._side_pending.add(dev.index if dev.index is not None else torch.cuda.current_device())
            try:
                hook()
            except BaseException:
                if side is not None:
                    torch.cuda.current_stream(dev).wait_stream(side)
                    for t in (arena, work):
                        t.record_stream(side)
                ctx.arena = None
                raise
            _lib.call("gh_get_backward", *args, 2, main, side_raw)
        ctx.arena = None
        if pool is not None:
            pool.give(arena)
            pool.give(work)
        if direct:
            return (None, None, None) + (None,) * len(ctx.anchor_ids)
        return (None, None, None) + tuple(views.get(i) for i in ctx.anchor_ids)


def model_pool(model) -> _ArenaPool:
    return _binding(model).pool


def eligible(model, query, kargs) -> bool:
    if not ENABLED or not query.is_cuda:
        return False
    if K.DocContentNoPaddingEvidence not in kargs or kargs[K.DocContentNoPaddingEvidence].shape[0] == 0:
        return False
    return _binding(model).eligible()


def forward(model, query, document, kargs):
    binding = _binding(model)
    doc = kargs[K.DocContentNoPaddingEvidence]
    q_adj = ops.as_packed(kargs[K.Query_Adj])
    d_adj = ops.as_packed(kargs[K.Evd_Docs_Adj])
    plan = d_adj.plan
    if plan is not None and plan.m_real <= 0:
        plan = None
    if plan is None and AUTO_COMPACT and not isinstance(kargs[K.Evd_Docs_Adj], PackedAdj):
        plan = _plan_from_dense(d_adj, doc)
    prep = _prepare(model, query, document, kargs, q_adj, d_adj, plan, doc)
    side = ops.side_stream(query.device) if ops.CLAIM_SIDE_STREAM else None
    params = binding.params + [t for t in binding.tables if t.requires_grad]
    if torch.is_grad_enabled() and all(ops._direct(p) for p in params):
        anchors = (params[-1],)
    else:
        anchors = tuple(params)
    phi, word_w, evd_w, score, keep = _GetFused.apply(binding, prep, side, *anchors)
    gw = model.ggnn_with_gsl
    gw.last_score, gw.last_keep = score, keep
    return phi, word_w, evd_w, plan


AUTO_COMPACT = os.environ.get("GET_AMD_AUTO_COMPACT", "1") != "0"


def _plan_from_dense(d_adj: PackedAdj, doc: torch.Tensor):
    n, r = d_adj.n, d_adj.r
    with torch.no_grad():
        real = doc.reshape(n, r) >= 1
        n_nodes = real.sum(1, dtype=torch.int32)
        prefix = torch.arange(r, device=doc.device, dtype=torch.int32)[None, :] < n_nodes[:, None]
        row_has_edges = (d_adj.bits != 0).any(-1)
        bad = ((real != prefix) | (row_has_edges & ~real)).sum()
        m_real, bad = torch.stack([n_nodes.sum().to(torch.int64), bad.to(torch.int64)]).tolist()
    if bad or m_real <= 0 or m_real >= n * r:
        return None
    return ops.RaggedPlan(n_nodes, _i32(doc.reshape(n, r)), int(m_real))


class _CrossEntropy(torch.autograd.Function):

    @staticmethod
    def forward(ctx, phi, labels):
        phi = ops._f32(phi)
        b, c = phi.shape
        labels = labels.to(torch.int64).contiguous()
        out = torch.empty(1 + b * c, device=phi.device, dtype=torch.float32)
        _lib.call("gh_cross_entropy", phi.data_ptr(), labels.data_ptr(), b, c, out.data_ptr(), out[1:].data_ptr(), _lib.stream())
        ctx.save_for_backward(out)
        ctx.shape = (b, c)
        return out[0]

    @staticmethod
    def backward(ctx, g):
        (out,) = ctx.saved_tensors
        if g.data_ptr() == unit_seed(g.device).data_ptr():
            return out[1:].view(ctx.shape).clone(), None
        return out[1:].view(ctx.shape) * g, None


_UNIT = {}


def unit_seed(device) -> torch.Tensor:
    key = (device.type, device.index)
    t = _UNIT.get(key)
    if t is None:
        t = _UNIT[key] = torch.ones((), device=device, dtype=torch.float32)
    return t


def backward(loss: torch.Tensor) -> None:
    if loss.dim() != 0 or loss.dtype != torch.float32 or not loss.is_cuda:
        loss.backward()
        return
    torch.autograd.backward(loss, grad_tensors=[unit_seed(loss.device)])


def cross_entropy(phi: torch.Tensor, labels: torch.Tensor) -> torch.Tensor:
    _lib.require_cuda(phi, labels)
    return _CrossEntropy.apply(phi, labels)
```

### include/get_hip.h

```cpp
#ifndef GET_HIP_H
#define GET_HIP_H

#include <stdint.h>

#ifdef __cplusplus
extern "C" {
#endif

typedef void* gh_stream_t;

#define GH_ABI_VERSION 10

int gh_abi_version(void);
const char* gh_last_error(void);

int gh_graph_build(const int32_t* tokens, const int32_t* lengths, int n_texts, int fixed_length, int window,
                   int32_t* node_ids, int32_t* n_nodes, uint64_t* bits, float* dinv, gh_stream_t stream);

int gh_adj_pack_f64(const double* adj, int n, int r, uint64_t* bits, float* vals, gh_stream_t stream);
int gh_adj_pack_f32(const float* adj, int n, int r, uint64_t* bits, float* vals, gh_stream_t stream);

int gh_ref_depad(const int64_t* counts, int b, int n_max, int r, const void* ids, int ids_i64, const double* adj,
                 int32_t* d_ids, uint64_t* bits, float* vals, float* dinv, int32_t* n_nodes, int64_t* stats, int force_vals,
                 gh_stream_t stream);

int gh_ragged_plan(const int32_t* n_nodes, const int32_t* node_ids, int n, int r, int32_t* goff, int32_t* rowg,
                   int32_t* src, int32_t* cids, float* maskf, gh_stream_t stream);

int gh_spmm(const uint64_t* bits, const float* dinv, const float* vals, const uint64_t* keep,
            const int32_t* goff, int m_real, const float* x, float* y, int n, int r, int h, int transpose,
            int accumulate, gh_stream_t stream);

int gh_spmm_bf16(const uint64_t* bits, const float* dinv, const float* vals, const uint64_t* keep,
                 const int32_t* goff, int m_real, const void* x16, void* y16, int n, int r, int h, int transpose,
                 int accumulate, gh_stream_t stream);

int gh_transpose(const float* w, float* wt, int rows, int cols, gh_stream_t stream);
int gh_transpose_batch(int n, const void* const* src_host, void* const* dst_host, const int* rows_host,
                       const int* cols_host, gh_stream_t stream);

int gh_ggnn_cell_fwd(const uint64_t* bits, const float* dinv, const float* vals, const uint64_t* keep,
                     const int32_t* goff, int m_real, int m_rows,
                     const float* x, const int32_t* ids, int n, int r, int din, int h,
                     const float* w_p, const float* w_z0, const float* w_z1, const float* w_r0,
                     const float* w_r1, const float* w_h0, const float* w_h1,
                     const float* b_z0, const float* b_z1, const float* b_r0, const float* b_r1,
                     const float* b_h0, const float* b_h1,
                     float* xp, float* a, float* z, float* rr, float* rx, float* hh, float* out,
                     float drop_p, uint32_t drop_seed,
                     const float* score_w, float* score_x, float score_drop_p, uint32_t score_drop_seed,
                     gh_stream_t stream);

int gh_ggnn_cell_bwd(const uint64_t* bits, const float* dinv, const float* vals, const uint64_t* keep,
                     const int32_t* goff, int m_real,
                     const float* x, const int32_t* ids, int n, int r, int din, int h,
                     const float* wt_p, const float* wt_z0, const float* wt_z1, const float* wt_r0,
                     const float* wt_r1, const float* wt_h0, const float* wt_h1,
                     const float* xp, const float* a, const float* z, const float* rr, const float* rx,
                     const float* hh, const float* g,
                     float* dhp, float* dzp, float* drp, float* dxp, float* da,
                     float* dx, float* dw_p, float* dw_z0, float* dw_z1, float* dw_r0, float* dw_r1,
                     float* dw_h0, float* dw_h1, float* db_z, float* db_r, float* db_h,
                     float* db_z1, float* db_r1, float* db_h1, float drop_p, uint32_t drop_seed, gh_stream_t stream);

int gh_ggnn_cell_fwd_bf16(const uint64_t* bits, const float* dinv, const float* vals, const uint64_t* keep,
                          const int32_t* goff, int m_real, int m_rows,
                          const void* x, const int32_t* ids, int n, int r, int din, int h,
                          const void* w_p, const void* w_z0, const void* w_z1, const void* w_r0,
                          const void* w_r1, const void* w_h0, const void* w_h1,
                          const float* b_z0, const float* b_z1, const float* b_r0, const float* b_r1,
                          const float* b_h0, const float* b_h1,
                          void* xp, void* a, void* z, void* rr, void* rx, void* hh, void* out, float* out32,
                          float drop_p, uint32_t drop_seed,
                          const float* score_w, float* score_x, float score_drop_p, uint32_t score_drop_seed,
                          gh_stream_t stream);
int gh_ggnn_cell_bwd_bf16(const uint64_t* bits, const float* dinv, const float* vals, const uint64_t* keep,
                          const int32_t* goff, int m_real,
                          const void* x, const int32_t* ids, int n, int r, int din, int h,
                          const void* wt_p, const void* wt_z0, const void* wt_z1, const void* wt_r0,
                          const void* wt_r1, const void* wt_h0, const void* wt_h1,
                          const void* xp, const void* a, const void* z, const void* rr, const void* rx,
                          const void* hh, const float* g,
                          void* dhp, void* dzp, void* drp, void* dxp, void* da,
                          float* dx, float* dw_p, float* dw_z0, float* dw_z1, float* dw_r0, float* dw_r1,
                          float* dw_h0, float* dw_h1, float* db_z, float* db_r, float* db_h,
                          float* db_z1, float* db_r1, float* db_h1, float drop_p, uint32_t drop_seed, gh_stream_t stream);

int gh_scorer_gsl(const uint64_t* bits, const float* dinv, const float* vals, const int32_t* goff, int pads_collapsed,
                  const float* feat, const float* score_x, const float* w_p, const float* gate, int n, int r, int h, int k,
                  float* score, uint64_t* keep, float drop_p, uint32_t drop_seed, gh_stream_t stream);
int gh_gsl_topk(const float* score, int n, int r, int k, uint64_t* keep, gh_stream_t stream);
int gh_adj_unpack(const uint64_t* bits, const float* dinv, const float* vals, const uint64_t* keep,
                  int n, int r, float* adj, gh_stream_t stream);

int gh_concat_att_fwd(const float* left, const float* right, const float* mask, const int32_t* goff,
                      const int32_t* rowg, int m_real, int b, int l, int xl, int dr,
                      int ha, int heads, const float* w1, const float* w2,
                      float* u, float* t, float* e, float* weights, float* attended, gh_stream_t stream);
int gh_concat_att_bwd(const float* left, const float* right, const int32_t* goff, int m_real, int b, int l, int xl,
                      int dr, int ha, int heads,
                      const float* w1t, const float* w2, const float* t, const float* weights,
                      const float* g_att, const float* g_w,
                      float* de, float* dpre, float* du,
                      float* dleft, float* dright, float* dw1, float* dw2, gh_stream_t stream);

int gh_set_gemm_mode(int mode);
int gh_weights_changed(void);
int gh_fp32x3_refresh(gh_stream_t stream);
int gh_fp32x3_clear(void);

int gh_set_workspace(void* ptr, int64_t bytes);
int gh_set_stream_workspace(gh_stream_t stream, void* ptr, int64_t bytes);

int gh_linear_fwd(const float* x, const float* w, const float* bias, float* y, int m, int k, int n,
                  gh_stream_t stream);
int gh_linear_bwd(const float* x, const float* wt, const float* w, const float* g, int m, int k, int n,
                  float* dx, float* dw, float* db, gh_stream_t stream);

int gh_linear_wgrad_bf16(const void* g16, int ldg, const void* x16, int ldx, int m, int n, int k,
                         float* dw, int lddw, float* db, gh_stream_t stream);

int gh_gat_layer_fwd(const uint64_t* bits, const float* vals, const uint64_t* keep, const float* x, const float* w_lin,
                     const float* a, int n, int r, int din, int heads, int f, float alpha, int mode, int layer,
                     float drop_p, uint32_t drop_seed, float* h, float* s, float* stats, float* hp, float* out,
                     gh_stream_t stream);
int gh_gat_layer_bwd(const uint64_t* bits, const float* vals, const uint64_t* keep, const float* x, const float* w_cat,
                     const float* a, int n, int r, int din, int heads, int f, float alpha, int mode, int layer,
                     float drop_p, uint32_t drop_seed, const float* h, const float* s, const float* stats,
                     const float* hp, const float* out, const float* g, float* dh, float* da_part, float* dx,
                     float* dw_cat, float* da, gh_stream_t stream);
int gh_gcn_norm(const uint64_t* bits, const float* dinv, const float* vals, const uint64_t* keep, int n, int r,
                float* scale, gh_stream_t stream);
int gh_feat_dropout(const float* x, float* y, int rows, int cols, float p, uint32_t seed, gh_stream_t stream);
int gh_scale_rows(const float* x, const float* scale, const float* mask, float* y, int rows, int cols, gh_stream_t stream);

int gh_seg_offsets(const int64_t* counts, int b, int32_t* offsets, int32_t* pair2claim, int b1, float* has,
                   gh_stream_t stream);
int gh_seg_broadcast(const float* src, const int32_t* pair2claim, float* dst, int b1, int x, gh_stream_t stream);
int gh_seg_sum(const float* src, const int32_t* offsets, float* dst, int b, int x, gh_stream_t stream);
int gh_seg_pad(const float* src, const int32_t* offsets, float* dst, int b, int n_max, int x, int dst_ld,
               gh_stream_t stream);
int gh_seg_unpad(const float* src, const int32_t* offsets, float* dst, int b, int n_max, int x, int src_ld,
                 gh_stream_t stream);
int gh_evd_assemble_fwd(const float* avg, const int32_t* offsets, const float* table, int table_rows, const void* sources, int sources_i64,
                        const void* document, int document_i64, int b, int n_max, int xa, int ds, int r,
                        float* right, float* mask, gh_stream_t stream);
int gh_evd_assemble_bwd(const float* g, const int32_t* offsets, const void* sources, int sources_i64, int table_rows, int b, int n_max,
                        int xa, int ds, float* d_avg, float* d_table, gh_stream_t stream);
int gh_clamp_events(int64_t* out4_host, int reset);
int gh_masked_mean_fwd(const float* hid, const int32_t* ids, const float* lens, float* dst, int b, int l, int h,
                       gh_stream_t stream);
int gh_masked_mean_bwd(const float* g, const int32_t* ids, const float* lens, float* dhid, int b, int l, int h,
                       gh_stream_t stream);

int gh_adam_step(float* p, const float* g, float* m, float* v, int64_t count, float lr, float beta1, float beta2,
                 float eps, float weight_decay, int step, float grad_scale, gh_stream_t stream);

int gh_comm_unique_id(void* id128);
int gh_comm_init(const void* id128, int rank, int world, void** comm);
int gh_comm_destroy(void* comm);
int gh_comm_info(void* comm, int* rank, int* world);
const char* gh_comm_library(void);
int gh_flat_allreduce(void* comm, float* buf, int64_t count, gh_stream_t stream);
int gh_flat_broadcast(void* comm, float* buf, int64_t count, int root, gh_stream_t stream);

typedef struct gh_cell_params {
  const float *w_p, *w_z0, *w_z1, *w_r0, *w_r1, *w_h0, *w_h1;
  const float *b_z0, *b_z1, *b_r0, *b_r1, *b_h0, *b_h1;
  const float *wt_p, *wt_z0, *wt_z1, *wt_r0, *wt_r1, *wt_h0, *wt_h1;
  float *dw_p, *dw_z0, *dw_z1, *dw_r0, *dw_r1, *dw_h0, *dw_h1;
  float *db_z0, *db_z1, *db_r0, *db_r1, *db_h0, *db_h1;
} gh_cell_params;
typedef struct gh_cell_bf16 {
  const void *w_p, *w_z0, *w_z1, *w_r0, *w_r1, *w_h0, *w_h1;
  const void *wt_p, *wt_z0, *wt_z1, *wt_r0, *wt_r1, *wt_h0, *wt_h1;
} gh_cell_bf16;
typedef struct gh_att_params {
  const float *w1, *w2, *w1t;
  float *dw1, *dw2;
} gh_att_params;
typedef struct gh_get_model {
  int d, h, word_heads, evd_heads, n_classes;
  int claim_src_dim, article_src_dim;
  int claim_src_rows, article_src_rows;
  const float* embedding;
  gh_cell_params claim, cell1, cell2;
  const float* scorer_w;
  const float* scorer_gate;
  gh_att_params att_word, att_evd;
  const float *claim_src_table, *article_src_table;
  float *d_claim_src_table, *d_article_src_table;
  const float *out0_w, *out0_b, *out0_wt;
  const float *out1_w, *out1_b, *out1_wt;
  float *d_out0_w, *d_out0_b, *d_out1_w, *d_out1_b;
  int storage;
  const void* embedding16;
  gh_cell_bf16 cell1_16, cell2_16;
  const void *att_word_w1_16, *att_word_w1t_16;
} gh_get_model;
typedef struct gh_get_batch {
  int b, b1, l, r, n_max;
  int m_real;
  int collapsed;
  int k_keep;
  const int32_t* q_ids;
  const void* q_lens; int q_lens_kind;
  const uint64_t* q_bits; const float* q_dinv; const float* q_vals;
  const int32_t* d_ids;
  const uint64_t* d_bits; const float* d_dinv; const float* d_vals;
  const int32_t *goff, *rowg, *cids; const float* maskf;
  const int64_t* counts;
  int counts_fit;
  const void* doc_sources; int doc_sources_i64;
  const void* query_sources; int query_sources_i64;
  const void* document; int document_i64;
  float drop_claim, drop_gnn;
  uint32_t seed_claim, seed_cell1, seed_scorer, seed_cell2;
} gh_get_batch;
typedef struct gh_get_plan {
  int64_t fwd_floats, bwd_floats, obs_floats;
  int64_t phi, word_w, evd_w, score, keep;
} gh_get_plan;
int gh_get_plan_buffers(const gh_get_model* model, const gh_get_batch* batch, gh_get_plan* plan);
int gh_get_struct_sizes(int64_t* out5_host);
int gh_get_forward(const gh_get_model* model, const gh_get_batch* batch, float* arena_fwd, float* obs, gh_stream_t stream,
                   gh_stream_t side_stream);
int gh_get_backward(const gh_get_model* model, const gh_get_batch* batch, const float* arena_fwd, const float* obs, float* arena_bwd,
                    const float* g_phi, const float* g_word_w, const float* g_evd_w, int phase,
                    gh_stream_t stream, gh_stream_t side_stream);
int gh_cross_entropy(const float* phi, const int64_t* labels, int b, int c, float* loss, float* dphi, gh_stream_t stream);
int gh_get_prepare(const int32_t* claim_tokens, const int32_t* claim_len, int b, int l,
                   const int32_t* evd_tokens, const int32_t* evd_len, int b1, int r, int window,
                   int32_t* q_ids, int32_t* q_n, uint64_t* q_bits, float* q_dinv,
                   int32_t* d_ids, int32_t* d_n, uint64_t* d_bits, float* d_dinv,
                   int m_real, int32_t* goff, int32_t* rowg, int32_t* src, int32_t* cids, float* maskf,
                   const int64_t* slot, int32_t* document, gh_stream_t stream);

int gh_weights_refresh(int n, const void* const* src, void* const* dst_t, void* const* dst_w16, void* const* dst_t16,
                       const int* rows, const int* cols, gh_stream_t stream);

#define GH_PROFILE_ROWS 13
int gh_profile_enable(int on);
int gh_profile_select(uint32_t tag_mask);
int gh_profile_collect(double* out_host, int rows);

int gh_gemm_path_counters(int64_t* out_host, int reset);

#ifdef __cplusplus
}
#endif
#endif
```

Baseline: 165,800.

## Overlap GGNN backward row gathers and split-K reductions on side stream

```diff
diff --git a/get_amd/_lib.py b/get_amd/_lib.py
--- a/get_amd/_lib.py
+++ b/get_amd/_lib.py
@@ -68,6 +68,7 @@
     "gh_get_forward": [_P, _P, _P, _P, _P, _P],
     "gh_get_backward": [_P, _P, _P, _P, _P, _P, _P, _P, _I, _P, _P],
     "gh_cross_entropy": [_P, _P, _I, _I, _P, _P, _P],
+    "gh_cross_entropy_dup": [_P, _P, _I, _I, _P, _P, _P, _P],
     "gh_get_prepare": [_P, _P, _I, _I, _P, _P, _I, _I, _I] + [_P] * 8 + [_I] + [_P] * 5 + [_P, _P, _P],
     "gh_get_struct_sizes": [_P],
     "gh_comm_unique_id": [_P],
diff --git a/get_amd/csrc/common.h b/get_amd/csrc/common.h
--- a/get_amd/csrc/common.h
+++ b/get_amd/csrc/common.h
@@ -78,6 +78,8 @@
 int launch_colsum(const float* a, float* oa, int m, int h, hipStream_t s);
 struct Workspace { float* p; size_t bytes; float* cs; size_t cs_bytes; };
 Workspace workspace_for(hipStream_t s);
+void workspace_busy_until(hipStream_t s, hipEvent_t done);
+hipError_t workspace_acquire(hipStream_t s);
 int launch_gather_rows(const float* table, const int32_t* ids, float* dst, int m, int d, hipStream_t s,
                        float drop_p = 0.f, unsigned drop_seed = 0, int bf16 = 0);
 int launch_tiny_linear_fwd(const float* x, const float* w, const float* bias, float* y, int m, int k, int n, hipStream_t s);
@@ -101,6 +103,18 @@
 
 struct GateFuse { const float* z; const float* hh; const float* xp; float* dhp; float* dzp; float* dxp; int bf16; };
 
+struct CellSide {
+  hipStream_t ss;
+  const float* xgath; hipEvent_t ev_xgath;
+  const float* next_x; const int32_t* next_ids; int next_din; float next_drop_p; uint32_t next_drop_seed;
+  hipEvent_t ev_agg, ev_next;
+  hipEvent_t red_gemm, red_done;
+};
+inline bool cell_bwd_gathers(int bf, const float* xdrop, const int32_t* ids, float drop_p, int din, int h) {
+  if (bf && xdrop && drop_p > 0.f && din <= h) return false;
+  return (ids || drop_p > 0.f || bf) && din <= h;
+}
+
 int cell_fwd_impl(int bf, float* out32, const uint64_t* bits, const float* dinv, const float* vals, const uint64_t* keep,
                   const int32_t* goff, int m_real, int m_rows, const float* x, const int32_t* ids, int n, int r, int din, int h,
                   const float* w_p, const float* w_z0, const float* w_z1, const float* w_r0, const float* w_r1, const float* w_h0,
@@ -119,7 +133,8 @@
                   float* db_r, float* db_h, float* db_z1, float* db_r1, float* db_h1, float drop_p, uint32_t drop_seed, void* stream,
                   void* wstream, hipEvent_t ev_l1, hipEvent_t ev_agg,
                   int pre_done, const GateFuse* next,
-                  const float* xdrop = nullptr);
+                  const float* xdrop = nullptr,
+                  const CellSide* side = nullptr);
 int att_fwd_impl(const float* left, int nl, const int32_t* rowu, const float* right, const float* mask, const int32_t* goff,
                  const int32_t* rowg, int m_real, int b, int l, int xl, int dr, int ha, int heads, const float* w1, const float* w2,
                  float* u, float* t, float* e, float* weights, float* attended, hipStream_t s, int u_mode = 0,
diff --git a/get_amd/csrc/gemm_ops.hip b/get_amd/csrc/gemm_ops.hip
--- a/get_amd/csrc/gemm_ops.hip
+++ b/get_amd/csrc/gemm_ops.hip
@@ -300,6 +300,22 @@
   std::lock_guard<std::mutex> lk(g_ws_mu);
   auto it = g_ws_stream.find(WsKey{current_device(), s});
   return it != g_ws_stream.end() ? it->second : g_ws_default;
+}
+static std::unordered_map<WsKey, hipEvent_t, WsKeyHash> g_ws_busy;
+void workspace_busy_until(hipStream_t s, hipEvent_t done) {
+  std::lock_guard<std::mutex> lk(g_ws_mu);
+  g_ws_busy[WsKey{current_device(), s}] = done;
+}
+hipError_t workspace_acquire(hipStream_t s) {
+  hipEvent_t ev = nullptr;
+  {
+    std::lock_guard<std::mutex> lk(g_ws_mu);
+    auto it = g_ws_busy.find(WsKey{current_device(), s});
+    if (it == g_ws_busy.end()) return hipSuccess;
+    ev = it->second;
+    g_ws_busy.erase(it);
+  }
+  return hipStreamWaitEvent(s, ev, 0);
 }
 
 struct ReduceItem { const float* ws; float* out; int I, J, ldc, ks; long long stride; };
@@ -476,6 +492,8 @@
   float* cs_out2[GH_MAX_PROBLEMS] = {nullptr};
   bool colsum_fused = false;
   bool colsum_missed = false;
+  hipStream_t red_s = nullptr;
+  hipEvent_t red_gemm = nullptr, red_done = nullptr;
   bool split_done = false;
   void want_colsum(float* o, float* o2) { if (L.nprob > 0) { cs_out[L.nprob - 1] = o; cs_out2[L.nprob - 1] = o2; } }
 
@@ -642,14 +660,26 @@
           w += (size_t)L.ksplit * q.M;
           if (q.M / 4 > max_cs) max_cs = q.M / 4;
         }
-        hipError_t e = launch_any();
+        hipError_t e = workspace_acquire(s);
+        if (e == hipSuccess) e = launch_any();
         if (e != hipSuccess) err = e;
+        hipStream_t rs = s;
+        if (red_s && red_s != s && red_gemm && red_done && err == hipSuccess) {
+          e = hipEventRecord(red_gemm, s);
+          if (e == hipSuccess) e = hipStreamWaitEvent(red_s, red_gemm, 0);
+          if (e != hipSuccess) err = e; else rs = red_s;
+        }
         for (int i = 0; i < RC.n; ++i) R.it[R.n++] = RC.it[i];
         if (max_cs > max_elems) max_elems = max_cs;
-        hipLaunchKernelGGL(reduce_partials_kernel, dim3((max_elems + 255) / 256, R.n), dim3(256), 0, s, R);
+        hipLaunchKernelGGL(reduce_partials_kernel, dim3((max_elems + 255) / 256, R.n), dim3(256), 0, rs, R);
         if (RC.n > 0) colsum_fused = true;
         e = hipGetLastError();
         if (e != hipSuccess) err = e;
+        if (rs != s) {
+          e = hipEventRecord(red_done, rs);
+          if (e != hipSuccess) err = e;
+          workspace_busy_until(s, red_done);
+        }
         reset();
         return;
       }
@@ -729,7 +759,8 @@
     }
     L.ksplit = ks;
     L.kchunk = ct * 16;
-    hipError_t e = launch_any();
+    hipError_t e = workspace_acquire(s);
+    if (e == hipSuccess) e = launch_any();
     if (e != hipSuccess) err = e;
     F.split = (ks >= 16 && max_m <= 8192) ? 1 : 0;
     hipLaunchKernelGGL(nt_finish_kernel, dim3(F.split ? max_m : (max_m + 3) / 4, F.n), dim3(256), 0, s, F);
@@ -928,7 +959,7 @@
                                 float* dw_h0, float* dw_h1, float* db_z, float* db_r, float* db_h,
                                 float* db_z1, float* db_r1, float* db_h1, float drop_p, uint32_t drop_seed,
                                 gh_stream_t stream, gh_stream_t wstream, hipEvent_t ev_l1, hipEvent_t ev_agg,
-                                int pre_done, const GateFuse* next, const float* xdrop) {
+                                int pre_done, const GateFuse* next, const float* xdrop, const CellSide* side) {
   hipStream_t s = (hipStream_t)stream;
   hipStream_t sw = wstream ? (hipStream_t)wstream : s;
   const bool two = sw != s;
@@ -992,6 +1023,14 @@
     GH_CHECK_HIP(hipEventRecord(ev_agg, s));
     GH_CHECK_HIP(hipStreamWaitEvent(sw, ev_agg, 0));
   }
+  if (side && side->next_x && side->ss != s) {
+    GH_REQUIRE(!two && (side->xgath || !cell_bwd_gathers(bf, xdrop, ids, drop_p, din, h)) && side->ev_agg && side->ev_next && side->next_din <= h,
+               "ggnn_cell_bwd: the next cell's operand rows need this cell's `da` scratch to be free");
+    GH_CHECK_HIP(hipEventRecord(side->ev_agg, s));
+    GH_CHECK_HIP(hipStreamWaitEvent(side->ss, side->ev_agg, 0));
+    if (int e = launch_gather_rows(side->next_x, side->next_ids, da, M, side->next_din, side->ss, side->next_drop_p, side->next_drop_seed, bf)) return e;
+    GH_CHECK_HIP(hipEventRecord(side->ev_next, side->ss));
+  }
   if (dx || next) {
     GH_REQUIRE(!next || (din % 4 == 0 && (next->bf16 != 0) == (bf != 0)), "ggnn_cell_bwd: the fused gate head needs float4-shaped rows and both cells in the same storage mode");
     Batch b(false, M, s, wide && din % 256 == 0, 5, din);
@@ -1007,6 +1046,7 @@
   }
   {
     Batch b(true, M, sw);
+    if (side && !two && side->red_gemm && side->ss != s) { b.red_s = side->ss; b.red_gemm = side->red_gemm; b.red_done = side->red_done; }
     if (!two) {
       b.add(tn_problem(h, h, dw_z0, h, dzp, h, a, h, M, nullptr, bf));  if (cs) b.want_colsum(db_z, db_z1);
       b.add(tn_problem(h, h, dw_z1, h, dzp, h, xp, h, M, nullptr, bf));
@@ -1017,6 +1057,9 @@
     }
     if (bf && xdrop && drop_p > 0.f && din <= h) {
       b.add(tn_problem(h, din, dw_p, din, dxp, h, xdrop, din, M, nullptr, bf));
+    } else if (side && side->xgath && cell_bwd_gathers(bf, xdrop, ids, drop_p, din, h)) {
+      if (side->ev_xgath) GH_CHECK_HIP(hipStreamWaitEvent(sw, side->ev_xgath, 0));
+      b.add(tn_problem(h, din, dw_p, din, dxp, h, side->xgath, din, M, nullptr, bf));
     } else if ((ids || drop_p > 0.f || bf) && din <= h) {
       if (int e = launch_gather_rows(x, ids, da, M, din, sw, drop_p, drop_seed, bf)) return e;
       b.add(tn_problem(h, din, dw_p, din, dxp, h, da, din, M, nullptr, bf));
@@ -1117,6 +1160,7 @@
       const size_t need = (size_t)nb * (size_t)M * heads * sizeof(float);
       if (M >= 8192 && wsp.p && need <= wsp.bytes && ha % 4 == 0) {
         blocks = true;
+        GH_CHECK_HIP(workspace_acquire(s));
         bt.e_block_stride = (long long)M * heads;
         p.e = wsp.p;
         e_parts = wsp.p; n_parts = nb;
@@ -1177,6 +1221,7 @@
   const Workspace wsp = workspace_for(s);
   const bool late = dleft_late && dw2_buf && ha % 4 == 0;
   dw2_part = late ? dw2_buf : ((wsp.p && dw2_bytes <= wsp.bytes && ha % 4 == 0) ? wsp.p : nullptr);
+  if (dw2_part && !late) GH_CHECK_HIP(workspace_acquire(s));
   if (int e = launch_att_dpre(de, w2, t, goff, m_real, b, l, ha, heads, dpre, du, dw2_part, s, dw_written ? dw_tmp : nullptr,
                               dw_written ? weights : nullptr, dw_written ? de : nullptr, dpre16,
                               (long long)m_real * heads, dw_written > 1 ? dw_written : 1)) return e;
diff --git a/get_amd/csrc/model_ops.hip b/get_amd/csrc/model_ops.hip
--- a/get_amd/csrc/model_ops.hip
+++ b/get_amd/csrc/model_ops.hip
@@ -252,7 +252,7 @@
 
 __global__ void __launch_bounds__(256)
 cross_entropy_kernel(const float* __restrict__ phi, const int64_t* __restrict__ labels, int B, int C, float* __restrict__ loss,
-                     float* __restrict__ dphi, unsigned int* __restrict__ clamped) {
+                     float* __restrict__ dphi, float* __restrict__ dphi2, unsigned int* __restrict__ clamped) {
   __shared__ float part[256];
   float acc = 0.f;
   const float invb = 1.f / (float)B;
@@ -267,7 +267,11 @@
     const int y = yl < 0 ? 0 : (yl >= C ? C - 1 : (int)yl);
     if (yl < 0 || yl >= C) atomicAdd(clamped, 1u);
     acc += lse - p[y];
-    for (int c = 0; c < C; ++c) dphi[(size_t)b * C + c] = (expf(p[c] - lse) - (c == y ? 1.f : 0.f)) * invb;
+    for (int c = 0; c < C; ++c) {
+      const float g = (expf(p[c] - lse) - (c == y ? 1.f : 0.f)) * invb;
+      dphi[(size_t)b * C + c] = g;
+      if (dphi2) dphi2[(size_t)b * C + c] = g;
+    }
   }
   part[threadIdx.x] = acc;
   __syncthreads();
@@ -327,7 +331,7 @@
 static int cell_bwd(const gh_cell_params& c, const gh_cell_bf16* c16, const CellBuf& cb, const float* A, const uint64_t* bits, const float* dinv,
                     const float* vals, const uint64_t* keep, const int32_t* goff, int m_real, const float* x, const int32_t* ids, int n,
                     int r, int din, int h, const float* g, float* W, const int64_t* sc, float* dx, float drop_p, uint32_t seed,
-                    hipStream_t s, int pre_done = 0, const GateFuse* next = nullptr) {
+                    hipStream_t s, int pre_done = 0, const GateFuse* next = nullptr, const CellSide* side = nullptr) {
   GH_REQUIRE(c.dw_p && c.db_z0 && c.db_z1, "get_backward: a cell's gradient outputs are missing");
   if (c16) {
     typedef const float* cf;
@@ -337,13 +341,13 @@
                          (cf)c16->wt_r0, (cf)c16->wt_r1, (cf)c16->wt_h0, (cf)c16->wt_h1, A + cb.xp, A + cb.a, A + cb.z, A + cb.rr,
                          A + cb.rx, A + cb.hh, g, W + sc[0], W + sc[1], W + sc[2], W + sc[3], W + sc[4], dx, c.dw_p, c.dw_z0, c.dw_z1,
                          c.dw_r0, c.dw_r1, c.dw_h0, c.dw_h1, c.db_z0, c.db_r0, c.db_h0, c.db_z1, c.db_r1, c.db_h1, drop_p, seed, (void*)s,
-                         nullptr, nullptr, nullptr, pre_done, next, cb.xdrop >= 0 ? A + cb.xdrop : nullptr);
+                         nullptr, nullptr, nullptr, pre_done, next, cb.xdrop >= 0 ? A + cb.xdrop : nullptr, side);
   }
   GH_REQUIRE(c.wt_p, "get_backward: a cell's transposes are missing");
   return cell_bwd_impl(0, bits, dinv, vals, keep, goff, m_real, x, ids, n, r, din, h, c.wt_p, c.wt_z0, c.wt_z1, c.wt_r0, c.wt_r1,
                        c.wt_h0, c.wt_h1, A + cb.xp, A + cb.a, A + cb.z, A + cb.rr, A + cb.rx, A + cb.hh, g, W + sc[0], W + sc[1],
                        W + sc[2], W + sc[3], W + sc[4], dx, c.dw_p, c.dw_z0, c.dw_z1, c.dw_r0, c.dw_r1, c.dw_h0, c.dw_h1, c.db_z0,
-                       c.db_r0, c.db_h0, c.db_z1, c.db_r1, c.db_h1, drop_p, seed, (void*)s, nullptr, nullptr, nullptr, pre_done, next);
+                       c.db_r0, c.db_h0, c.db_z1, c.db_r1, c.db_h1, drop_p, seed, (void*)s, nullptr, nullptr, nullptr, pre_done, next, nullptr, side);
 }
 
 extern "C" int gh_get_forward(const gh_get_model* Mo, const gh_get_batch* Ba, float* A, float* O, gh_stream_t stream, gh_stream_t side_stream) {
@@ -479,7 +483,27 @@
   const gh_cell_bf16* c16_1 = d.bf ? &Mo->cell1_16 : nullptr;
   const gh_cell_bf16* c16_2 = d.bf ? &Mo->cell2_16 : nullptr;
   const float* table1 = d.bf ? (const float*)Mo->embedding16 : Mo->embedding;
+  const bool off_chain = ss != s;
+  const float* xdrop1 = (d.bf && f.c1.xdrop >= 0) ? A + f.c1.xdrop : nullptr;
+  const float* xdrop2 = (d.bf && f.c2.xdrop >= 0) ? A + f.c2.xdrop : nullptr;
+  const bool gath2 = off_chain && cell_bwd_gathers(d.bf ? 1 : 0, xdrop2, nullptr, Ba->drop_gnn, H, H);
+  const bool gath1 = off_chain && phase == 0 && d.Mr > 0 && cell_bwd_gathers(d.bf ? 1 : 0, xdrop1, ids1, Ba->drop_gnn, d.D, H) &&
+                     (gath2 || !cell_bwd_gathers(d.bf ? 1 : 0, xdrop2, nullptr, Ba->drop_gnn, H, H));
+  CellSide side2 = {ss, nullptr, nullptr, nullptr, nullptr, 0, 0.f, 0u, nullptr, nullptr, nullptr, nullptr};
+  CellSide side1 = side2;
+  if (gath2) { side2.xgath = Wb + w.sc1[4]; side2.ev_xgath = ev.ev[7]; }
+  if (gath1) {
+    side2.next_x = table1; side2.next_ids = ids1; side2.next_din = d.D; side2.next_drop_p = Ba->drop_gnn; side2.next_drop_seed = Ba->seed_cell1;
+    side2.ev_agg = ev.ev[8]; side2.ev_next = ev.ev[9];
+    side1.xgath = Wb + w.sc2[4]; side1.ev_xgath = ev.ev[9];
+  }
+  if (off_chain && phase == 0) { side2.red_gemm = ev.ev[10]; side2.red_done = ev.ev[11]; }
   if (phase != 2) {
+    if (gath2) {
+      GH_TRY(stream_after(ss, s, ev.ev[6]));
+      GH_TRY(launch_gather_rows(A + f.c1.out, nullptr, Wb + w.sc1[4], d.Mr, H, ss, Ba->drop_gnn, Ba->seed_cell2, d.bf ? 1 : 0));
+      GH_CHECK_HIP(hipEventRecord(ev.ev[7], ss));
+    }
     if (d.C <= 8 && H % 4 == 0 && Mo->out0_w && Mo->out1_w && head_bwd_lds(d.B, H, d.C, d.E, Mo->out0_w) > 0) {
       GH_TRY(launch_head_bwd(g_phi, A + f.y0, Mo->out1_w, Mo->out0_w, d.B, H, d.C, d.Xl, d.E, Wb + w.d_y0, Mo->d_out1_w, Mo->d_out1_b,
                              Wb + w.d_new_left, 0, Wb + w.d_att_e, s));
@@ -524,30 +548,34 @@
                     Wb + w.d_qhid, Wb, w.qs, nullptr, Ba->drop_claim, Ba->seed_claim, ss));
     if (fuse_gate)
       GH_TRY(cell_bwd(Mo->cell2, c16_2, f.c2, A, Ba->d_bits, Ba->d_dinv, Ba->d_vals, keep, goff, d.Mr, A + f.c1.out, nullptr, d.B1, d.R, H, H,
-                      Wb + w.g2, Wb, w.sc2, nullptr, Ba->drop_gnn, Ba->seed_cell2, s, 1, &gf1));
+                      Wb + w.g2, Wb, w.sc2, nullptr, Ba->drop_gnn, Ba->seed_cell2, s, 1, &gf1, &side2));
     else
       GH_TRY(cell_bwd(Mo->cell2, c16_2, f.c2, A, Ba->d_bits, Ba->d_dinv, Ba->d_vals, keep, goff, d.Mr, A + f.c1.out, nullptr, d.B1, d.R, H, H,
-                      Wb + w.g2, Wb, w.sc2, Wb + w.dx2, Ba->drop_gnn, Ba->seed_cell2, s, 0, nullptr));
+                      Wb + w.g2, Wb, w.sc2, Wb + w.dx2, Ba->drop_gnn, Ba->seed_cell2, s, 0, nullptr, &side2));
   }
   if (phase != 1) {
     if (fuse_gate)
       GH_TRY(cell_bwd(Mo->cell1, c16_1, f.c1, A, Ba->d_bits, Ba->d_dinv, Ba->d_vals, nullptr, goff, d.Mr, table1, ids1, d.B1, d.R, d.D, H,
-                      nullptr, Wb, w.sc1, nullptr, Ba->drop_gnn, Ba->seed_cell1, s, 1, nullptr));
+                      nullptr, Wb, w.sc1, nullptr, Ba->drop_gnn, Ba->seed_cell1, s, 1, nullptr, &side1));
     else
       GH_TRY(cell_bwd(Mo->cell1, c16_1, f.c1, A, Ba->d_bits, Ba->d_dinv, Ba->d_vals, nullptr, goff, d.Mr, table1, ids1, d.B1, d.R, d.D, H,
-                      Wb + w.dx2, Wb, w.sc1, nullptr, Ba->drop_gnn, Ba->seed_cell1, s, 0, nullptr));
+                      Wb + w.dx2, Wb, w.sc1, nullptr, Ba->drop_gnn, Ba->seed_cell1, s, 0, nullptr, &side1));
     GH_TRY(stream_after(s, ss, ev.ev[5]));
   }
   return 0;
 }
 
-extern "C" int gh_cross_entropy(const float* phi, const int64_t* labels, int b, int c, float* loss, float* dphi, gh_stream_t stream) {
+extern "C" int gh_cross_entropy_dup(const float* phi, const int64_t* labels, int b, int c, float* loss, float* dphi, float* dphi2,
+                                    gh_stream_t stream) {
   GH_REQUIRE(b > 0 && c > 0 && phi && labels && loss && dphi, "cross_entropy: bad arguments");
   unsigned int* cl = clamp_counter();
   GH_REQUIRE(cl, "cross_entropy: cannot allocate the clamp counter");
-  hipLaunchKernelGGL(cross_entropy_kernel, dim3(1), dim3(256), 0, (hipStream_t)stream, phi, labels, b, c, loss, dphi, cl);
+  hipLaunchKernelGGL(cross_entropy_kernel, dim3(1), dim3(256), 0, (hipStream_t)stream, phi, labels, b, c, loss, dphi, dphi2, cl);
   GH_LAUNCH_CHECK();
   return 0;
+}
+extern "C" int gh_cross_entropy(const float* phi, const int64_t* labels, int b, int c, float* loss, float* dphi, gh_stream_t stream) {
+  return gh_cross_entropy_dup(phi, labels, b, c, loss, dphi, nullptr, stream);
 }
 
 extern "C" int gh_get_prepare(const int32_t* claim_tokens, const int32_t* claim_len, int b, int l,
diff --git a/get_amd/fused.py b/get_amd/fused.py
--- a/get_amd/fused.py
+++ b/get_amd/fused.py
@@ -529,19 +529,26 @@
     def forward(ctx, phi, labels):
         phi = ops._f32(phi)
         b, c = phi.shape
+        n = b * c
         labels = labels.to(torch.int64).contiguous()
-        out = torch.empty(1 + b * c, device=phi.device, dtype=torch.float32)
-        _lib.call("gh_cross_entropy", phi.data_ptr(), labels.data_ptr(), b, c, out.data_ptr(), out[1:].data_ptr(), _lib.stream())
+        out = torch.empty(2 * n + 1, device=phi.device, dtype=torch.float32)
+        _lib.call("gh_cross_entropy_dup", phi.data_ptr(), labels.data_ptr(), b, c, out[n:].data_ptr(), out[n + 1:].data_ptr(),
+                  out.data_ptr(), _lib.stream())
         ctx.save_for_backward(out)
         ctx.shape = (b, c)
-        return out[0]
+        ctx.spare = True
+        return out[n]
 
     @staticmethod
     def backward(ctx, g):
         (out,) = ctx.saved_tensors
+        n = ctx.shape[0] * ctx.shape[1]
         if g.data_ptr() == unit_seed(g.device).data_ptr():
-            return out[1:].view(ctx.shape).clone(), None
-        return out[1:].view(ctx.shape) * g, None
+            if ctx.spare:
+                ctx.spare = False
+                return out[:n].view(ctx.shape), None
+            return out[n + 1:].view(ctx.shape).clone(), None
+        return out[n + 1:].view(ctx.shape) * g, None
 
 
 _UNIT = {}
diff --git a/include/get_hip.h b/include/get_hip.h
--- a/include/get_hip.h
+++ b/include/get_hip.h
@@ -229,6 +229,8 @@
                     const float* g_phi, const float* g_word_w, const float* g_evd_w, int phase,
                     gh_stream_t stream, gh_stream_t side_stream);
 int gh_cross_entropy(const float* phi, const int64_t* labels, int b, int c, float* loss, float* dphi, gh_stream_t stream);
+int gh_cross_entropy_dup(const float* phi, const int64_t* labels, int b, int c, float* loss, float* dphi, float* dphi2,
+                         gh_stream_t stream);
 int gh_get_prepare(const int32_t* claim_tokens, const int32_t* claim_len, int b, int l,
                    const int32_t* evd_tokens, const int32_t* evd_len, int b1, int r, int window,
                    int32_t* q_ids, int32_t* q_n, uint64_t* q_bits, float* q_dinv,
```

Result: no change. 166,000 (median of 6 runs) (+0.2%).
